# skhu101/SHERF

Hardware: AMD Instinct MI355X
Metric: rendered rays/sec at 512x512x64 samples (ImportanceRenderer.forward) (higher is better)
Workload: dtype f16 MFMA (fp16 operands rounded to nearest, one product, fp32 accumulate), fp32 elsewhere

## Files before the change

include/sherf_hip.h:

```cpp
#ifndef SHERF_HIP_H
#define SHERF_HIP_H
#include <stdint.h>

#ifdef __cplusplus
extern "C" {
#endif

typedef void* sherf_stream_t;

#define SHERF_OK 0
#define SHERF_EINVAL (-1)
#define SHERF_ELAUNCH (-2)

#define SHERF_V 6890
#define SHERF_NJ 24
#define SHERF_MAX_CELLS (64 * 64 * 64)
#define SHERF_SHELL_RADIUS 0.05f

int sherf_version(void);
const char* sherf_last_error(void);
int sherf_set_debug(int flags);

int sherf_smpl_bones(const float* poses, const float* shapes, int n_sets, const float* J_template,
                     const float* J_shapedirs, const int32_t* parents, float* A, float* posefeat,
                     sherf_stream_t stream);

int sherf_smpl_offsets(const float* posedirs, const float* shapedirs, const float* posefeat,
                       const float* shapes, int n_sets, float* PO, float* SO, sherf_stream_t stream);

int sherf_smpl_t2c_table(const float* weights, const float* A_tgt, const float* A_big, const float* PO_tgt,
                         const float* SO_tgt, const float* PO_big, float* T2C, sherf_stream_t stream);

int sherf_smpl_c2s_table(const float* weights, const float* A_big, const float* A_obs, const float* PO_big,
                         const float* SO_obs, const float* PO_obs, const float* R_obs, const float* Th_obs,
                         const float* cam_R, const float* cam_T, const float* cam_K, float* C2S,
                         sherf_stream_t stream);

int sherf_build_cells(const float* verts, int n, const float* R, const float* Th, float cell_size,
                      float* grid_hdr, int32_t* cell_start, float* cell_pts, int32_t* scratch,
                      uint32_t* near_mask, sherf_stream_t stream);
int sherf_build_cells2(const float* verts_a, const float* R_a, const float* Th_a, const float* verts_b, int n,
                       float cell_size, float* grid_hdr, int32_t* cell_start, float* cell_pts, int32_t* scratch,
                       uint32_t* near_mask, sherf_stream_t stream);
#define SHERF_NEAR_SUBCELLS 524288
int sherf_build_near_lists(const float* grid_hdr, const float* cell_pts, int n, float radius, int32_t* near_hdr,
                           uint16_t* near_list, int64_t list_cap, uint32_t* near_mask, sherf_stream_t stream);

int sherf_sample_mask_nn(const float* ray_o, const float* ray_d, const float* near, const float* far,
                         int R, int S, const float* Rg, const float* Th, const float* grid_hdr,
                         const int32_t* cell_start, const float* cell_pts, const uint32_t* near_mask,
                         int64_t capacity, int32_t* counters, int32_t* ray_base, int32_t* ray_cnt, int32_t* cs_idx,
                         int32_t* cs_vid, float* cs_xs, int32_t* dense_vid, uint64_t* ray_mask,
                         int32_t* scan_ws, const int32_t* near_hdr, const uint16_t* near_list, sherf_stream_t stream);

int sherf_warp_geom(const int32_t* counters, const int32_t* cs_idx, const int32_t* cs_vid, const float* cs_xs,
                    const float* ray_d, int S, const float* Rg, const float* T2C, const float* C2S,
                    const float* t_verts, const float* tgrid_hdr, const int32_t* tcell_start,
                    const float* tcell_pts, int64_t capacity, float* geom, int32_t* cs_tvid,
                    sherf_stream_t stream);

typedef struct {
    const uint32_t* wp;
    const float* rows;
    int32_t D, H, W;
} sherf_vox_level;

int sherf_gather_tokens(const int32_t* counters, const float* geom, const float* planes_f, int P,
                        const float* feat_f, int Hf, int Wf, const float* img4, int H, int W,
                        const sherf_vox_level* levels_host, const float* tok_bias, const float* bounds,
                        const float* vox_min, const int32_t* vox_sh_host, int mode, int64_t capacity, float* tokens,
                        float* extras, sherf_stream_t stream);

int sherf_gather_tokens_bwd(const int32_t* counters, const float* geom, const float* d_tokens, int P, int Hf, int Wf,
                            int H, int W, const sherf_vox_level* levels_host, const float* bounds, const float* vox_min,
                            const int32_t* vox_sh_host, int64_t capacity, float* d_planes_f, float* d_feat_f,
                            float* d_rows0, float* d_rows1, float* d_rows2, float* d_tok_bias, sherf_stream_t stream);
int sherf_gather_tokens_bwd_binned(const int32_t* counters, const float* geom, const float* d_tokens, int P, int Hf, int Wf,
                                   int H, int W, const sherf_vox_level* levels_host, const float* bounds, const float* vox_min,
                                   const int32_t* vox_sh_host, int64_t capacity, float* d_planes_f, float* d_feat_f,
                                   float* d_rows0, float* d_rows1, float* d_rows2, float* d_tok_bias, int32_t* scratch,
                                   int64_t scratch_words, sherf_stream_t stream);
int sherf_gather_bwd_scratch_words(const sherf_vox_level* levels_host, int64_t capacity, int64_t* words_host);
int sherf_gather_tokens_bwd_masked(const int32_t* counters, const float* geom, const float* d_tokens, int P, int Hf, int Wf,
                                   int H, int W, const sherf_vox_level* levels_host, const float* bounds, const float* vox_min,
                                   const int32_t* vox_sh_host, int64_t capacity, float* d_planes_f, float* d_feat_f,
                                   float* d_rows0, float* d_rows1, float* d_rows2, float* d_tok_bias, int32_t* scratch,
                                   int64_t scratch_words, int branches, sherf_stream_t stream);

int sherf_fold_tables(const float* in, const float* Wt, float* out, int HW, int groups, int pix_stride,
                      int64_t group_base, int out_half, sherf_stream_t stream);
int sherf_img_to_hwc4(const float* img, float* out, int HW, sherf_stream_t stream);

int sherf_nerf_mlp(const int32_t* counters, const float* tokens, const float* extras, const void* wstream,
                   const float* wbias, int prec, int64_t capacity, float* out, sherf_stream_t stream);
#define SHERF_MLP_NO_TRANSFORMER 256
#define SHERF_MLP_OSG_DECODER 512
int sherf_osg_decoder(const int32_t* counters, const float* tokens, const float* extras, const float* weights, int flags,
                      int64_t capacity, float* out, sherf_stream_t stream);
int sherf_nerf_mlp_part(const int32_t* counters, const float* tokens, const float* extras, const void* wstream,
                        const float* wbias, int prec, int64_t capacity, float* out, int part, int nparts, sherf_stream_t stream);
int sherf_nerf_mlp2(const int32_t* counters, const float* tokens, const float* extras, const void* wstream,
                    const float* wbias, int prec, int64_t capacity, float* out, sherf_stream_t stream);
int sherf_nerf_mlp3(const int32_t* counters, const float* tokens, const float* extras, const void* wstream,
                    const float* wbias, int prec, int64_t capacity, float* out, sherf_stream_t stream);
int sherf_nerf_mlp3_part(const int32_t* counters, const float* tokens, const float* extras, const void* wstream, const float* wbias, int prec,
                         int64_t capacity, float* out, int part, int nparts, int wgs_per_cu, sherf_stream_t stream);
int sherf_gather_tokens_pe(const int32_t* counters, const float* geom, const float* planes_f, int P,
                           const float* feat_f, int Hf, int Wf, const float* img4, int H, int W,
                           const sherf_vox_level* levels_host, const float* tok_bias, const float* bounds,
                           const float* vox_min, const int32_t* vox_sh_host, int mode, int64_t capacity, float* tokens,
                           float* extras, void* pefrag, sherf_stream_t stream);
int sherf_nerf_mlp3_pe(const int32_t* counters, const float* tokens, const float* extras, const void* pefrag, const void* wstream,
                       const float* wbias, int prec, int64_t capacity, float* out, sherf_stream_t stream);
int sherf_nerf_mlp_split(const int32_t* counters, const float* tokens, const float* extras, const void* wstream,
                         const float* wbias, int prec, int64_t capacity, void* zfrag, float* out, sherf_stream_t stream);
int sherf_mlp_pack_stream(const float* flat, const int32_t* src, int64_t n_slots, int prec, void* stream_out,
                          const int32_t* bias_src, int n_bias, float* bias_out, int32_t* flag, sherf_stream_t stream);
int sherf_mlp_stream_layout(int prec, int32_t* n_steps, int32_t* step_pieces_host, int32_t* units, int32_t max_steps);

#define SHERF_COMPOSITE_WHITE_BACK 1
#define SHERF_COMPOSITE_SOFTPLUS 2

int sherf_composite_compact(const int32_t* counters, const int32_t* ray_base, const int32_t* ray_cnt,
                            const int32_t* cs_idx, const float* sample_out, const float* ray_d,
                            const float* near, const float* far, int R, int S, int white_back, float* rgb,
                            float* depth, float* acc, sherf_stream_t stream);
int sherf_composite_compact_cap(int32_t* counters, const int32_t* ray_base, const int32_t* ray_cnt,
                                const int32_t* cs_idx, const float* sample_out, const float* ray_d,
                                const float* near, const float* far, int R, int S, int white_back, int64_t tok_cap,
                                float* rgb, float* depth, float* acc, sherf_stream_t stream);

int sherf_composite_compact_bwd(const int32_t* ray_base, const int32_t* ray_cnt, const int32_t* cs_idx,
                                const float* sample_out, const float* ray_d, const float* near, const float* far,
                                int R, int S, int white_back, const float* d_rgb, const float* d_acc,
                                float* d_sample_out, sherf_stream_t stream);

int sherf_composite_dense(const float* colors, const float* sigma, const float* depths, const float* rays_d,
                          int R, int S, int white_back, const float* dminmax, float* rgb, float* depth,
                          float* weights, sherf_stream_t stream);
int sherf_composite_dense_bwd(const float* colors, const float* sigma, const float* depths, const float* rays_d,
                              int R, int S, int white_back, const float* dminmax, const float* d_rgb,
                              const float* d_depth, const float* d_weights, float* d_colors, float* d_sigma,
                              sherf_stream_t stream);

int sherf_svox_mark_rows(const int32_t* coord, int n, int D, int H, int W, uint32_t* bitmap, sherf_stream_t stream);
int sherf_svox_mark_down(const int32_t* keys, const int32_t* n_rows, int D, int H, int W, uint32_t* bitmap_out,
                         int max_rows, sherf_stream_t stream);
int sherf_svox_scan(const uint32_t* bitmap, int n_words, int32_t* prefix, int32_t* n_rows, int32_t* chunk_ws,
                    uint32_t* wp, sherf_stream_t stream);
int sherf_svox_keys(const uint32_t* bitmap, const int32_t* prefix, int n_words, int32_t* keys, sherf_stream_t stream);
int sherf_svox_scatter_rows(const int32_t* coord, const float* feat, int n, int C, int D, int H, int W,
                            const uint32_t* bitmap, const int32_t* prefix, const int32_t* n_rows, int64_t* acc_fix,
                            float* g, int32_t* mult, sherf_stream_t stream);
int sherf_svox_conv3(const int32_t* keys_out, const int32_t* n_rows_out, int Do, int Ho, int Wo,
                     const uint32_t* wp_in, int Di, int Hi, int Wi, const float* in_raw, int Cin,
                     const float* in_bn, const int32_t* in_mult, const void* w_packed, int Cout, int mode,
                     int max_rows, float* out_raw, int64_t* out_acc, sherf_stream_t stream);
int sherf_svox_conv3_dgrad(const int32_t* keys_i, const int32_t* n_rows_i, int Di, int Hi, int Wi, const uint32_t* wp_o, int Do,
                           int Ho, int Wo, const float* d_raw, int Cout, const uint32_t* d_raw_amax, const void* w_packed_t,
                           int Cin, int down, int max_rows, float* d_in, sherf_stream_t stream);
int sherf_svox_bn_finalize(const int64_t* acc, const int32_t* n_total_rows, int C, const float* gamma, const float* beta,
                           float* stats, int training, float* bnparam, sherf_stream_t stream);
int sherf_svox_bn_running_update(int n_layers, const float* const* stats, float* const* running_mean, float* const* running_var,
                                 int64_t* const* num_batches_tracked, const int32_t* const* n_rows, const int32_t* channels,
                                 const float* momentum, sherf_stream_t stream);
#define SHERF_SVOX_MAX_LAYERS 16
typedef struct {
    uint32_t* bitmap;
    int32_t* prefix;
    int32_t* n_rows;
    int32_t* chunk_ws;
    uint32_t* wp;
    int32_t* keys;
    int32_t n_words, cap, D, H, W, pad_;
} sherf_svox_level_ws;
typedef struct {
    int32_t cin, cout, down, tap;
    const void* wt;
    const float* gamma;
    const float* beta;
    float* stats;
    float* bnparam;
    float* out;
    int64_t* acc;
} sherf_svox_layer;
typedef struct {
    sherf_svox_level_ws lev[4];
    sherf_svox_layer layers[SHERF_SVOX_MAX_LAYERS];
    int32_t n_layers, pad_;
    int64_t* acc_fix;
    float* g0;
    int32_t* mult;
    const int32_t* n_total;
    void* zero_ptr;
    int64_t zero_bytes;
    const float* fold_mat[3];
    float* fold_rows[3];
} sherf_svox_plan;
int sherf_svox_encode(const sherf_svox_plan* plan, const int32_t* coord, const float* feat, int n, int training,
                      sherf_vox_level* levels_out_host, sherf_stream_t stream);

#define SHERF_FRAME_EXACT_GRIDS 1
#define SHERF_FRAME_HALF_TABLES 2
#define SHERF_FRAME_ENCODER_SINGLE 4
#define SHERF_FRAME_MLP_SPLIT 8
#define SHERF_FRAME_MLP_TWO_TILES 32
#define SHERF_FRAME_MLP_PIPELINED 64
#define SHERF_FRAME_REPORT_COUNT 16
#define SHERF_FRAME_PE_FRAGS 128
#define SHERF_FRAME_REUSE_OBSERVATION 256
typedef struct {
    const float* poses; const float* shapes;
    const float* J_template; const float* J_shapedirs; const int32_t* parents;
    const float* posedirs; const float* shapedirs; const float* weights;
    float* A; float* posefeat; float* PO; float* SO; float* T2C; float* C2S;
    const float* obs_R; const float* obs_Th; const float* cam_R; const float* cam_T; const float* cam_K;
    const float* verts; const float* Rg; const float* Th; const float* tverts;
    float* grid_hdr; int32_t* cell_start; float* cell_pts; int32_t* cell_scratch; uint32_t* near_mask;
    const float* ray_o; const float* ray_d; const float* near; const float* far;
    int32_t R, S; int64_t capacity;
    int32_t* counters; int32_t* ray_base; int32_t* ray_cnt; int32_t* cs_idx; int32_t* cs_vid; float* cs_xs;
    int32_t* dense_vid; uint64_t* ray_mask; int32_t* scan_ws;
    const float* planes; const float* Wa_t; float* planes_f; int32_t P, flags;
    const float* obs_feat; const float* Wb_t; float* feat_f; int32_t Hf, Wf;
    const float* obs_img; float* img4; int32_t H, W;
    float* geom; int32_t* cs_tvid;
    const float* tok_bias; const float* bounds; const float* vox_min; int32_t vox_sh[3]; int32_t gather_split;
    float* tokens; float* extras;
    const sherf_svox_plan* vox_plan; const int32_t* vox_coord; const float* vox_feat; int32_t vox_n, vox_training;
    const void* wstream; const float* wbias; int32_t mlp_prec, mlp_parts; float* sample_out;
    int32_t white_back;
    int32_t main_after_layer;
    float* rgb; float* depth; float* acc;
    void* zfrag;
    int32_t* near_hdr; uint16_t* near_list; int64_t near_list_cap;
    int64_t tok_capacity;
    void* pefrag;
    int32_t* sticky;
} sherf_frame;
int sherf_render_frame(const sherf_frame* frame, int phase, sherf_vox_level* levels_out_host, sherf_stream_t stream_main,
                       sherf_stream_t stream_side, sherf_stream_t stream_aux);
int sherf_points_mask_nn(const float* points, int64_t n, const float* Rg, const float* Th, const float* grid_hdr,
                         const int32_t* cell_start, const float* cell_pts, const uint32_t* near_mask, int64_t capacity,
                         int32_t* counters, int32_t* ray_base, int32_t* ray_cnt, int32_t* cs_idx, int32_t* cs_vid, float* cs_xs,
                         int32_t* dense_vid, uint64_t* ray_mask, int32_t* scan_ws, const int32_t* near_hdr,
                         const uint16_t* near_list, sherf_stream_t stream);
int sherf_field_scatter(int32_t* counters, const uint64_t* ray_mask, const int32_t* ray_base, const float* sample_out,
                        int64_t n, int64_t tok_cap, float* rgb, float* sigma, uint8_t* mask, sherf_stream_t stream);
typedef struct {
    const float* points;
    const float* dirs;
    int64_t n;
    float* rgb;
    float* sigma;
    uint8_t* mask;
} sherf_field_query;
int sherf_query_field(const sherf_frame* frame, const sherf_field_query* query, sherf_vox_level* levels_out_host,
                      sherf_stream_t stream_main, sherf_stream_t stream_side, sherf_stream_t stream_aux);

int sherf_frame_count(int32_t* nv_host);
int sherf_frame_graphs(int enable);
int sherf_frame_graph_stats(int64_t* stats_host, int32_t n);
int sherf_frame_observation_stats(int64_t* stats_host, int32_t n);
int sherf_struct_sizes(int32_t* sizes_host, int32_t n);
#define SHERF_PROF_FIELDS 8
int sherf_profile_frames(int enable);
int sherf_profile_frames_read(float* ms_host, int32_t max_n, int32_t* n_host);

int sherf_vertex_features(const float* verts, const int32_t* tri, const int32_t* last_face, int V, const float* cam_R,
                          const float* cam_T, const float* cam_K, const float* feat, int Hf, int Wf, const float* img, int H, int W,
                          const float* Wp, const float* bp, float* f3d, uint8_t* front, sherf_stream_t stream);
int sherf_voxelize(const float* t_verts, const float* can, int V, float* bounds, int32_t* coord, int32_t* out_sh,
                   sherf_stream_t stream);

int sherf_ray_sampler(const float* cam2world, const float* intrinsics, int N, int res, float* origins,
                      float* dirs, sherf_stream_t stream);
int sherf_dataset_rays(const double* K_inv, const double* Rc, const double* Tc, const double* bounds, int H, int W,
                       float* ray_o, float* ray_d, float* near, float* far, uint8_t* mask_at_box,
                       sherf_stream_t stream);

#ifdef __cplusplus
}
#endif
#endif
```

sherf_amd/_lib.py:

```python
import ctypes
import os
import re

import torch

_HERE = os.path.dirname(os.path.abspath(__file__))
HEADER = os.path.join(_HERE, '..', 'include', 'sherf_hip.h')
LIB_PATH = os.environ.get('SHERF_HIP_LIB') or os.path.join(_HERE, 'libsherf_hip.so')

_lib = None
_protos = None


_vp, _i32, _i64 = ctypes.c_void_p, ctypes.c_int32, ctypes.c_int64


class VoxLevel(ctypes.Structure):
    _fields_ = [('wp', _vp), ('rows', _vp), ('D', _i32), ('H', _i32), ('W', _i32)]


class SvoxLevelWs(ctypes.Structure):
    _fields_ = [(n, _vp) for n in ('bitmap', 'prefix', 'n_rows', 'chunk_ws', 'wp', 'keys')] + \
               [(n, _i32) for n in ('n_words', 'cap', 'D', 'H', 'W', 'pad_')]


class SvoxLayer(ctypes.Structure):
    _fields_ = [(n, _i32) for n in ('cin', 'cout', 'down', 'tap')] + \
               [(n, _vp) for n in ('wt', 'gamma', 'beta', 'stats', 'bnparam', 'out', 'acc')]


SVOX_MAX_LAYERS = 16


class SvoxPlan(ctypes.Structure):
    _fields_ = [('lev', SvoxLevelWs * 4), ('layers', SvoxLayer * SVOX_MAX_LAYERS), ('n_layers', _i32), ('pad_', _i32),
                ('acc_fix', _vp), ('g0', _vp), ('mult', _vp), ('n_total', _vp), ('zero_ptr', _vp), ('zero_bytes', _i64),
                ('fold_mat', _vp * 3), ('fold_rows', _vp * 3)]


def _frame_fields():
    f = []
    P = lambda *names: f.extend((n, _vp) for n in names)
    I = lambda *names: f.extend((n, _i32) for n in names)
    P('poses', 'shapes', 'J_template', 'J_shapedirs', 'parents', 'posedirs', 'shapedirs', 'weights',
      'A', 'posefeat', 'PO', 'SO', 'T2C', 'C2S', 'obs_R', 'obs_Th', 'cam_R', 'cam_T', 'cam_K',
      'verts', 'Rg', 'Th', 'tverts', 'grid_hdr', 'cell_start', 'cell_pts', 'cell_scratch', 'near_mask',
      'ray_o', 'ray_d', 'near', 'far')
    I('R', 'S')
    f.append(('capacity', _i64))
    P('counters', 'ray_base', 'ray_cnt', 'cs_idx', 'cs_vid', 'cs_xs', 'dense_vid', 'ray_mask', 'scan_ws')
    P('planes', 'Wa_t', 'planes_f'); I('P', 'flags')
    P('obs_feat', 'Wb_t', 'feat_f'); I('Hf', 'Wf')
    P('obs_img', 'img4'); I('H', 'W')
    P('geom', 'cs_tvid', 'tok_bias', 'bounds', 'vox_min')
    f.append(('vox_sh', _i32 * 3)); I('gather_split')
    P('tokens', 'extras', 'vox_plan', 'vox_coord', 'vox_feat'); I('vox_n', 'vox_training')
    P('wstream', 'wbias'); I('mlp_prec', 'mlp_parts')
    P('sample_out'); I('white_back', 'main_after_layer')
    P('rgb', 'depth', 'acc', 'zfrag', 'near_hdr', 'near_list')
    f.append(('near_list_cap', _i64))
    f.append(('tok_capacity', _i64))
    P('pefrag')
    P('sticky')
    return f


class Frame(ctypes.Structure):
    _fields_ = _frame_fields()


class FieldQuery(ctypes.Structure):
    _fields_ = [('points', _vp), ('dirs', _vp), ('n', _i64), ('rgb', _vp), ('sigma', _vp), ('mask', _vp)]


_STRUCTS = (VoxLevel, SvoxLevelWs, SvoxLayer, SvoxPlan, Frame)


COMPOSITE_WHITE_BACK, COMPOSITE_SOFTPLUS = 1, 2
CLAMP_MODES = ('relu', 'softplus')


def composite_bits(white_back, clamp_mode='relu'):
    if clamp_mode not in CLAMP_MODES:
        raise AssertionError("MipRayMarcher only supports `clamp_mode`=`softplus`!")
    return (COMPOSITE_WHITE_BACK if white_back else 0) | (COMPOSITE_SOFTPLUS if clamp_mode == 'softplus' else 0)


BRANCH_PLANES, BRANCH_PIXEL, BRANCH_VOXEL = 1, 2, 4


def branch_mask(on):
    return (BRANCH_PLANES if on[0] else 0) | (BRANCH_PIXEL if on[1] else 0) | (BRANCH_VOXEL if on[2] else 0)


MLP_NO_TRANSFORMER, MLP_OSG_DECODER = 256, 512


FRAME_REUSE_OBSERVATION = 256


def frame_observation_stats():
    s = (ctypes.c_int64 * 2)()
    call('sherf_frame_observation_stats', s, 2)
    return int(s[0]), int(s[1])


_SCALARS = {'int': ctypes.c_int, 'int32_t': ctypes.c_int32, 'int64_t': ctypes.c_int64, 'float': ctypes.c_float,
            'sherf_stream_t': ctypes.c_void_p}


def parse_header(path=HEADER):
    src = open(path).read()
    src = re.sub(r'/\*.*?\*/', '', src, flags=re.S)
    protos = {}
    for m in re.finditer(r'(int|const char\*)\s+(sherf_\w+)\s*\(([^;{]*?)\)\s*;', src, flags=re.S):
        ret, name, args = m.group(1), m.group(2), m.group(3).strip()
        parsed = []
        if args and args != 'void':
            for a in args.split(','):
                a = ' '.join(a.split())
                is_ptr = '*' in a
                base = a.replace('const ', '').replace('*', ' ').split()
                ctype = ctypes.c_void_p if is_ptr else _SCALARS[base[0]]
                parsed.append((ctype, is_ptr, base[-1]))
        protos[name] = (ctypes.c_char_p if ret != 'int' else ctypes.c_int, parsed)
    return protos


def _init():
    global _lib, _protos
    if _lib is not None:
        return _lib
    if not os.path.exists(LIB_PATH):
        raise RuntimeError(f'{LIB_PATH} not found: build it with `python -m sherf_amd.build` '
                           '(hipcc --offload-arch=gfx950). There is no CPU fallback.')
    lib = ctypes.CDLL(LIB_PATH)
    _protos = parse_header()
    for name, (ret, args) in _protos.items():
        fn = getattr(lib, name)
        fn.restype = ret
        fn.argtypes = [a[0] for a in args]
    sizes = (ctypes.c_int32 * len(_STRUCTS))()
    if lib.sherf_struct_sizes(sizes, len(_STRUCTS)) != 0 or [int(v) for v in sizes] != [ctypes.sizeof(c) for c in _STRUCTS]:
        raise RuntimeError(f'struct layout mismatch between include/sherf_hip.h and sherf_amd/_lib.py: '
                           f'{[int(v) for v in sizes]} vs {[ctypes.sizeof(c) for c in _STRUCTS]}')
    _lib = lib
    return lib


def lib():
    return _init()


def addr(t, dtype=None):
    p = ptr(t, dtype)
    return None if p is None else p.value


def ptr(t, dtype=None, channels_last_ok=False):
    if t is None:
        return None
    if not isinstance(t, torch.Tensor):
        raise RuntimeError(f'expected a tensor, got {type(t)}')
    if not t.is_cuda:
        raise RuntimeError('sherf_amd: tensor is not on a GPU; the HIP path has no CPU fallback')
    if not t.is_contiguous() and not (channels_last_ok and t.ndim == 4 and t.is_contiguous(memory_format=torch.channels_last)):
        raise RuntimeError('sherf_amd: tensor must be contiguous')
    if dtype is not None and t.dtype != dtype:
        raise RuntimeError(f'sherf_amd: expected dtype {dtype}, got {t.dtype}')
    return ctypes.c_void_p(t.data_ptr())


def stream():
    return ctypes.c_void_p(torch.cuda.current_stream().cuda_stream)


def call(name, *args):
    l = _init()
    rc = getattr(l, name)(*args)
    if rc != 0:
        raise RuntimeError(f'{name} failed ({rc}): {l.sherf_last_error().decode()}')


HEADER_BWD = os.path.join(_HERE, '..', 'include', 'sherf_hip_bwd.h')
LIB_BWD_PATH = os.path.join(_HERE, 'libsherf_hip_bwd.so')
_lib_bwd = None


def lib_bwd():
    global _lib_bwd
    if _lib_bwd is None:
        if not os.path.exists(LIB_BWD_PATH):
            raise RuntimeError(f'{LIB_BWD_PATH} not found: build it with `python -m sherf_amd.build`')
        l = ctypes.CDLL(LIB_BWD_PATH)
        for name, (ret, args) in parse_header(HEADER_BWD).items():
            fn = getattr(l, name)
            fn.restype = ret
            fn.argtypes = [a[0] for a in args]
        _lib_bwd = l
    return _lib_bwd


def call_bwd(name, *args):
    l = lib_bwd()
    rc = getattr(l, name)(*args)
    if rc != 0:
        raise RuntimeError(f'{name} failed ({rc}): {l.sherf_bwd_last_error().decode()}')


HEADER_OPS = os.path.join(_HERE, '..', 'include', 'sherf_hip_ops.h')
LIB_OPS_PATH = os.path.join(_HERE, 'libsherf_hip_ops.so')
_lib_ops = None


def lib_ops():
    global _lib_ops
    if _lib_ops is None:
        if not os.path.exists(LIB_OPS_PATH):
            raise RuntimeError(f'{LIB_OPS_PATH} not found: build it with `python -m sherf_amd.build`. There is no CPU fallback.')
        l = ctypes.CDLL(LIB_OPS_PATH)
        for name, (ret, args) in parse_header(HEADER_OPS).items():
            fn = getattr(l, name)
            fn.restype = ret
            fn.argtypes = [a[0] for a in args]
        _lib_ops = l
    return _lib_ops


def call_ops(name, *args):
    l = lib_ops()
    rc = getattr(l, name)(*args)
    if rc != 0:
        raise RuntimeError(f'{name} failed ({rc}): {l.sherf_ops_last_error().decode()}')
```

sherf_amd/csrc/frame.hip:

```cpp
#include "common.h"

#include <algorithm>
#include <chrono>
#include <cstdlib>
#include <functional>
#include <mutex>

int sherf_svox_encode_impl(const sherf_svox_plan* p, const int32_t* coord, const float* feat, int n, int training,
                           sherf_vox_level* levels_out_host, sherf_stream_t stream, hipEvent_t ev, int ev_layer,
                           sherf_stream_t aux, hipEvent_t* lev_ev, const std::function<int()>* after_levels, int fold_half);
int sherf_sample_mask_nn_impl(const float* ray_o, const float* ray_d, const float* near, const float* far, int R, int S, const float* Rg, const float* Th,
                              const float* grid_hdr, const int32_t* cell_start, const float* cell_pts, const uint32_t* near_mask, int64_t capacity,
                              int32_t* counters, int32_t* ray_base, int32_t* ray_cnt, int32_t* cs_idx, int32_t* cs_vid, float* cs_xs, int32_t* dense_vid,
                              uint64_t* ray_mask, int32_t* scan_ws, const int32_t* near_hdr, const uint16_t* near_list, sherf_stream_t stream,
                              int32_t* sticky);
int sherf_warp_geom_impl(const int32_t* counters, const int32_t* cs_idx, const int32_t* cs_vid, const float* cs_xs, const float* ray_d, int S, const float* Rg,
                         const float* T2C, const float* C2S, const float* t_verts, const float* tgrid_hdr, const int32_t* tcell_start, const float* tcell_pts,
                         int64_t capacity, float* geom, int32_t* cs_tvid, sherf_stream_t stream);
int sherf_points_mask_nn_impl(const float* points, int64_t n, const float* Rg, const float* Th, const float* grid_hdr, const int32_t* cell_start,
                              const float* cell_pts, const uint32_t* near_mask, int64_t capacity, int32_t* counters, int32_t* ray_base, int32_t* ray_cnt,
                              int32_t* cs_idx, int32_t* cs_vid, float* cs_xs, int32_t* dense_vid, uint64_t* ray_mask, int32_t* scan_ws, const int32_t* near_hdr,
                              const uint16_t* near_list, sherf_stream_t stream, int32_t* sticky);

namespace {

constexpr int kMaxDev = 16;
constexpr int kRing = 64;
constexpr int kMaxParts = 8;

struct DevState {
    bool init = false;
    hipEvent_t ev_start, ev_smpl, ev_enc, ev_mid, ev_fold, ev_lev[8], ev_cnt, ev_part[kMaxParts], ev_mlp;
    int32_t* host_nv = nullptr;
    hipEvent_t ev_rep[8];
    int rep_next = 0;
    unsigned long long rep_seq[8] = {0, 0, 0, 0, 0, 0, 0, 0}, rep_counter = 0;
    hipStream_t cap_stream = nullptr;
};
thread_local int t_rep_last[kMaxDev] = {-1, -1, -1, -1, -1, -1, -1, -1, -1, -1, -1, -1, -1, -1, -1, -1};
thread_local unsigned long long t_rep_seq[kMaxDev] = {0};
DevState g_dev[kMaxDev];
std::mutex g_mu;
std::mutex g_frame_mu;

constexpr int kEv = 7;
bool g_prof_on = false;
int g_prof_n = 0;
hipEvent_t g_prof_ev[kRing][kEv];
float g_prof_host_ms[kRing];
bool g_prof_init = false;

}

extern "C" int sherf_struct_sizes(int32_t* sizes_host, int32_t n) {
    SHERF_CHECK_ARG(sizes_host && n >= 5);
    sizes_host[0] = (int32_t)sizeof(sherf_vox_level);
    sizes_host[1] = (int32_t)sizeof(sherf_svox_level_ws);
    sizes_host[2] = (int32_t)sizeof(sherf_svox_layer);
    sizes_host[3] = (int32_t)sizeof(sherf_svox_plan);
    sizes_host[4] = (int32_t)sizeof(sherf_frame);
    return SHERF_OK;
}

extern "C" int sherf_profile_frames(int enable) {
    std::lock_guard<std::mutex> lk(g_mu);
    if (enable && !g_prof_init) {
        for (int i = 0; i < kRing; ++i)
            for (int j = 0; j < kEv; ++j) SHERF_HIP_CHECK(hipEventCreate(&g_prof_ev[i][j]));
        g_prof_init = true;
    }
    g_prof_on = enable != 0;
    g_prof_n = 0;
    return SHERF_OK;
}

extern "C" int sherf_profile_frames_read(float* ms_host, int32_t max_n, int32_t* n_host) {
    SHERF_CHECK_ARG(ms_host && n_host && max_n > 0);
    std::lock_guard<std::mutex> lk(g_mu);
    const int have = g_prof_n < kRing ? g_prof_n : kRing;
    const int n = have < max_n ? have : max_n;
    const int first = g_prof_n - have;
    for (int i = 0; i < n; ++i) {
        const int slot = (first + i) % kRing;
        float* o = ms_host + (size_t)i * SHERF_PROF_FIELDS;
        SHERF_HIP_CHECK(hipEventSynchronize(g_prof_ev[slot][kEv - 1]));
        o[0] = g_prof_host_ms[slot];
        for (int j = 1; j < kEv; ++j) SHERF_HIP_CHECK(hipEventElapsedTime(&o[j], g_prof_ev[slot][0], g_prof_ev[slot][j]));
        o[7] = o[5] - o[4];
    }
    *n_host = n;
    return SHERF_OK;
}

extern "C" int sherf_frame_count(int32_t* nv_host) {
    SHERF_CHECK_ARG(nv_host);
    int dev = 0;
    SHERF_HIP_CHECK(hipGetDevice(&dev));
    SHERF_CHECK_ARG(dev >= 0 && dev < kMaxDev);
    DevState& d = g_dev[dev];
    const int slot = t_rep_last[dev];
    hipEvent_t ev;
    auto overtaken = [&]() -> int {
        snprintf(g_sherf_err, sizeof(g_sherf_err), "sherf_frame_count: eight later frames on this device have reused the slot of this thread's last frame");
        return SHERF_EINVAL;
    };
    {
        std::lock_guard<std::mutex> frame_lock(g_frame_mu);
        SHERF_CHECK_ARG(d.init && slot >= 0);
        if (d.rep_seq[slot] != t_rep_seq[dev]) return overtaken();
        ev = d.ev_rep[slot];
    }
    SHERF_HIP_CHECK(hipEventSynchronize(ev));
    const int32_t nv = d.host_nv[8 + slot];
    {
        std::lock_guard<std::mutex> frame_lock(g_frame_mu);
        if (d.rep_seq[slot] != t_rep_seq[dev]) return overtaken();
    }
    *nv_host = nv;
    return SHERF_OK;
}

static int render_frame_enqueue(const sherf_frame* f, int phase, sherf_vox_level* levels, sherf_stream_t stream_main,
                                sherf_stream_t stream_side, sherf_stream_t stream_aux, const sherf_field_query* q = nullptr) {
    hipStream_t main = as_stream(stream_main), side = as_stream(stream_side);
    if (phase == 4) {
        SHERF_CHECK_ARG(f->R > 0 && f->S > 0 && f->capacity > 0);
        const bool lists = f->near_hdr && f->near_list;
        SHERF_RUN(sherf_build_cells2(f->verts, f->Rg, f->Th, f->tverts, SHERF_V, 0.05f, f->grid_hdr, f->cell_start, f->cell_pts,
                                     f->cell_scratch, lists ? nullptr : f->near_mask, stream_main));
        if (lists)
            SHERF_RUN(sherf_build_near_lists(f->grid_hdr, f->cell_pts, SHERF_V, 0.05f, f->near_hdr, f->near_list, f->near_list_cap, f->near_mask, stream_main));
        SHERF_RUN(sherf_sample_mask_nn_impl(f->ray_o, f->ray_d, f->near, f->far, f->R, f->S, f->Rg, f->Th, f->grid_hdr, f->cell_start,
                                       f->cell_pts, f->near_mask, f->capacity, f->counters, f->ray_base, f->ray_cnt, f->cs_idx,
                                       f->cs_vid, f->cs_xs, f->dense_vid, f->ray_mask, f->scan_ws, f->near_hdr, f->near_list, stream_main, f->sticky));
        return SHERF_OK;
    }
    const int64_t tok_cap = (f->tok_capacity > 0 && f->tok_capacity < f->capacity) ? f->tok_capacity : f->capacity;
    const auto host_t0 = std::chrono::steady_clock::now();
    static int cur_slot = -1;
#define SHERF_PROF(j, strm) do { if (cur_slot >= 0) SHERF_HIP_CHECK(hipEventRecord(g_prof_ev[cur_slot][j], strm)); } while (0)
    if (phase & 1) {
        int dev = 0;
        SHERF_HIP_CHECK(hipGetDevice(&dev));
        SHERF_CHECK_ARG(dev >= 0 && dev < kMaxDev);
        DevState& d = g_dev[dev];
        {
            std::lock_guard<std::mutex> lk(g_mu);
            if (!d.init) {
                const unsigned evf = hipEventDisableTiming | ((sherf_experiment() & 4) ? hipEventReleaseToDevice : 0u);
                SHERF_HIP_CHECK(hipEventCreateWithFlags(&d.ev_start, evf));
                SHERF_HIP_CHECK(hipEventCreateWithFlags(&d.ev_smpl, evf));
                SHERF_HIP_CHECK(hipEventCreateWithFlags(&d.ev_enc, evf));
                SHERF_HIP_CHECK(hipEventCreateWithFlags(&d.ev_mid, evf));
                SHERF_HIP_CHECK(hipEventCreateWithFlags(&d.ev_fold, evf));
                for (int k = 0; k < 8; ++k) SHERF_HIP_CHECK(hipEventCreateWithFlags(&d.ev_lev[k], evf));
                SHERF_HIP_CHECK(hipEventCreateWithFlags(&d.ev_cnt, hipEventDisableTiming));
                for (int k = 0; k < kMaxParts; ++k) SHERF_HIP_CHECK(hipEventCreateWithFlags(&d.ev_part[k], evf));
                SHERF_HIP_CHECK(hipEventCreateWithFlags(&d.ev_mlp, evf));
                SHERF_HIP_CHECK(hipHostMalloc(reinterpret_cast<void**>(&d.host_nv), 64, 0));
                for (int k = 0; k < 8; ++k) SHERF_HIP_CHECK(hipEventCreateWithFlags(&d.ev_rep[k], hipEventDisableTiming));
                d.init = true;
            }
        }
        SHERF_CHECK_ARG((q || (f->R > 0 && f->S > 0)) && f->capacity > 0 && f->vox_plan);
        const int V = SHERF_V;
        {
            std::lock_guard<std::mutex> lk(g_mu);
            cur_slot = g_prof_on ? g_prof_n % kRing : -1;
        }
        const int xp = sherf_experiment();
        SHERF_HOST_STAMP(xp, "frame enter");
        SHERF_PROF(0, main);
        SHERF_GPU_STAMP(xp, main, "frame start");
        SHERF_CAP_TRACE("record ev_start");
        SHERF_HIP_CHECK(hipEventRecord(d.ev_start, main));
        SHERF_CAP_TRACE("side waits ev_start");
        SHERF_HIP_CHECK(hipStreamWaitEvent(side, d.ev_start, 0));
        const bool reuse = (f->flags & SHERF_FRAME_REUSE_OBSERVATION) != 0;
        auto smpl_tables = [&](sherf_stream_t st) -> int {
            SHERF_RUN(sherf_smpl_bones(f->poses, f->shapes, 3, f->J_template, f->J_shapedirs, f->parents, f->A, f->posefeat, st));
            SHERF_RUN(sherf_smpl_offsets(f->posedirs, f->shapedirs, f->posefeat, f->shapes, 3, f->PO, f->SO, st));
            const float *A0 = f->A, *A1 = f->A + 24 * 12, *A2 = f->A + 2 * 24 * 12;
            const float *PO0 = f->PO, *PO1 = f->PO + V * 3, *PO2 = f->PO + 2 * V * 3;
            const float *SO0 = f->SO, *SO2 = f->SO + 2 * V * 3;
            SHERF_RUN(sherf_smpl_t2c_table(f->weights, A0, A1, PO0, SO0, PO1, f->T2C, st));
            SHERF_RUN(sherf_smpl_c2s_table(f->weights, A1, A2, PO1, SO2, PO2, f->obs_R, f->obs_Th, f->cam_R, f->cam_T, f->cam_K,
                                           f->C2S, st));
            SHERF_HIP_CHECK(hipEventRecord(d.ev_smpl, as_stream(st)));
            SHERF_PROF(1, as_stream(st));
            return SHERF_OK;
        };
        if (!stream_aux) SHERF_RUN(smpl_tables(stream_side));
        const int stagger = reuse ? -1 : f->main_after_layer;
        const int half_tables = (f->flags & SHERF_FRAME_HALF_TABLES) ? 1 : 0;
        auto fold_tables = [&](sherf_stream_t st) -> int {
            SHERF_RUN(sherf_fold_tables(f->planes, f->Wa_t, f->planes_f, f->P * f->P, 3, 32, (int64_t)f->P * f->P * 32, half_tables, st));
            SHERF_RUN(sherf_fold_tables(f->obs_feat, f->Wb_t, f->feat_f, f->Hf * f->Wf, 2, 64, 32, half_tables, st));
            return sherf_img_to_hwc4(f->obs_img, f->img4, f->H * f->W, st);
        };
        SHERF_CAP_TRACE("fold tables on aux");
        if (stream_aux) {
            SHERF_HIP_CHECK(hipStreamWaitEvent(as_stream(stream_aux), d.ev_start, 0));
            if (reuse) {
                SHERF_RUN(smpl_tables(stream_aux));
            } else {
                SHERF_RUN(fold_tables(stream_aux));
                SHERF_HIP_CHECK(hipEventRecord(d.ev_fold, as_stream(stream_aux)));
            }
        }
        const size_t ncell1 = (size_t)SHERF_MAX_CELLS + 1;
        auto enqueue_encoder = [&]() -> int {
            if (reuse) {
                SHERF_PROF(2, side);
                return SHERF_OK;
            }
            const std::function<int()> smpl_on_aux = [&]() -> int { return smpl_tables(stream_aux); };
            SHERF_RUN(sherf_svox_encode_impl(f->vox_plan, f->vox_coord, f->vox_feat, f->vox_n, f->vox_training, levels, stream_side,
                                             stagger >= 0 ? d.ev_mid : nullptr, stagger, stream_aux, d.ev_lev,
                                             stream_aux ? &smpl_on_aux : nullptr,
                                             half_tables | ((f->flags & SHERF_FRAME_ENCODER_SINGLE) ? 2 : 0)));
            SHERF_HIP_CHECK(hipEventRecord(d.ev_enc, side));
            SHERF_PROF(2, side);
            return SHERF_OK;
        };
        const bool encoder_first = stagger >= 0 || (xp & 8);
        SHERF_CAP_TRACE("cells");
        if (encoder_first) SHERF_RUN(enqueue_encoder());
        const bool lists = f->near_hdr && f->near_list;
        SHERF_RUN(sherf_build_cells2(f->verts, f->Rg, f->Th, f->tverts, V, 0.05f, f->grid_hdr, f->cell_start, f->cell_pts,
                                     f->cell_scratch, lists ? nullptr : f->near_mask, stream_main));
        if (stagger >= 0) SHERF_HIP_CHECK(hipStreamWaitEvent(main, stagger < f->vox_plan->n_layers ? d.ev_mid : d.ev_enc, 0));
        SHERF_CAP_TRACE("near lists");
        if (lists)
            SHERF_RUN(sherf_build_near_lists(f->grid_hdr, f->cell_pts, V, 0.05f, f->near_hdr, f->near_list, f->near_list_cap, f->near_mask, stream_main));
        SHERF_CAP_TRACE("sampler");
        if (q)
            SHERF_RUN(sherf_points_mask_nn_impl(q->points, q->n, f->Rg, f->Th, f->grid_hdr, f->cell_start, f->cell_pts, f->near_mask, f->capacity, f->counters,
                                                f->ray_base, f->ray_cnt, f->cs_idx, f->cs_vid, f->cs_xs, f->dense_vid, f->ray_mask, f->scan_ws, f->near_hdr,
                                                f->near_list, stream_main, f->sticky));
        else
        SHERF_RUN(sherf_sample_mask_nn_impl(f->ray_o, f->ray_d, f->near, f->far, f->R, f->S, f->Rg, f->Th, f->grid_hdr, f->cell_start,
                                       f->cell_pts, f->near_mask, f->capacity, f->counters, f->ray_base, f->ray_cnt, f->cs_idx,
                                       f->cs_vid, f->cs_xs, f->dense_vid, f->ray_mask, f->scan_ws, f->near_hdr, f->near_list, stream_main, f->sticky));
        SHERF_CAP_TRACE("sampler queued");
        if (f->flags & SHERF_FRAME_REPORT_COUNT) {
            const int slot = d.rep_next;
            d.rep_next = (d.rep_next + 1) % 8;
            SHERF_HIP_CHECK(hipMemcpyAsync(d.host_nv + 8 + slot, f->counters, sizeof(int32_t), hipMemcpyDeviceToHost, main));
            SHERF_HIP_CHECK(hipEventRecord(d.ev_rep[slot], main));
            t_rep_last[dev] = slot;
            d.rep_seq[slot] = t_rep_seq[dev] = ++d.rep_counter;
        }
        const bool exact = (f->flags & SHERF_FRAME_EXACT_GRIDS) != 0;
        if (exact) {
            SHERF_HIP_CHECK(hipMemcpyAsync(d.host_nv, f->counters, sizeof(int32_t), hipMemcpyDeviceToHost, main));
            SHERF_HIP_CHECK(hipEventRecord(d.ev_cnt, main));
        }
        SHERF_CAP_TRACE("encoder");
        if (!encoder_first) SHERF_RUN(enqueue_encoder());
        SHERF_CAP_TRACE("encoder queued");
        if (!stream_aux && !reuse) SHERF_RUN(fold_tables(stream_main));
        SHERF_HIP_CHECK(hipStreamWaitEvent(main, d.ev_smpl, 0));
        if (stream_aux && !reuse) SHERF_HIP_CHECK(hipStreamWaitEvent(main, d.ev_fold, 0));
        int64_t cap = tok_cap;
        if (exact) {
            SHERF_HOST_STAMP(xp, "count wait begins");
            SHERF_HIP_CHECK(hipEventSynchronize(d.ev_cnt));
            SHERF_HOST_STAMP(xp, "count wait ends");
            int64_t c = *d.host_nv > 0 ? ((int64_t)*d.host_nv + 255) / 256 * 256 : 256;
            if (c < cap) cap = c;
        }
        SHERF_CAP_TRACE("warp");
        if (q)
            SHERF_RUN(sherf_warp_geom_impl(f->counters, f->cs_idx, f->cs_vid, f->cs_xs, q->dirs, 1, f->Rg, f->T2C, f->C2S, f->tverts,
                                           f->grid_hdr + kGridHdr, f->cell_start + ncell1, f->cell_pts + (size_t)V * 4, cap, f->geom,
                                           f->cs_tvid, stream_main));
        else
        SHERF_RUN(sherf_warp_geom(f->counters, f->cs_idx, f->cs_vid, f->cs_xs, f->ray_d, f->S, f->Rg, f->T2C, f->C2S, f->tverts,
                                  f->grid_hdr + kGridHdr, f->cell_start + ncell1, f->cell_pts + (size_t)V * 4, cap, f->geom,
                                  f->cs_tvid, stream_main));
        const int gv = ((f->gather_split & 2) ? 4 : 0) | ((f->gather_split & 4) ? 12 : 0) |
                       (half_tables ? 16 : 0);
        const bool osg = (f->mlp_prec & SHERF_MLP_OSG_DECODER) != 0;
        const int nparts = osg ? 1 : std::min(((g_sherf_debug >> 16) & 15) ? ((g_sherf_debug >> 16) & 15) : f->mlp_parts, kMaxParts);
        const bool split_form = !osg && f->zfrag && (((f->flags & SHERF_FRAME_MLP_SPLIT) != 0) != ((g_sherf_debug & 8192) != 0));
        const bool pe_frags = !osg && (f->flags & SHERF_FRAME_PE_FRAGS) && f->pefrag && half_tables && (f->mlp_prec & 255) == 2 && (f->flags & SHERF_FRAME_MLP_PIPELINED) &&
                              !(g_sherf_debug & (1 << 25)) && !split_form && nparts <= 1 && !(f->gather_split & 7) && !(g_sherf_debug & (2048 | (1 << 29)));
        if (nparts > 1 && !(f->gather_split & 1) && !split_form) {
            SHERF_PROF(3, main);
            if (!reuse) SHERF_HIP_CHECK(hipStreamWaitEvent(main, d.ev_enc, 0));
            for (int k = 0; k < nparts; ++k) {
                SHERF_RUN(sherf_gather_tokens(f->counters, f->geom, f->planes_f, f->P, f->feat_f, f->Hf, f->Wf, f->img4, f->H, f->W,
                                              levels, f->tok_bias, f->bounds, f->vox_min, f->vox_sh, 0 | gv | (k << 8) | (nparts << 16), cap,
                                              f->tokens, f->extras, stream_main));
                SHERF_HIP_CHECK(hipEventRecord(d.ev_part[k], main));
                SHERF_HIP_CHECK(hipStreamWaitEvent(side, d.ev_part[k], 0));
                if ((f->mlp_prec & 255) != 1 && (f->flags & SHERF_FRAME_MLP_PIPELINED))
                    SHERF_RUN(sherf_nerf_mlp3_part(f->counters, f->tokens, f->extras, f->wstream, f->wbias, f->mlp_prec, cap, f->sample_out, k, nparts,
                                                   (g_sherf_debug & (1 << 26)) ? 3 : (g_sherf_debug & (1 << 27)) ? 1 : 2, stream_side));
                else
                    SHERF_RUN(sherf_nerf_mlp_part(f->counters, f->tokens, f->extras, f->wstream, f->wbias, f->mlp_prec, cap, f->sample_out, k, nparts,
                                                  stream_side));
            }
            SHERF_PROF(4, main);
            SHERF_HIP_CHECK(hipEventRecord(d.ev_mlp, side));
            SHERF_HIP_CHECK(hipStreamWaitEvent(main, d.ev_mlp, 0));
            SHERF_PROF(5, main);
        } else {
        if (f->gather_split & 1) {
            SHERF_RUN(sherf_gather_tokens(f->counters, f->geom, f->planes_f, f->P, f->feat_f, f->Hf, f->Wf, f->img4, f->H, f->W,
                                          nullptr, f->tok_bias, f->bounds, f->vox_min, f->vox_sh, 1 | gv, cap, f->tokens,
                                          f->extras, stream_main));
            SHERF_PROF(3, main);
            if (!reuse) SHERF_HIP_CHECK(hipStreamWaitEvent(main, d.ev_enc, 0));
            SHERF_RUN(sherf_gather_tokens(f->counters, f->geom, f->planes_f, f->P, f->feat_f, f->Hf, f->Wf, f->img4, f->H, f->W,
                                          levels, f->tok_bias, f->bounds, f->vox_min, f->vox_sh, 2 | gv, cap, f->tokens,
                                          f->extras, stream_main));
        } else {
            SHERF_PROF(3, main);
            if (!reuse) SHERF_HIP_CHECK(hipStreamWaitEvent(main, d.ev_enc, 0));
            if (pe_frags)
                SHERF_RUN(sherf_gather_tokens_pe(f->counters, f->geom, f->planes_f, f->P, f->feat_f, f->Hf, f->Wf, f->img4, f->H, f->W,
                                                 levels, f->tok_bias, f->bounds, f->vox_min, f->vox_sh, 0 | gv, cap, f->tokens,
                                                 f->extras, f->pefrag, stream_main));
            else
            SHERF_RUN(sherf_gather_tokens(f->counters, f->geom, f->planes_f, f->P, f->feat_f, f->Hf, f->Wf, f->img4, f->H, f->W,
                                          levels, f->tok_bias, f->bounds, f->vox_min, f->vox_sh, 0 | gv, cap, f->tokens,
                                          f->extras, stream_main));
        }
        SHERF_CAP_TRACE("network");
        SHERF_PROF(4, main);
        const bool split = split_form;
        if (osg)
            SHERF_RUN(sherf_osg_decoder(f->counters, f->tokens, f->extras, static_cast<const float*>(f->wstream), (f->mlp_prec & SHERF_MLP_NO_TRANSFORMER) ? 1 : 0, cap,
                                        f->sample_out, stream_main));
        else if (pe_frags)
            SHERF_RUN(sherf_nerf_mlp3_pe(f->counters, f->tokens, f->extras, f->pefrag, f->wstream, f->wbias, f->mlp_prec, cap, f->sample_out, stream_main));
        else if (split)
            SHERF_RUN(sherf_nerf_mlp_split(f->counters, f->tokens, f->extras, f->wstream, f->wbias, f->mlp_prec, cap, f->zfrag,
                                           f->sample_out, stream_main));
        else if ((f->mlp_prec & 255) != 1 && (((f->flags & SHERF_FRAME_MLP_PIPELINED) != 0) != ((g_sherf_debug & (1 << 25)) != 0)))
            SHERF_RUN(sherf_nerf_mlp3(f->counters, f->tokens, f->extras, f->wstream, f->wbias, f->mlp_prec, cap, f->sample_out, stream_main));
        else if ((f->mlp_prec & 255) != 1 && (((f->flags & SHERF_FRAME_MLP_TWO_TILES) != 0) != ((g_sherf_debug & (1 << 24)) != 0)))
            SHERF_RUN(sherf_nerf_mlp2(f->counters, f->tokens, f->extras, f->wstream, f->wbias, f->mlp_prec, cap, f->sample_out, stream_main));
        else
            SHERF_RUN(sherf_nerf_mlp(f->counters, f->tokens, f->extras, f->wstream, f->wbias, f->mlp_prec, cap,
                                     f->sample_out, stream_main));
        SHERF_PROF(5, main);
        }
    }
    if (phase & 2) {
        SHERF_CAP_TRACE("compositing");
        if (q)
            SHERF_RUN(sherf_field_scatter(f->counters, f->ray_mask, f->ray_base, f->sample_out, q->n, tok_cap, q->rgb, q->sigma, q->mask, stream_main));
        else
        SHERF_RUN(sherf_composite_compact_cap(f->counters, f->ray_base, f->ray_cnt, f->cs_idx, f->sample_out, f->ray_d, f->near, f->far,
                                              f->R, f->S, f->white_back, tok_cap, f->rgb, f->depth, f->acc, stream_main));
        SHERF_PROF(6, main);
        SHERF_HOST_STAMP(sherf_experiment(), "frame leave");
        if (cur_slot >= 0) {
            std::lock_guard<std::mutex> lk(g_mu);
            g_prof_host_ms[cur_slot] = std::chrono::duration<float, std::milli>(std::chrono::steady_clock::now() - host_t0).count();
            ++g_prof_n;
            cur_slot = -1;
        }
    }
#undef SHERF_PROF
    return SHERF_OK;
}

namespace {

struct GraphEntry {
    uint64_t key = 0, stamp = 0;
    int state = 0;
    hipGraph_t graph = nullptr;
    hipGraphExec_t exec = nullptr;
    sherf_vox_level lv[3];
};
constexpr int kGraphSlots = 8;
GraphEntry g_graphs[kMaxDev][kGraphSlots];
uint64_t g_graph_clock = 0;
int g_graph_on = -1;
bool g_graph_aux_ok = false;
int64_t g_graph_stats[4] = {0, 0, 0, 0};
int64_t g_obs_stats[2] = {0, 0};

inline void fnv(uint64_t& h, const void* p, size_t n) {
    const unsigned char* b = static_cast<const unsigned char*>(p);
    for (size_t i = 0; i < n; ++i) { h ^= b[i]; h *= 1099511628211ull; }
}

void graph_drop(GraphEntry& e) {
    if (e.exec) (void)hipGraphExecDestroy(e.exec);
    if (e.graph) (void)hipGraphDestroy(e.graph);
    e = GraphEntry();
}

}

extern "C" int sherf_frame_graphs(int enable) {
    std::lock_guard<std::mutex> frame_lock(g_frame_mu);
    g_graph_on = enable ? 1 : 0;
    if (!enable)
        for (auto& dev : g_graphs)
            for (auto& e : dev) graph_drop(e);
    return SHERF_OK;
}

extern "C" int sherf_frame_graph_stats(int64_t* stats_host, int32_t n) {
    SHERF_CHECK_ARG(stats_host && n >= 4);
    std::lock_guard<std::mutex> frame_lock(g_frame_mu);
    for (int i = 0; i < 4; ++i) stats_host[i] = g_graph_stats[i];
    return SHERF_OK;
}

extern "C" int sherf_frame_observation_stats(int64_t* stats_host, int32_t n) {
    SHERF_CHECK_ARG(stats_host && n >= 2);
    std::lock_guard<std::mutex> frame_lock(g_frame_mu);
    for (int i = 0; i < 2; ++i) stats_host[i] = g_obs_stats[i];
    return SHERF_OK;
}

static int check_frame_call(const sherf_frame* f, int phase, const sherf_vox_level* levels, sherf_stream_t stream_main, sherf_stream_t stream_side,
                            sherf_stream_t stream_aux) {
    SHERF_CHECK_ARG(f && levels && ((phase & 3) || phase == 4) && stream_side != stream_main && (!stream_aux || (stream_aux != stream_main && stream_aux != stream_side)));
    SHERF_CHECK_ARG((f->white_back & ~(SHERF_COMPOSITE_WHITE_BACK | SHERF_COMPOSITE_SOFTPLUS)) == 0);
    SHERF_CHECK_ARG(!(f->mlp_prec & SHERF_MLP_OSG_DECODER) || f->wstream);
    if (phase != 4 && (phase & 1) && (f->flags & SHERF_FRAME_REUSE_OBSERVATION)) {
        SHERF_CHECK_ARG(f->vox_plan && f->planes_f && f->feat_f && f->img4);
        for (int i = 0; i < 3; ++i)
            SHERF_CHECK_ARG(levels[i].wp && levels[i].rows && levels[i].rows == f->vox_plan->fold_rows[i] && levels[i].D > 0 && levels[i].H > 0 && levels[i].W > 0);
    }
    return SHERF_OK;
}

extern "C" int sherf_query_field(const sherf_frame* f, const sherf_field_query* q, sherf_vox_level* levels, sherf_stream_t stream_main,
                                 sherf_stream_t stream_side, sherf_stream_t stream_aux) {
    SHERF_CHECK_ARG(q && q->points && q->dirs && q->rgb && q->sigma && q->mask && q->n > 0 && q->n < 2147483648LL);
    SHERF_RUN(check_frame_call(f, 3, levels, stream_main, stream_side, stream_aux));
    SHERF_CHECK_ARG(f->capacity > 0 && f->capacity >= q->n && f->vox_plan);
    std::lock_guard<std::mutex> frame_lock(g_frame_mu);
    ++g_obs_stats[(f->flags & SHERF_FRAME_REUSE_OBSERVATION) ? 1 : 0];
    return render_frame_enqueue(f, 3, levels, stream_main, stream_side, stream_aux, q);
}

extern "C" int sherf_render_frame(const sherf_frame* f, int phase, sherf_vox_level* levels, sherf_stream_t stream_main,
                                  sherf_stream_t stream_side, sherf_stream_t stream_aux) {
    SHERF_RUN(check_frame_call(f, phase, levels, stream_main, stream_side, stream_aux));
    std::lock_guard<std::mutex> frame_lock(g_frame_mu);
    if (phase != 4 && (phase & 1)) ++g_obs_stats[(f->flags & SHERF_FRAME_REUSE_OBSERVATION) ? 1 : 0];
    if (g_graph_on < 0) {
        const char* e = getenv("SHERF_FRAME_GRAPH");
        g_graph_on = (e && atoi(e) != 0) ? 1 : 0;
        const char* ea = getenv("SHERF_FRAME_GRAPH_AUX");
        g_graph_aux_ok = ea && atoi(ea) != 0;
    }
    int dev = 0;
    bool prof;
    { std::lock_guard<std::mutex> lk(g_mu); prof = g_prof_on; }
    const int xp = sherf_experiment();
    const bool eligible = g_graph_on == 1 && (phase == 1 || phase == 3) && !prof && !(f->flags & (SHERF_FRAME_EXACT_GRIDS | SHERF_FRAME_REPORT_COUNT)) &&
                          !(xp & (16 | 32)) && f->vox_plan && hipGetDevice(&dev) == hipSuccess && dev >= 0 && dev < kMaxDev && g_dev[dev].init &&
                          (!stream_aux || g_graph_aux_ok);
    if (!eligible) {
        ++g_graph_stats[2];
        return render_frame_enqueue(f, phase, levels, stream_main, stream_side, stream_aux);
    }
    uint64_t key = 1469598103934665603ull;
    fnv(key, f, sizeof(*f));
    fnv(key, f->vox_plan, sizeof(*f->vox_plan));
    const uint64_t words[7] = {(uint64_t)phase, (uint64_t)(size_t)stream_main, (uint64_t)(size_t)stream_side, (uint64_t)(size_t)stream_aux,
                               (uint64_t)(unsigned)g_sherf_debug, (uint64_t)(unsigned)xp, (uint64_t)dev};
    fnv(key, words, sizeof(words));
    if (key == 0) key = 1;
    GraphEntry* slot = nullptr;
    GraphEntry* lru = &g_graphs[dev][0];
    for (auto& e : g_graphs[dev]) {
        if (e.state && e.key == key) { slot = &e; break; }
        if (e.stamp < lru->stamp) lru = &e;
    }
    hipStream_t main = as_stream(stream_main);
    if (slot && slot->state == 2) {
        slot->stamp = ++g_graph_clock;
        for (int i = 0; i < 3; ++i) levels[i] = slot->lv[i];
        SHERF_HIP_CHECK(hipGraphLaunch(slot->exec, main));
        ++g_graph_stats[1];
        return SHERF_OK;
    }
    if (!slot) {
        graph_drop(*lru);
        lru->key = key; lru->state = 1; lru->stamp = ++g_graph_clock;
        ++g_graph_stats[2];
        return render_frame_enqueue(f, phase, levels, stream_main, stream_side, stream_aux);
    }
    slot->stamp = ++g_graph_clock;
    if (slot->state == 3) {
        ++g_graph_stats[2];
        return render_frame_enqueue(f, phase, levels, stream_main, stream_side, stream_aux);
    }
    hipGraph_t graph = nullptr;
    hipGraphExec_t exec = nullptr;
    int rc = SHERF_ELAUNCH;
    const char* stage = "stream";
    hipError_t e = hipSuccess;
    DevState& d = g_dev[dev];
    if (!d.cap_stream) e = hipStreamCreateWithFlags(&d.cap_stream, hipStreamNonBlocking);
    bool ok = e == hipSuccess && d.cap_stream;
    g_sherf_cap_trace = getenv("SHERF_FRAME_GRAPH_DEBUG") ? 1 : 0;
    SHERF_CAP_TRACE("begin");
    if (ok) { stage = "begin"; e = hipStreamBeginCapture(d.cap_stream, hipStreamCaptureModeThreadLocal); ok = e == hipSuccess; }
    if (ok) {
        stage = "enqueue";
        rc = render_frame_enqueue(f, phase, levels, reinterpret_cast<sherf_stream_t>(d.cap_stream), stream_side, stream_aux);
        SHERF_CAP_TRACE("end capture");
        e = hipStreamEndCapture(d.cap_stream, &graph);
        SHERF_CAP_TRACE("capture ended");
        if (rc == SHERF_OK) stage = "end";
        ok = rc == SHERF_OK && e == hipSuccess && graph != nullptr;
    }
    if (ok) { stage = "instantiate"; SHERF_CAP_TRACE(stage); e = hipGraphInstantiate(&exec, graph, nullptr, nullptr, 0); ok = e == hipSuccess && exec != nullptr; }
    if (ok) { stage = "launch"; SHERF_CAP_TRACE(stage); e = hipGraphLaunch(exec, main); ok = e == hipSuccess; }
    SHERF_CAP_TRACE("done");
    g_sherf_cap_trace = 0;
    if (!ok) {
        if (getenv("SHERF_FRAME_GRAPH_DEBUG"))
            fprintf(stderr, "[sherf] frame graph: capture failed at '%s' (rc %d, %s: %s); this descriptor renders launch by launch\n", stage, rc,
                    hipGetErrorName(e), rc != SHERF_OK ? g_sherf_err : hipGetErrorString(e));
        (void)hipGetLastError();
        if (exec) (void)hipGraphExecDestroy(exec);
        if (graph) (void)hipGraphDestroy(graph);
        slot->state = 3;
        ++g_graph_stats[3]; ++g_graph_stats[2];
        return render_frame_enqueue(f, phase, levels, stream_main, stream_side, stream_aux);
    }
    slot->graph = graph; slot->exec = exec; slot->state = 2;
    for (int i = 0; i < 3; ++i) slot->lv[i] = levels[i];
    ++g_graph_stats[0];
    return SHERF_OK;
}
```

sherf_amd/csrc/sample.hip:

```cpp
#include "common.h"

namespace {

constexpr float kThresh2 = (float)(0.05 * 0.05);
constexpr float kShellRadius = SHERF_SHELL_RADIUS;

constexpr int kLdsCells = 24576;

__device__ __forceinline__ void build_cells_body(const float* __restrict__ verts, int n,
                                                           const float* __restrict__ R, const float* __restrict__ Th,
                                                           float cell_size, float* __restrict__ hdr,
                                                           int32_t* __restrict__ cell_start, float4* __restrict__ cell_pts,
                                                           int32_t* __restrict__ scratch, uint32_t* __restrict__ near_mask) {
    __shared__ float red[6][1024 / 64];
    __shared__ float s_hdr[kGridHdr];
    __shared__ int s_part[1024];
    const int tid = threadIdx.x, lane = tid & 63, wave = tid >> 6;
    float* pos = reinterpret_cast<float*>(scratch) ;
    int32_t* cid = scratch + 3 * n;
    int32_t* rank = scratch + 4 * n;
    float mn[3] = {3.0e38f, 3.0e38f, 3.0e38f}, mx[3] = {-3.0e38f, -3.0e38f, -3.0e38f};
    for (int i = tid; i < n; i += 1024) {
        float x = verts[i * 3], y = verts[i * 3 + 1], z = verts[i * 3 + 2];
        if (R) to_smpl_frame(x, y, z, R, Th, x, y, z);
        pos[i * 3] = x; pos[i * 3 + 1] = y; pos[i * 3 + 2] = z;
        mn[0] = fminf(mn[0], x); mn[1] = fminf(mn[1], y); mn[2] = fminf(mn[2], z);
        mx[0] = fmaxf(mx[0], x); mx[1] = fmaxf(mx[1], y); mx[2] = fmaxf(mx[2], z);
    }
    for (int c = 0; c < 3; ++c) {
        float a = mn[c], b = mx[c];
        for (int off = 32; off > 0; off >>= 1) { a = fminf(a, __shfl_xor(a, off)); b = fmaxf(b, __shfl_xor(b, off)); }
        if (lane == 0) { red[c][wave] = a; red[3 + c][wave] = b; }
    }
    __syncthreads();
    if (tid == 0) {
        float lo[3], hi[3];
        for (int c = 0; c < 3; ++c) {
            lo[c] = red[c][0]; hi[c] = red[3 + c][0];
            for (int w = 1; w < 16; ++w) { lo[c] = fminf(lo[c], red[c][w]); hi[c] = fmaxf(hi[c], red[3 + c][w]); }
        }
        float cell = cell_size;
        for (int c = 0; c < 3; ++c) cell = fmaxf(cell, (hi[c] - lo[c]) / 60.0f);
        float inv = 1.0f / cell;
        int dims[3];
        for (int c = 0; c < 3; ++c) dims[c] = min(64, (int)floorf((hi[c] - lo[c]) * inv) + 3);
        for (int c = 0; c < 3; ++c) {
            float o = lo[c] - cell;
            const float step = fmaxf(fabsf(lo[c]), cell) * 2.4e-7f;
            for (int it = 0; it < 8 && (lo[c] - o) * inv < 1.0f; ++it) o -= step;
            s_hdr[c] = o;
        }
        s_hdr[3] = cell; s_hdr[4] = inv;
        s_hdr[5] = __int_as_float(dims[0]); s_hdr[6] = __int_as_float(dims[1]); s_hdr[7] = __int_as_float(dims[2]);
        const int sub = (8 * dims[0] * dims[1] * dims[2] <= 16384 * 32) ? 2 : 1;
        s_hdr[8] = __int_as_float(sub); s_hdr[9] = s_hdr[10] = s_hdr[11] = 0.f;
        for (int i = 0; i < kGridHdr; ++i) hdr[i] = s_hdr[i];
    }
    __syncthreads();
    const float ox = s_hdr[0], oy = s_hdr[1], oz = s_hdr[2], inv = s_hdr[4];
    const int nx = __float_as_int(s_hdr[5]), ny = __float_as_int(s_hdr[6]), nz = __float_as_int(s_hdr[7]);
    const int ncell = nx * ny * nz;
    if (ncell + 1 <= kLdsCells && n <= 8 * 1024) {
        __shared__ int s_cnt[kLdsCells];
        for (int i = tid; i <= ncell; i += 1024) s_cnt[i] = 0;
        __syncthreads();
        constexpr int kPer = 8;
        float px[kPer], py[kPer], pz[kPer];
        int pc[kPer], pr[kPer];
#pragma unroll
        for (int k = 0; k < kPer; ++k) {
            const int i = tid + k * 1024;
            pc[k] = -1;
            if (i < n) {
                px[k] = pos[i * 3]; py[k] = pos[i * 3 + 1]; pz[k] = pos[i * 3 + 2];
                const int cx = min(nx - 1, max(0, (int)floorf((px[k] - ox) * inv)));
                const int cy = min(ny - 1, max(0, (int)floorf((py[k] - oy) * inv)));
                const int cz = min(nz - 1, max(0, (int)floorf((pz[k] - oz) * inv)));
                pc[k] = (cz * ny + cy) * nx + cx;
                pr[k] = atomicAdd(&s_cnt[pc[k]], 1);
            }
        }
        __syncthreads();
        const int seg = (ncell + 1 + 1023) / 1024;
        const int s0 = tid * seg, s1 = min(ncell + 1, s0 + seg);
        int sum = 0;
        for (int i = s0; i < s1; ++i) sum += s_cnt[i];
        s_part[tid] = sum;
        __syncthreads();
        for (int off = 1; off < 1024; off <<= 1) {
            int v = tid >= off ? s_part[tid - off] : 0;
            __syncthreads();
            s_part[tid] += v;
            __syncthreads();
        }
        int run = s_part[tid] - sum;
        for (int i = s0; i < s1; ++i) { const int c = s_cnt[i]; s_cnt[i] = run; run += c; }
        __syncthreads();
        for (int i = tid; i <= ncell; i += 1024) cell_start[i] = s_cnt[i];
#pragma unroll
        for (int k = 0; k < kPer; ++k)
            if (pc[k] >= 0) cell_pts[s_cnt[pc[k]] + pr[k]] = make_float4(px[k], py[k], pz[k], __int_as_float(tid + k * 1024));
        return;
    }
    for (int i = tid; i <= ncell; i += 1024) cell_start[i] = 0;
    __syncthreads();
    for (int i = tid; i < n; i += 1024) {
        int cx = min(nx - 1, max(0, (int)floorf((pos[i * 3] - ox) * inv)));
        int cy = min(ny - 1, max(0, (int)floorf((pos[i * 3 + 1] - oy) * inv)));
        int cz = min(nz - 1, max(0, (int)floorf((pos[i * 3 + 2] - oz) * inv)));
        int c = (cz * ny + cy) * nx + cx;
        cid[i] = c;
        rank[i] = atomicAdd(&cell_start[c], 1);
    }
    __syncthreads();
    const int seg = (ncell + 1 + 1023) / 1024;
    const int s0 = tid * seg, s1 = min(ncell + 1, s0 + seg);
    int sum = 0;
    for (int i = s0; i < s1; ++i) sum += __hip_atomic_load(&cell_start[i], __ATOMIC_RELAXED, __HIP_MEMORY_SCOPE_AGENT);
    s_part[tid] = sum;
    __syncthreads();
    for (int off = 1; off < 1024; off <<= 1) {
        int v = tid >= off ? s_part[tid - off] : 0;
        __syncthreads();
        s_part[tid] += v;
        __syncthreads();
    }
    int run = s_part[tid] - sum;
    for (int i = s0; i < s1; ++i) {
        int c = __hip_atomic_load(&cell_start[i], __ATOMIC_RELAXED, __HIP_MEMORY_SCOPE_AGENT);
        cell_start[i] = run; run += c;
    }
    __syncthreads();
    for (int i = tid; i < n; i += 1024)
        cell_pts[cell_start[cid[i]] + rank[i]] = make_float4(pos[i * 3], pos[i * 3 + 1], pos[i * 3 + 2], __int_as_float(i));
}

__global__ void __launch_bounds__(1024) build_cells_kernel(const float* __restrict__ verts, int n, const float* __restrict__ R,
                                                           const float* __restrict__ Th, float cell_size, float* __restrict__ hdr,
                                                           int32_t* __restrict__ cell_start, float4* __restrict__ cell_pts,
                                                           int32_t* __restrict__ scratch, uint32_t* __restrict__ near_mask) {
    build_cells_body(verts, n, R, Th, cell_size, hdr, cell_start, cell_pts, scratch, near_mask);
}

__global__ void __launch_bounds__(1024) build_cells2_kernel(const float* __restrict__ verts_a, const float* __restrict__ R_a,
                                                            const float* __restrict__ Th_a, const float* __restrict__ verts_b, int n,
                                                            float cell_size, float* __restrict__ hdr, int32_t* __restrict__ cell_start,
                                                            float4* __restrict__ cell_pts, int32_t* __restrict__ scratch,
                                                            uint32_t* __restrict__ near_mask) {
    if (blockIdx.x == 0)
        build_cells_body(verts_a, n, R_a, Th_a, cell_size, hdr, cell_start, cell_pts, scratch, near_mask);
    else
        build_cells_body(verts_b, n, nullptr, nullptr, cell_size, hdr + kGridHdr, cell_start + (SHERF_MAX_CELLS + 1), cell_pts + n,
                         scratch + 5 * n, nullptr);
}

__global__ void __launch_bounds__(256) near_mask_kernel(const float* __restrict__ pos, int n, const float* __restrict__ hdr,
                                                        float radius, uint32_t* __restrict__ near_mask) {
    extern __shared__ uint32_t s_mask[];
    const CellGrid g = load_grid(hdr);
    const int sub = g.sub, snx = g.nx * sub, sny = g.ny * sub, snz = g.nz * sub;
    const int words = (snx * sny * snz + 31) / 32;
    for (int w = threadIdx.x; w < words; w += 256) s_mask[w] = 0u;
    __syncthreads();
    const int i = blockIdx.x * 256 + threadIdx.x;
    if (i < n) {
        const float px = pos[i * 3], py = pos[i * 3 + 1], pz = pos[i * 3 + 2];
        const float cs = g.cell / (float)sub, rad = radius + 1e-3f * cs, rad2 = rad * rad, fs = g.inv_cell * (float)sub;
        const int sx = (int)floorf((px - g.ox) * fs), sy = (int)floorf((py - g.oy) * fs), sz = (int)floorf((pz - g.oz) * fs);
        for (int dz = -sub; dz <= sub; ++dz)
            for (int dy = -sub; dy <= sub; ++dy)
                for (int dx = -sub; dx <= sub; ++dx) {
                    const int qx = sx + dx, qy = sy + dy, qz = sz + dz;
                    if (qx < 0 || qx >= snx || qy < 0 || qy >= sny || qz < 0 || qz >= snz) continue;
                    const float bx = g.ox + qx * cs, by = g.oy + qy * cs, bz = g.oz + qz * cs;
                    const float ex = fmaxf(fmaxf(bx - px, px - (bx + cs)), 0.f), ey = fmaxf(fmaxf(by - py, py - (by + cs)), 0.f),
                                ez = fmaxf(fmaxf(bz - pz, pz - (bz + cs)), 0.f);
                    if (ex * ex + ey * ey + ez * ez < rad2) {
                        const int q = (qz * sny + qy) * snx + qx;
                        atomicOr(&s_mask[q >> 5], 1u << (q & 31));
                    }
                }
    }
    __syncthreads();
    for (int w = threadIdx.x; w < words; w += 256) {
        const uint32_t m = s_mask[w];
        if (m) atomicOr(&near_mask[w], m);
    }
}

template <bool FILL>
__global__ void __launch_bounds__(256) near_lists_pairs_kernel(const float4* __restrict__ pts, int n, const float* __restrict__ hdr,
                                                               float radius, int2* __restrict__ near_hdr,
                                                               uint16_t* __restrict__ near_list, int64_t list_cap, int32_t* __restrict__ cursor) {
    const CellGrid g = load_grid(hdr);
    const int sub = g.sub, snx = g.nx * sub, sny = g.ny * sub, snz = g.nz * sub;
    if (!FILL && cursor && blockIdx.x == 0 && threadIdx.x == 0) { cursor[0] = 0; cursor[1] = 0; }
    const int i = (blockIdx.x * 256 + threadIdx.x) >> 5, t = threadIdx.x & 31;
    if (i >= n) return;
    const float4 p = pts[i];
    const float cs = g.cell / (float)sub, rad = radius + 1e-3f * cs, rad2 = rad * rad, fs = g.inv_cell * (float)sub;
    const int sx = (int)floorf((p.x - g.ox) * fs), sy = (int)floorf((p.y - g.oy) * fs), sz = (int)floorf((p.z - g.oz) * fs);
    const int w = 2 * sub + 1, w3 = w * w * w;
    for (int e = t; e < w3; e += 32) {
        const int dz = e / (w * w) - sub, dy = (e / w) % w - sub, dx = e % w - sub;
        const int qx = sx + dx, qy = sy + dy, qz = sz + dz;
        if (qx < 0 || qx >= snx || qy < 0 || qy >= sny || qz < 0 || qz >= snz) continue;
        const float bx = g.ox + qx * cs, by = g.oy + qy * cs, bz = g.oz + qz * cs;
        const float ex = fmaxf(fmaxf(bx - p.x, p.x - (bx + cs)), 0.f), ey = fmaxf(fmaxf(by - p.y, p.y - (by + cs)), 0.f),
                    ez = fmaxf(fmaxf(bz - p.z, p.z - (bz + cs)), 0.f);
        if (ex * ex + ey * ey + ez * ez < rad2) {
            const int q = (qz * sny + qy) * snx + qx;
            if (!FILL) atomicAdd(&near_hdr[q].y, 1);
            else {
                const int start = near_hdr[q].x;
                const int64_t at = (int64_t)start + atomicAdd(&near_hdr[q].y, 1);
                if (at < list_cap) near_list[at] = (uint16_t)i;
            }
        }
    }
}

__global__ void __launch_bounds__(256) near_lists_alloc_kernel(const float* __restrict__ hdr, int2* __restrict__ near_hdr, int32_t* __restrict__ cursor,
                                                               int64_t list_cap, uint32_t* __restrict__ near_mask) {
    const CellGrid g = load_grid(hdr);
    const int nsub = g.nx * g.ny * g.nz * g.sub * g.sub * g.sub;
    if ((int)blockIdx.x * 256 >= ((nsub + 63) & ~63)) return;
    const int q = blockIdx.x * 256 + threadIdx.x, lane = threadIdx.x & 63;
    const int c = q < nsub ? near_hdr[q].y : 0;
    const int pc = (c + 3) & ~3;
    int incl = pc;
    for (int off = 1; off < 64; off <<= 1) { const int v = __shfl_up(incl, off); if (lane >= off) incl += v; }
    const int total = __shfl(incl, 63);
    int base = 0;
    if (lane == 0 && total) base = atomicAdd(cursor, total);
    base = __shfl(base, 0);
    const unsigned long long any = __ballot(c > 0);
    if (near_mask && (lane & 31) == 0) near_mask[q >> 5] = (uint32_t)(any >> (lane & 32));
    if (q < nsub) {
        const int64_t start = (int64_t)base + (incl - pc);
        near_hdr[q] = start + pc <= list_cap ? make_int2((int)start, 0) : make_int2(0, 0);
    }
}

__device__ __forceinline__ float depth_at(float near, float range, int k, int S) {
    float step = __fdiv_rn((float)k, (float)(S - 1));
    return __fadd_rn(near, __fmul_rn(step, range));
}

struct Cand { float x, y, z; uint16_t s[9]; uint16_t cum[9]; unsigned long long key; };
static_assert(sizeof(Cand) == 56, "candidate record layout");
constexpr int kMaxPtsUnroll = 4;

template <int NCH>
__global__ void __launch_bounds__(256) sample_nn_kernel(const float* __restrict__ ray_o, const float* __restrict__ ray_d,
                                                        const float* __restrict__ near, const float* __restrict__ far,
                                                        int R, int S, const float* __restrict__ Rg,
                                                        const float* __restrict__ Th, const float* __restrict__ hdr,
                                                        const int32_t* __restrict__ cell_start,
                                                        const float4* __restrict__ cell_pts,
                                                        const uint32_t* __restrict__ near_mask,
                                                        int32_t* __restrict__ ray_cnt, uint64_t* __restrict__ ray_mask,
                                                        int32_t* __restrict__ dense_vid, int dbg) {
    __shared__ Cand s_cand[4][64];
    const int lane = threadIdx.x & 63, wave = threadIdx.x >> 6;
    const int ray = blockIdx.x * 4 + wave;
    if (ray >= R) return;
    const CellGrid g = load_grid(hdr);
    const float o0 = ray_o[ray * 3], o1 = ray_o[ray * 3 + 1], o2 = ray_o[ray * 3 + 2];
    const float d0 = ray_d[ray * 3], d1 = ray_d[ray * 3 + 1], d2 = ray_d[ray * 3 + 2];
    const float nr = near[ray], range = __fsub_rn(far[ray], nr);
    const unsigned long long kInit = ((unsigned long long)__float_as_uint(kThresh2) << 32) | 0x7FFFFFFFull;
    Cand* const rec = s_cand[wave];
    const int grp = lane >> 3, sub = lane & 7;
    int total = 0;
#pragma unroll
    for (int ch = 0; ch < NCH; ++ch) {
        const int k = ch * 64 + lane;
        bool cand = false;
        float xs = 0.f, ys = 0.f, zs = 0.f;
        int cx = 0, cy = 0, cz = 0;
        if (k < S) {
            float t = depth_at(nr, range, k, S);
            float x = __fadd_rn(o0, __fmul_rn(t, d0)), y = __fadd_rn(o1, __fmul_rn(t, d1)), z = __fadd_rn(o2, __fmul_rn(t, d2));
            to_smpl_frame(x, y, z, Rg, Th, xs, ys, zs);
            const float fs = g.inv_cell * (float)g.sub;
            const int sx = (int)floorf((xs - g.ox) * fs), sy = (int)floorf((ys - g.oy) * fs), sz = (int)floorf((zs - g.oz) * fs);
            cx = g.sub == 2 ? sx >> 1 : sx; cy = g.sub == 2 ? sy >> 1 : sy; cz = g.sub == 2 ? sz >> 1 : sz;
            if (sx >= 0 && cx < g.nx && sy >= 0 && cy < g.ny && sz >= 0 && cz < g.nz) {
                const int q = (sz * (g.ny * g.sub) + sy) * (g.nx * g.sub) + sx;
                cand = (((dbg & 2) || ((near_mask[q >> 5] >> (q & 31)) & 1u)) && !(dbg & 1));
            }
        }
        const unsigned long long cmask = __ballot(cand);
        const int ncand = __popcll(cmask);
        const int rank = __popcll(cmask & ((1ull << lane) - 1ull));
        if (cand) {
            Cand& c = rec[rank];
            c.x = xs; c.y = ys; c.z = zs; c.key = kInit;
            const float r = 0.05f + 1e-4f * g.cell;
            int st[9], en[9];
#pragma unroll
            for (int i = 0; i < 9; ++i) {
                const int qz = cz + i / 3 - 1, qy = cy + i % 3 - 1;
                const float y0 = g.oy + qy * g.cell, z0 = g.oz + qz * g.cell;
                const float ey = fmaxf(fmaxf(y0 - ys, ys - (y0 + g.cell)), 0.f), ez = fmaxf(fmaxf(z0 - zs, zs - (z0 + g.cell)), 0.f);
                const float rem = r * r - (ey * ey + ez * ez);
                const bool ok = qz >= 0 && qz < g.nz && qy >= 0 && qy < g.ny && rem > 0.f;
                const float rx = sqrtf(fmaxf(rem, 0.f)) + 1e-4f * g.cell;
                const int x0 = max(max((int)floorf((xs - rx - g.ox) * g.inv_cell), cx - 1), 0);
                const int x1 = min(min((int)floorf((xs + rx - g.ox) * g.inv_cell), cx + 1), g.nx - 1);
                const int row = ok ? (qz * g.ny + qy) * g.nx : 0;
                st[i] = cell_start[row + (ok ? x0 : 0)];
                en[i] = ok && x1 >= x0 ? cell_start[row + x1 + 1] : st[i];
            }
            int cum = 0;
#pragma unroll
            for (int i = 0; i < 9; ++i) { c.s[i] = (uint16_t)st[i]; cum += en[i] - st[i]; c.cum[i] = (uint16_t)cum; }
        }
        __builtin_amdgcn_wave_barrier();
        for (int c0 = 0; c0 < ncand; c0 += 8) {
            const int ci = c0 + grp;
            if (ci < ncand) {
                Cand& c = rec[ci];
                const float qx = c.x, qy = c.y, qz = c.z;
                int bs[9], cum[9];
#pragma unroll
                for (int i = 0; i < 9; ++i) { bs[i] = c.s[i]; cum[i] = c.cum[i]; }
                const int npts = cum[8];
                for (int base = 0; base < npts; base += 8 * kMaxPtsUnroll) {
                    float4 v[kMaxPtsUnroll];
#pragma unroll
                    for (int u = 0; u < kMaxPtsUnroll; ++u) {
                        const int t = base + u * 8 + sub;
                        int p = bs[0] + t;
#pragma unroll
                        for (int i = 1; i < 9; ++i) p = (t >= cum[i - 1]) ? bs[i] + (t - cum[i - 1]) : p;
                        v[u] = cell_pts[t < npts ? p : 0];
                    }
#pragma unroll
                    for (int u = 0; u < kMaxPtsUnroll; ++u) {
                        const int t = base + u * 8 + sub;
                        const float dd = dist2_exact(qx, qy, qz, v[u].x, v[u].y, v[u].z);
                        if (t < npts && dd < kThresh2)
                            atomicMin(&c.key, ((unsigned long long)__float_as_uint(dd) << 32) | (unsigned)__float_as_int(v[u].w));
                    }
                }
            }
        }
        __builtin_amdgcn_wave_barrier();
        const unsigned long long my_key = cand ? __hip_atomic_load(&rec[rank].key, __ATOMIC_RELAXED, __HIP_MEMORY_SCOPE_WAVEFRONT) : kInit;
        __builtin_amdgcn_wave_barrier();
        const bool valid = (unsigned)(my_key >> 32) < __float_as_uint(kThresh2);
        const uint64_t m = __ballot(valid);
        if (valid) dense_vid[(size_t)ray * S + k] = (int)(my_key & 0x7FFFFFFFull);
        if (lane == 0) ray_mask[(size_t)ray * NCH + ch] = m;
        total += __popcll(m);
    }
    if (lane == 0) ray_cnt[ray] = total;
}

constexpr int kMarkRays = 4;

template <int NCH>
__global__ void __launch_bounds__(256) cand_mark_kernel(const float* __restrict__ ray_o, const float* __restrict__ ray_d,
                                                        const float* __restrict__ near, const float* __restrict__ far, int R, int S,
                                                        const float* __restrict__ Rg, const float* __restrict__ Th,
                                                        const float* __restrict__ hdr, const uint32_t* __restrict__ near_mask,
                                                        float4* __restrict__ cand_list, int64_t list_cap, int32_t* __restrict__ cand_count,
                                                        uint64_t* __restrict__ ray_mask, int dbg) {
    constexpr int RPW = 16 / NCH;
    __shared__ int s_list[4096];
    __shared__ int s_n, s_base;
    const int lane = threadIdx.x & 63, wave = threadIdx.x >> 6;
    if (threadIdx.x == 0) s_n = 0;
    __syncthreads();
    const CellGrid g = load_grid(hdr);
    const float fs = g.inv_cell * (float)g.sub;
    const int ray0 = (blockIdx.x * 4 + wave) * RPW;
    for (int rb = 0; rb < RPW; rb += kMarkRays) {
        float o[kMarkRays][3], d[kMarkRays][3], nr[kMarkRays], rg[kMarkRays];
#pragma unroll
        for (int u = 0; u < kMarkRays; ++u) {
            const int ray = min(ray0 + rb + u, R - 1);
            o[u][0] = ray_o[ray * 3]; o[u][1] = ray_o[ray * 3 + 1]; o[u][2] = ray_o[ray * 3 + 2];
            d[u][0] = ray_d[ray * 3]; d[u][1] = ray_d[ray * 3 + 1]; d[u][2] = ray_d[ray * 3 + 2];
            nr[u] = near[ray]; rg[u] = __fsub_rn(far[ray], nr[u]);
        }
#pragma unroll
        for (int ch = 0; ch < NCH; ++ch) {
            const int k = ch * 64 + lane;
            uint32_t word[kMarkRays];
            int bit[kMarkRays];
#pragma unroll
            for (int u = 0; u < kMarkRays; ++u) {
                bit[u] = -1; word[u] = 0u;
                if (k < S && rb + u < RPW && ray0 + rb + u < R) {
                    const float t = depth_at(nr[u], rg[u], k, S);
                    const float x = __fadd_rn(o[u][0], __fmul_rn(t, d[u][0])), y = __fadd_rn(o[u][1], __fmul_rn(t, d[u][1])),
                                z = __fadd_rn(o[u][2], __fmul_rn(t, d[u][2]));
                    float xs, ys, zs;
                    to_smpl_frame(x, y, z, Rg, Th, xs, ys, zs);
                    const int sx = (int)floorf((xs - g.ox) * fs), sy = (int)floorf((ys - g.oy) * fs), sz = (int)floorf((zs - g.oz) * fs);
                    const int cx = g.sub == 2 ? sx >> 1 : sx, cy = g.sub == 2 ? sy >> 1 : sy, cz = g.sub == 2 ? sz >> 1 : sz;
                    if (sx >= 0 && cx < g.nx && sy >= 0 && cy < g.ny && sz >= 0 && cz < g.nz) {
                        const int q = (sz * (g.ny * g.sub) + sy) * (g.nx * g.sub) + sx;
                        bit[u] = q & 31;
                        word[u] = near_mask[q >> 5];
                    }
                }
            }
#pragma unroll
            for (int u = 0; u < kMarkRays; ++u) {
                const int ray = ray0 + rb + u;
                const bool cand = bit[u] >= 0 && (((dbg & 2) || ((word[u] >> bit[u]) & 1u)) && !(dbg & 1));
                const unsigned long long cm = __ballot(cand);
                if (rb + u < RPW && ray < R && lane == 0) ray_mask[(size_t)ray * NCH + ch] = 0ull;
                if (cm) {
                    int base = 0;
                    if (lane == 0) base = atomicAdd(&s_n, __popcll(cm));
                    base = __shfl(base, 0);
                    if (cand) s_list[base + __popcll(cm & ((1ull << lane) - 1ull))] = ray * S + k;
                }
            }
        }
    }
    __syncthreads();
    const int n = s_n;
    if (threadIdx.x == 0) s_base = n ? atomicAdd(cand_count, n) : 0;
    __syncthreads();
    const int64_t gb = s_base;
    for (int i = threadIdx.x; i < n; i += 256)
        if (gb + i < list_cap) {
            const int idx = s_list[i];
            const int ray = idx / S, k = idx - ray * S;
            const float nr1 = near[ray], t = depth_at(nr1, __fsub_rn(far[ray], nr1), k, S);
            const float x = __fadd_rn(ray_o[ray * 3], __fmul_rn(t, ray_d[ray * 3])), y = __fadd_rn(ray_o[ray * 3 + 1], __fmul_rn(t, ray_d[ray * 3 + 1])),
                        z = __fadd_rn(ray_o[ray * 3 + 2], __fmul_rn(t, ray_d[ray * 3 + 2]));
            float xs, ys, zs;
            to_smpl_frame(x, y, z, Rg, Th, xs, ys, zs);
            cand_list[gb + i] = make_float4(xs, ys, zs, __int_as_float(idx));
        }
}

constexpr int kSearchU = 1;

template <int NCH>
__global__ void __launch_bounds__(256) cand_search_kernel(const float4* __restrict__ cand_list, int64_t list_cap,
                                                          const int32_t* __restrict__ cand_count, int S, const float* __restrict__ hdr,
                                                          const int32_t* __restrict__ cell_start, const float4* __restrict__ cell_pts,
                                                          unsigned long long* __restrict__ ray_mask, int32_t* __restrict__ dense_vid) {
    constexpr int U = kSearchU;
    __shared__ int s_seg[U][32][20];
    const int grp = threadIdx.x >> 3, sub = threadIdx.x & 7;
    const CellGrid g = load_grid(hdr);
    const int64_t n = min((int64_t)*cand_count, list_cap);
    const float r = 0.05f + 1e-4f * g.cell;
    const unsigned long long kInit = ((unsigned long long)__float_as_uint(kThresh2) << 32) | 0x7FFFFFFFull;
    float4 rec_next[U];
#pragma unroll
    for (int u = 0; u < U; ++u) {
        const int64_t ci = (int64_t)blockIdx.x * 32 * U + u * 32 + grp;
        rec_next[u] = cand_list[ci < n ? ci : 0];
    }
    for (int64_t c0 = (int64_t)blockIdx.x * 32 * U; c0 < n; c0 += (int64_t)gridDim.x * 32 * U) {
        bool live[U];
        int idx[U], ray[U], k[U];
        float xs[U], ys[U], zs[U];
#pragma unroll
        for (int u = 0; u < U; ++u) {
            const int64_t ci = c0 + u * 32 + grp;
            live[u] = ci < n;
            const float4 rec = rec_next[u];
            const int64_t cn = ci + (int64_t)gridDim.x * 32 * U;
            rec_next[u] = cand_list[cn < n ? cn : 0];
            xs[u] = rec.x; ys[u] = rec.y; zs[u] = rec.z;
            idx[u] = live[u] ? __float_as_int(rec.w) : 0;
            ray[u] = idx[u] / S; k[u] = idx[u] - ray[u] * S;
        }
#pragma unroll
        for (int u = 0; u < U; ++u) {
            const int cx = (int)floorf((xs[u] - g.ox) * g.inv_cell), cy = (int)floorf((ys[u] - g.oy) * g.inv_cell), cz = (int)floorf((zs[u] - g.oz) * g.inv_cell);
#pragma unroll
            for (int pass = 0; pass < 2; ++pass) {
                const int i = pass ? 8 : sub;
                if (pass && sub != 0) break;
                const int qz = cz + i / 3 - 1, qy = cy + i % 3 - 1;
                const float y0 = g.oy + qy * g.cell, z0 = g.oz + qz * g.cell;
                const float ey = fmaxf(fmaxf(y0 - ys[u], ys[u] - (y0 + g.cell)), 0.f), ez = fmaxf(fmaxf(z0 - zs[u], zs[u] - (z0 + g.cell)), 0.f);
                const float rem = r * r - (ey * ey + ez * ez);
                const bool ok = live[u] && qz >= 0 && qz < g.nz && qy >= 0 && qy < g.ny && rem > 0.f;
                const float rx = sqrtf(fmaxf(rem, 0.f)) + 1e-4f * g.cell;
                const int x0 = max(max((int)floorf((xs[u] - rx - g.ox) * g.inv_cell), cx - 1), 0);
                const int x1 = min(min((int)floorf((xs[u] + rx - g.ox) * g.inv_cell), cx + 1), g.nx - 1);
                const int row = ok ? (qz * g.ny + qy) * g.nx : 0;
                const int st = cell_start[row + (ok ? x0 : 0)];
                const int en = ok && x1 >= x0 ? cell_start[row + x1 + 1] : st;
                s_seg[u][grp][i] = st; s_seg[u][grp][9 + i] = en - st;
            }
        }
        __builtin_amdgcn_wave_barrier();
        int bs[U][9], cum[U][9], npts[U];
#pragma unroll
        for (int u = 0; u < U; ++u) {
            int run = 0;
#pragma unroll
            for (int i = 0; i < 9; ++i) { bs[u][i] = s_seg[u][grp][i]; run += s_seg[u][grp][9 + i]; cum[u][i] = run; }
            npts[u] = run;
        }
        __builtin_amdgcn_wave_barrier();
        unsigned long long key[U];
        int most = 0;
#pragma unroll
        for (int u = 0; u < U; ++u) { key[u] = kInit; most = max(most, npts[u]); }
        for (int base = 0; base < most; base += 8 * kMaxPtsUnroll) {
            float4 v[U][kMaxPtsUnroll];
#pragma unroll
            for (int u = 0; u < U; ++u)
#pragma unroll
                for (int w = 0; w < kMaxPtsUnroll; ++w) {
                    const int tt = base + w * 8 + sub;
                    int p = bs[u][0] + tt;
#pragma unroll
                    for (int i = 1; i < 9; ++i) p = (tt >= cum[u][i - 1]) ? bs[u][i] + (tt - cum[u][i - 1]) : p;
                    v[u][w] = cell_pts[tt < npts[u] ? p : 0];
                }
#pragma unroll
            for (int u = 0; u < U; ++u)
#pragma unroll
                for (int w = 0; w < kMaxPtsUnroll; ++w) {
                    const int tt = base + w * 8 + sub;
                    const float dd = dist2_exact(xs[u], ys[u], zs[u], v[u][w].x, v[u][w].y, v[u][w].z);
                    if (tt < npts[u] && dd < kThresh2) {
                        const unsigned long long cand = ((unsigned long long)__float_as_uint(dd) << 32) | (unsigned)__float_as_int(v[u][w].w);
                        key[u] = cand < key[u] ? cand : key[u];
                    }
                }
        }
#pragma unroll
        for (int u = 0; u < U; ++u) {
#pragma unroll
            for (int off = 4; off > 0; off >>= 1) {
                const unsigned lo = __shfl_xor((unsigned)key[u], off), hi = __shfl_xor((unsigned)(key[u] >> 32), off);
                const unsigned long long other = ((unsigned long long)hi << 32) | lo;
                key[u] = other < key[u] ? other : key[u];
            }
            if (live[u] && sub == 0 && (unsigned)(key[u] >> 32) < __float_as_uint(kThresh2)) {
                dense_vid[idx[u]] = (int)(key[u] & 0x7FFFFFFFull);
                atomicOr(&ray_mask[(size_t)ray[u] * NCH + (k[u] >> 6)], 1ull << (k[u] & 63));
            }
        }
    }
}

template <int NCH>
__global__ void __launch_bounds__(256) cand_search_lists_kernel(const float4* __restrict__ cand_list, int64_t list_cap,
                                                                const int32_t* __restrict__ cand_count, int S, const float* __restrict__ hdr,
                                                                const int2* __restrict__ near_hdr, const uint16_t* __restrict__ near_list,
                                                                const float4* __restrict__ cell_pts,
                                                                unsigned long long* __restrict__ ray_mask, int32_t* __restrict__ dense_vid) {
    const int grp = threadIdx.x >> 3, sub = threadIdx.x & 7;
    const CellGrid g = load_grid(hdr);
    const int snx = g.nx * g.sub, sny = g.ny * g.sub, snz = g.nz * g.sub;
    const float fs = g.inv_cell * (float)g.sub;
    const int64_t n = min((int64_t)*cand_count, list_cap);
    const unsigned long long kInit = ((unsigned long long)__float_as_uint(kThresh2) << 32) | 0x7FFFFFFFull;
    const int64_t stride = (int64_t)gridDim.x * 32;
    auto sub_cell = [&](const float4& rec) -> int {
        const int sx = (int)floorf((rec.x - g.ox) * fs), sy = (int)floorf((rec.y - g.oy) * fs), sz = (int)floorf((rec.z - g.oz) * fs);
        const bool in = sx >= 0 && sx < snx && sy >= 0 && sy < sny && sz >= 0 && sz < snz;
        return in ? (sz * sny + sy) * snx + sx : -1;
    };
    int64_t ci = (int64_t)blockIdx.x * 32 + grp;
    float4 rec = cand_list[ci < n ? ci : 0];
    float4 rec_next = cand_list[ci + stride < n ? ci + stride : 0];
    int q0 = sub_cell(rec);
    int2 h = near_hdr[ci < n && q0 >= 0 ? q0 : 0];
    for (; ci - grp < n; ci += stride) {
        const bool live = ci < n && sub_cell(rec) >= 0;
        const float xs = rec.x, ys = rec.y, zs = rec.z;
        const int idx = live ? __float_as_int(rec.w) : 0;
        const int st = h.x, cn = live ? h.y : 0;
        const int64_t cn1 = ci + stride, cn2 = ci + 2 * stride;
        rec = rec_next;
        const int qn = sub_cell(rec);
        h = near_hdr[cn1 < n && qn >= 0 ? qn : 0];
        rec_next = cand_list[cn2 < n ? cn2 : 0];
        unsigned long long key = kInit;
        for (int base = 0; base < cn; base += 32) {
            const int e = base + sub * 4;
            uint2 w = make_uint2(0u, 0u);
            if (e < cn) w = *reinterpret_cast<const uint2*>(near_list + st + e);
            const int id[4] = {(int)(w.x & 0xFFFFu), (int)(w.x >> 16), (int)(w.y & 0xFFFFu), (int)(w.y >> 16)};
            float4 v[4];
#pragma unroll
            for (int j = 0; j < 4; ++j) v[j] = cell_pts[e + j < cn ? id[j] : 0];
#pragma unroll
            for (int j = 0; j < 4; ++j) {
                const float dd = dist2_exact(xs, ys, zs, v[j].x, v[j].y, v[j].z);
                if (e + j < cn && dd < kThresh2) {
                    const unsigned long long cand = ((unsigned long long)__float_as_uint(dd) << 32) | (unsigned)__float_as_int(v[j].w);
                    key = cand < key ? cand : key;
                }
            }
        }
#pragma unroll
        for (int off = 4; off > 0; off >>= 1) {
            const unsigned lo = __shfl_xor((unsigned)key, off), hi = __shfl_xor((unsigned)(key >> 32), off);
            const unsigned long long other = ((unsigned long long)hi << 32) | lo;
            key = other < key ? other : key;
        }
        if (live && sub == 0 && (unsigned)(key >> 32) < __float_as_uint(kThresh2)) {
            const int ray = idx / S, k = idx - ray * S;
            dense_vid[idx] = (int)(key & 0x7FFFFFFFull);
            atomicOr(&ray_mask[(size_t)ray * NCH + (k >> 6)], 1ull << (k & 63));
        }
    }
}

template <int NCH, int WAVES>
__global__ void __launch_bounds__(256, WAVES) cand_search_lists2_kernel(const float4* __restrict__ cand_list, int64_t list_cap,
                                                                 const int32_t* __restrict__ cand_count, int S, const float* __restrict__ hdr,
                                                                 const int2* __restrict__ near_hdr, const uint16_t* __restrict__ near_list,
                                                                 const float4* __restrict__ cell_pts,
                                                                 unsigned long long* __restrict__ ray_mask, int32_t* __restrict__ dense_vid) {
    const int grp = threadIdx.x >> 3, sub = threadIdx.x & 7;
    const CellGrid g = load_grid(hdr);
    const int snx = g.nx * g.sub, sny = g.ny * g.sub, snz = g.nz * g.sub;
    const float fs = g.inv_cell * (float)g.sub;
    const int64_t n = min((int64_t)*cand_count, list_cap);
    const unsigned long long kInit = ((unsigned long long)__float_as_uint(kThresh2) << 32) | 0x7FFFFFFFull;
    const int64_t stride = (int64_t)gridDim.x * 32;
    auto sub_cell = [&](const float4& rec) -> int {
        const int sx = (int)floorf((rec.x - g.ox) * fs), sy = (int)floorf((rec.y - g.oy) * fs), sz = (int)floorf((rec.z - g.oz) * fs);
        const bool in = sx >= 0 && sx < snx && sy >= 0 && sy < sny && sz >= 0 && sz < snz;
        return in ? (sz * sny + sy) * snx + sx : -1;
    };
    auto entries = [&](int st, int cn, int e, uint2& a, uint2& b) {
        a = make_uint2(0u, 0u); b = make_uint2(0u, 0u);
        if (e < cn) a = *reinterpret_cast<const uint2*>(near_list + st + e);
        if (e + 4 < cn) b = *reinterpret_cast<const uint2*>(near_list + st + e + 4);
    };
    int64_t ci = (int64_t)blockIdx.x * 32 + grp;
    float4 r0 = cand_list[ci < n ? ci : 0];
    float4 r1 = cand_list[ci + stride < n ? ci + stride : 0];
    float4 r2 = cand_list[ci + 2 * stride < n ? ci + 2 * stride : 0];
    const int q0 = sub_cell(r0), q1 = sub_cell(r1);
    bool l0 = ci < n && q0 >= 0, l1 = ci + stride < n && q1 >= 0;
    int2 h0 = near_hdr[l0 ? q0 : 0], h1 = near_hdr[l1 ? q1 : 0];
    uint2 wa, wb;
    entries(h0.x, l0 ? h0.y : 0, sub * 8, wa, wb);
    for (; ci - grp < n; ci += stride) {
        const bool live = l0;
        const float xs = r0.x, ys = r0.y, zs = r0.z;
        const int idx = live ? __float_as_int(r0.w) : 0;
        const int st = h0.x, cn = live ? h0.y : 0;
        uint2 ca = wa, cb = wb;
        const int cn1 = l1 ? h1.y : 0;
        entries(h1.x, cn1, sub * 8, wa, wb);
        const int q2 = sub_cell(r2);
        const bool l2 = ci + 2 * stride < n && q2 >= 0;
        const int2 h2 = near_hdr[l2 ? q2 : 0];
        const float4 r3 = cand_list[ci + 3 * stride < n ? ci + 3 * stride : 0];
        unsigned long long key = kInit;
        for (int base = 0; base < cn; base += 64) {
            const int e = base + sub * 8;
            if (base > 0) entries(st, cn, e, ca, cb);
            const int id[8] = {(int)(ca.x & 0xFFFFu), (int)(ca.x >> 16), (int)(ca.y & 0xFFFFu), (int)(ca.y >> 16),
                               (int)(cb.x & 0xFFFFu), (int)(cb.x >> 16), (int)(cb.y & 0xFFFFu), (int)(cb.y >> 16)};
            float4 v[8];
#pragma unroll
            for (int j = 0; j < 8; ++j) v[j] = cell_pts[e + j < cn ? id[j] : 0];
#pragma unroll
            for (int j = 0; j < 8; ++j) {
                const float dd = dist2_exact(xs, ys, zs, v[j].x, v[j].y, v[j].z);
                if (e + j < cn && dd < kThresh2) {
                    const unsigned long long cand = ((unsigned long long)__float_as_uint(dd) << 32) | (unsigned)__float_as_int(v[j].w);
                    key = cand < key ? cand : key;
                }
            }
        }
#pragma unroll
        for (int off = 4; off > 0; off >>= 1) {
            const unsigned lo = __shfl_xor((unsigned)key, off), hi = __shfl_xor((unsigned)(key >> 32), off);
            const unsigned long long other = ((unsigned long long)hi << 32) | lo;
            key = other < key ? other : key;
        }
        if (live && sub == 0 && (unsigned)(key >> 32) < __float_as_uint(kThresh2)) {
            const int ray = idx / S, k = idx - ray * S;
            dense_vid[idx] = (int)(key & 0x7FFFFFFFull);
            atomicOr(&ray_mask[(size_t)ray * NCH + (k >> 6)], 1ull << (k & 63));
        }
        r0 = r1; r1 = r2; r2 = r3; l0 = l1; l1 = l2; h0 = h1; h1 = h2;
    }
}

template <int NCH>
__global__ void __launch_bounds__(1024) scan_chunk_mask_kernel(const uint64_t* __restrict__ ray_mask, int R, int32_t* __restrict__ cnt,
                                                               int32_t* __restrict__ base, int32_t* __restrict__ chunk_sum) {
    __shared__ int s[1024];
    const int i = blockIdx.x * 1024 + threadIdx.x;
    int v = 0;
    if (i < R) {
#pragma unroll
        for (int ch = 0; ch < NCH; ++ch) v += __popcll(ray_mask[(size_t)i * NCH + ch]);
        cnt[i] = v;
    }
    s[threadIdx.x] = v;
    __syncthreads();
    for (int off = 1; off < 1024; off <<= 1) {
        int a = threadIdx.x >= off ? s[threadIdx.x - off] : 0;
        __syncthreads();
        s[threadIdx.x] += a;
        __syncthreads();
    }
    if (i < R) base[i] = s[threadIdx.x] - v;
    if (threadIdx.x == 1023) chunk_sum[blockIdx.x] = s[1023];
}

__global__ void __launch_bounds__(1024) scan_chunk_kernel(const int32_t* __restrict__ cnt, int R,
                                                          int32_t* __restrict__ base, int32_t* __restrict__ chunk_sum) {
    __shared__ int s[1024];
    const int i = blockIdx.x * 1024 + threadIdx.x;
    int v = i < R ? cnt[i] : 0;
    s[threadIdx.x] = v;
    __syncthreads();
    for (int off = 1; off < 1024; off <<= 1) {
        int a = threadIdx.x >= off ? s[threadIdx.x - off] : 0;
        __syncthreads();
        s[threadIdx.x] += a;
        __syncthreads();
    }
    if (i < R) base[i] = s[threadIdx.x] - v;
    if (threadIdx.x == 1023) chunk_sum[blockIdx.x] = s[1023];
}

__global__ void __launch_bounds__(1024) scan_top_kernel(int32_t* __restrict__ chunk_sum, int n_chunks,
                                                        int32_t* __restrict__ counters) {
    __shared__ int s[1024];
    int carry = 0;
    for (int b0 = 0; b0 < n_chunks; b0 += 1024) {
        int i = b0 + threadIdx.x;
        int v = i < n_chunks ? chunk_sum[i] : 0;
        s[threadIdx.x] = v;
        __syncthreads();
        for (int off = 1; off < 1024; off <<= 1) {
            int a = threadIdx.x >= off ? s[threadIdx.x - off] : 0;
            __syncthreads();
            s[threadIdx.x] += a;
            __syncthreads();
        }
        if (i < n_chunks) chunk_sum[i] = carry + s[threadIdx.x] - v;
        int tot = s[1023];
        __syncthreads();
        carry += tot;
    }
    if (threadIdx.x == 0) counters[0] = carry;
}

__global__ void __launch_bounds__(256) depth_minmax_kernel(const float* __restrict__ near, const float* __restrict__ far,
                                                           int R, int S, int32_t* __restrict__ counters) {
    __shared__ float smn[4], smx[4];
    float mn = 3.0e38f, mx = -3.0e38f;
    for (int r = blockIdx.x * 256 + threadIdx.x; r < R; r += gridDim.x * 256) {
        float nr = near[r], range = __fsub_rn(far[r], nr);
        float t0 = depth_at(nr, range, 0, S), t1 = depth_at(nr, range, S - 1, S);
        mn = fminf(mn, fminf(t0, t1)); mx = fmaxf(mx, fmaxf(t0, t1));
    }
    for (int off = 32; off > 0; off >>= 1) { mn = fminf(mn, __shfl_xor(mn, off)); mx = fmaxf(mx, __shfl_xor(mx, off)); }
    if ((threadIdx.x & 63) == 0) { smn[threadIdx.x >> 6] = mn; smx[threadIdx.x >> 6] = mx; }
    __syncthreads();
    if (threadIdx.x == 0) {
        for (int w = 1; w < 4; ++w) { mn = fminf(mn, smn[w]); mx = fmaxf(mx, smx[w]); }
        atomicMin(&counters[1], f2ord(fminf(mn, smn[0])));
        atomicMax(&counters[2], f2ord(fmaxf(mx, smx[0])));
    }
}

__global__ void init_counters_kernel(int32_t* counters, int32_t* cand_count, int32_t* sticky) {
    if (sticky) { sticky[0] = max(sticky[0], counters[0]); sticky[1] |= counters[3]; sticky[2] += 1; }
    counters[0] = 0; counters[1] = 0x7FFFFFFF; counters[2] = (int32_t)0x80000000; counters[3] = 0;
    *cand_count = 0;
}

template <int NCH>
__global__ void __launch_bounds__(256) compact_kernel(const float* __restrict__ ray_o, const float* __restrict__ ray_d,
                                                      const float* __restrict__ near, const float* __restrict__ far,
                                                      int R, int S, const float* __restrict__ Rg, const float* __restrict__ Th,
                                                      const int32_t* __restrict__ ray_base_local,
                                                      const int32_t* __restrict__ chunk_off, const uint64_t* __restrict__ ray_mask,
                                                      const int32_t* __restrict__ dense_vid, int64_t capacity,
                                                      int32_t* __restrict__ ray_base, int32_t* __restrict__ cs_idx,
                                                      int32_t* __restrict__ cs_vid, float4* __restrict__ cs_xs,
                                                      const float4* __restrict__ cell_pts_unused) {
    const int lane = threadIdx.x & 63;
    const int ray = blockIdx.x * 4 + (threadIdx.x >> 6);
    if (ray >= R) return;
    int base = ray_base_local[ray] + chunk_off[ray >> 10];
    if (lane == 0) ray_base[ray] = base;
    uint64_t any = 0;
#pragma unroll
    for (int ch = 0; ch < NCH; ++ch) any |= ray_mask[(size_t)ray * NCH + ch];
    if (any == 0) return;
    const float o0 = ray_o[ray * 3], o1 = ray_o[ray * 3 + 1], o2 = ray_o[ray * 3 + 2];
    const float d0 = ray_d[ray * 3], d1 = ray_d[ray * 3 + 1], d2 = ray_d[ray * 3 + 2];
    const float nr = near[ray], range = __fsub_rn(far[ray], nr);
#pragma unroll
    for (int ch = 0; ch < NCH; ++ch) {
        const uint64_t m = ray_mask[(size_t)ray * NCH + ch];
        const int k = ch * 64 + lane;
        if ((m >> lane) & 1ull) {
            int rank = __popcll(m & ((1ull << lane) - 1ull));
            int64_t c = (int64_t)base + rank;
            if (c < capacity) {
                float t = depth_at(nr, range, k, S);
                float x = __fadd_rn(o0, __fmul_rn(t, d0)), y = __fadd_rn(o1, __fmul_rn(t, d1)), z = __fadd_rn(o2, __fmul_rn(t, d2));
                float xs, ys, zs;
                to_smpl_frame(x, y, z, Rg, Th, xs, ys, zs);
                int vid = dense_vid[(size_t)ray * S + k];
                cs_idx[c] = ray * S + k;
                cs_vid[c] = vid;
                cs_xs[c] = make_float4(xs, ys, zs, 0.f);
            }
        }
        base += __popcll(m);
    }
}

template <int NCH>
__global__ void __launch_bounds__(256) compact_rays_kernel(const float* __restrict__ ray_o, const float* __restrict__ ray_d,
                                                           const float* __restrict__ near, const float* __restrict__ far,
                                                           int R, int S, const float* __restrict__ Rg, const float* __restrict__ Th,
                                                           const int32_t* __restrict__ ray_base_local,
                                                           const int32_t* __restrict__ chunk_off, const uint64_t* __restrict__ ray_mask,
                                                           const int32_t* __restrict__ dense_vid, int64_t capacity,
                                                           int32_t* __restrict__ ray_base, int32_t* __restrict__ cs_idx,
                                                           int32_t* __restrict__ cs_vid, float4* __restrict__ cs_xs) {
    const int lane = threadIdx.x & 63;
    const int ray0 = (blockIdx.x * 4 + (threadIdx.x >> 6)) * 64;
    if (ray0 >= R) return;
    const int my = ray0 + lane;
    int my_base = 0;
    uint64_t my_any = 0;
    if (my < R) {
        my_base = ray_base_local[my] + chunk_off[my >> 10];
        ray_base[my] = my_base;
#pragma unroll
        for (int ch = 0; ch < NCH; ++ch) my_any |= ray_mask[(size_t)my * NCH + ch];
    }
    uint64_t hits = __ballot(my_any != 0);
    while (hits) {
        const int rl = __ffsll((unsigned long long)hits) - 1;
        hits &= hits - 1;
        const int ray = ray0 + rl;
        int base = __shfl(my_base, rl);
        const float o0 = ray_o[ray * 3], o1 = ray_o[ray * 3 + 1], o2 = ray_o[ray * 3 + 2];
        const float d0 = ray_d[ray * 3], d1 = ray_d[ray * 3 + 1], d2 = ray_d[ray * 3 + 2];
        const float nr = near[ray], range = __fsub_rn(far[ray], nr);
#pragma unroll
        for (int ch = 0; ch < NCH; ++ch) {
            const uint64_t m = ray_mask[(size_t)ray * NCH + ch];
            const int k = ch * 64 + lane;
            if ((m >> lane) & 1ull) {
                const int rank = __popcll(m & ((1ull << lane) - 1ull));
                const int64_t c = (int64_t)base + rank;
                if (c < capacity) {
                    const float t = depth_at(nr, range, k, S);
                    const float x = __fadd_rn(o0, __fmul_rn(t, d0)), y = __fadd_rn(o1, __fmul_rn(t, d1)), z = __fadd_rn(o2, __fmul_rn(t, d2));
                    float xs, ys, zs;
                    to_smpl_frame(x, y, z, Rg, Th, xs, ys, zs);
                    cs_idx[c] = ray * S + k;
                    cs_vid[c] = dense_vid[(size_t)ray * S + k];
                    cs_xs[c] = make_float4(xs, ys, zs, 0.f);
                }
            }
            base += __popcll(m);
        }
    }
}

template <int NCH>
__global__ void __launch_bounds__(256) compact_quad_kernel(const float* __restrict__ ray_o, const float* __restrict__ ray_d,
                                                           const float* __restrict__ near, const float* __restrict__ far,
                                                           int R, int S, const float* __restrict__ Rg, const float* __restrict__ Th,
                                                           const int32_t* __restrict__ ray_base_local,
                                                           const int32_t* __restrict__ chunk_off, const uint64_t* __restrict__ ray_mask,
                                                           const int32_t* __restrict__ dense_vid, int64_t capacity,
                                                           int32_t* __restrict__ ray_base, int32_t* __restrict__ cs_idx,
                                                           int32_t* __restrict__ cs_vid, float4* __restrict__ cs_xs) {
    static_assert(NCH == 1 || NCH == 2 || NCH == 4, "a lane's samples must not straddle a mask word");
    constexpr int SPL = 4 * NCH;
    const int lane = threadIdx.x & 63, sub = lane & 15;
    const int ray = (blockIdx.x * 4 + (threadIdx.x >> 6)) * 4 + (lane >> 4);
    if (ray >= R) return;
    const int base = ray_base_local[ray] + chunk_off[ray >> 10];
    if (sub == 0) ray_base[ray] = base;
    const int k0 = sub * SPL, word = k0 >> 6, shift = k0 & 63;
    int below = 0;
    uint64_t mine = 0;
#pragma unroll
    for (int ch = 0; ch < NCH; ++ch) {
        const uint64_t m = ray_mask[(size_t)ray * NCH + ch];
        below += ch < word ? __popcll(m) : (ch == word ? __popcll(m & ((1ull << shift) - 1ull)) : 0);
        mine = ch == word ? m : mine;
    }
    const unsigned bits = (unsigned)(mine >> shift) & ((1u << SPL) - 1u);
    if (bits == 0) return;
    const float o0 = ray_o[ray * 3], o1 = ray_o[ray * 3 + 1], o2 = ray_o[ray * 3 + 2];
    const float d0 = ray_d[ray * 3], d1 = ray_d[ray * 3 + 1], d2 = ray_d[ray * 3 + 2];
    const float nr = near[ray], range = __fsub_rn(far[ray], nr);
    int vid[SPL];
#pragma unroll
    for (int j = 0; j < SPL; ++j) vid[j] = ((bits >> j) & 1u) ? dense_vid[(size_t)ray * S + k0 + j] : 0;
#pragma unroll
    for (int j = 0; j < SPL; ++j) {
        if (!((bits >> j) & 1u)) continue;
        const int k = k0 + j;
        const int64_t c = (int64_t)base + below + __popc(bits & ((1u << j) - 1u));
        if (c < capacity) {
            const float t = depth_at(nr, range, k, S);
            const float x = __fadd_rn(o0, __fmul_rn(t, d0)), y = __fadd_rn(o1, __fmul_rn(t, d1)), z = __fadd_rn(o2, __fmul_rn(t, d2));
            float xs, ys, zs;
            to_smpl_frame(x, y, z, Rg, Th, xs, ys, zs);
            cs_idx[c] = ray * S + k;
            cs_vid[c] = vid[j];
            cs_xs[c] = make_float4(xs, ys, zs, 0.f);
        }
    }
}

__global__ void __launch_bounds__(256) warp_geom_kernel(const int32_t* __restrict__ counters, const int32_t* __restrict__ cs_idx,
                                                        const int32_t* __restrict__ cs_vid, const float4* __restrict__ cs_xs,
                                                        const float* __restrict__ ray_d, int S, const float* __restrict__ Rg,
                                                        const float* __restrict__ T2C, const float* __restrict__ C2S,
                                                        const float* __restrict__ t_verts, const float* __restrict__ thdr,
                                                        const int32_t* __restrict__ tcell_start,
                                                        const float4* __restrict__ tcell_pts, int64_t capacity,
                                                        float* __restrict__ geom, int32_t* __restrict__ cs_tvid) {
    const int64_t nv = min((int64_t)counters[0], capacity);
    const CellGrid g = load_grid(thdr);
    for (int64_t c = (int64_t)blockIdx.x * 256 + threadIdx.x; c < nv; c += (int64_t)gridDim.x * 256) {
    const int ray = cs_idx[c] / S;
    const int vid = cs_vid[c];
    const float4 xs = cs_xs[c];
    float vx, vy, vz;
    const float* rd = ray_d + (size_t)ray * 3;
    rot_only(rd[0], rd[1], rd[2], Rg, vx, vy, vz);
    const float4* P4 = reinterpret_cast<const float4*>(T2C) + (size_t)vid * 3;
    const float4 pa = P4[0], pb = P4[1], pc = P4[2];
    const float P[12] = {pa.x, pa.y, pa.z, pa.w, pb.x, pb.y, pb.z, pb.w, pc.x, pc.y, pc.z, pc.w};
    float xc = P[0] * xs.x + P[1] * xs.y + P[2] * xs.z + P[9];
    float yc = P[3] * xs.x + P[4] * xs.y + P[5] * xs.z + P[10];
    float zc = P[6] * xs.x + P[7] * xs.y + P[8] * xs.z + P[11];
    float ux = P[0] * vx + P[1] * vy + P[2] * vz;
    float uy = P[3] * vx + P[4] * vy + P[5] * vz;
    float uz = P[6] * vx + P[7] * vy + P[8] * vz;
    float best = dist2_exact(xc, yc, zc, t_verts[vid * 3], t_verts[vid * 3 + 1], t_verts[vid * 3 + 2]);
    int bid = vid;
    float r = sqrtf(best) * 1.00001f + 1e-6f;
    nn_search_batched(g, tcell_start, tcell_pts, xc, yc, zc, r, best, bid);
    const float4* L4 = reinterpret_cast<const float4*>(C2S) + (size_t)bid * 3;
    const float4 la = L4[0], lb = L4[1], lc = L4[2];
    const float L[12] = {la.x, la.y, la.z, la.w, lb.x, lb.y, lb.z, lb.w, lc.x, lc.y, lc.z, lc.w};
    float hx = L[0] * xc + L[1] * yc + L[2] * zc + L[9];
    float hy = L[3] * xc + L[4] * yc + L[5] * zc + L[10];
    float hz = L[6] * xc + L[7] * yc + L[8] * zc + L[11];
    float iz = hz + 1e-5f;
    float4* o = reinterpret_cast<float4*>(geom + c * 8);
    o[0] = make_float4(xc, yc, zc, ux); o[1] = make_float4(uy, uz, hx / iz, hy / iz);
    cs_tvid[c] = bid;
    }
}

}

int sherf_sample_mask_nn_impl(const float* ray_o, const float* ray_d, const float* near, const float* far, int R, int S, const float* Rg, const float* Th,
                              const float* grid_hdr, const int32_t* cell_start, const float* cell_pts, const uint32_t* near_mask, int64_t capacity,
                              int32_t* counters, int32_t* ray_base, int32_t* ray_cnt, int32_t* cs_idx, int32_t* cs_vid, float* cs_xs, int32_t* dense_vid,
                              uint64_t* ray_mask, int32_t* scan_ws, const int32_t* near_hdr, const uint16_t* near_list, sherf_stream_t stream, int32_t* sticky);
int sherf_warp_geom_impl(const int32_t* counters, const int32_t* cs_idx, const int32_t* cs_vid, const float* cs_xs, const float* ray_d, int S, const float* Rg,
                         const float* T2C, const float* C2S, const float* t_verts, const float* tgrid_hdr, const int32_t* tcell_start, const float* tcell_pts,
                         int64_t capacity, float* geom, int32_t* cs_tvid, sherf_stream_t stream);

extern "C" int sherf_build_cells(const float* verts, int n, const float* R, const float* Th, float cell_size,
                                 float* grid_hdr, int32_t* cell_start, float* cell_pts, int32_t* scratch,
                                 uint32_t* near_mask, sherf_stream_t stream) {
    SHERF_CHECK_ARG(verts && grid_hdr && cell_start && cell_pts && scratch);
    SHERF_CHECK_ARG(n > 0 && n <= 65535 && cell_size > 0.f);
    SHERF_CHECK_ARG((R == nullptr) == (Th == nullptr));
    SHERF_CHECK_ARG(near_mask == nullptr || cell_size >= kShellRadius);
    hipLaunchKernelGGL(build_cells_kernel, dim3(1), dim3(1024), 0, as_stream(stream), verts, n, R, Th, cell_size,
                       grid_hdr, cell_start, reinterpret_cast<float4*>(cell_pts), scratch, near_mask);
    if (near_mask) {
        (void)hipMemsetAsync(near_mask, 0, 32768 * sizeof(uint32_t), as_stream(stream));
        hipLaunchKernelGGL(near_mask_kernel, dim3(cdiv(n, 256)), dim3(256), 16384 * sizeof(uint32_t), as_stream(stream),
                           reinterpret_cast<const float*>(scratch), n, grid_hdr, cell_size, near_mask);
    }
    SHERF_LAUNCH_CHECK();
}

extern "C" int sherf_build_cells2(const float* verts_a, const float* R_a, const float* Th_a, const float* verts_b, int n,
                                  float cell_size, float* grid_hdr, int32_t* cell_start, float* cell_pts, int32_t* scratch,
                                  uint32_t* near_mask, sherf_stream_t stream) {
    SHERF_CHECK_ARG(verts_a && R_a && Th_a && verts_b && grid_hdr && cell_start && cell_pts && scratch);
    SHERF_CHECK_ARG(n > 0 && n <= 65535 && cell_size >= kShellRadius);
    hipLaunchKernelGGL(build_cells2_kernel, dim3(2), dim3(1024), 0, as_stream(stream), verts_a, R_a, Th_a, verts_b, n, cell_size,
                       grid_hdr, cell_start, reinterpret_cast<float4*>(cell_pts), scratch, near_mask);
    if (near_mask) {
        (void)hipMemsetAsync(near_mask, 0, 32768 * sizeof(uint32_t), as_stream(stream));
        hipLaunchKernelGGL(near_mask_kernel, dim3(cdiv(n, 256)), dim3(256), 16384 * sizeof(uint32_t), as_stream(stream),
                           reinterpret_cast<const float*>(scratch), n, grid_hdr, cell_size, near_mask);
    }
    SHERF_LAUNCH_CHECK();
}

extern "C" int sherf_build_near_lists(const float* grid_hdr, const float* cell_pts, int n, float radius, int32_t* near_hdr,
                                      uint16_t* near_list, int64_t list_cap, uint32_t* near_mask, sherf_stream_t stream) {
    SHERF_CHECK_ARG(grid_hdr && cell_pts && near_hdr && near_list);
    SHERF_CHECK_ARG(n > 0 && n <= 65535 && radius >= kShellRadius && list_cap >= (int64_t)125 * n + 3 * SHERF_NEAR_SUBCELLS);
    hipStream_t st = as_stream(stream);
    int2* nh = reinterpret_cast<int2*>(near_hdr);
    int32_t* cursor = near_hdr + 2 * SHERF_NEAR_SUBCELLS;
    (void)hipMemsetAsync(near_hdr, 0, 2 * (size_t)SHERF_NEAR_SUBCELLS * sizeof(int32_t), st);
    const float4* pts = reinterpret_cast<const float4*>(cell_pts);
    hipLaunchKernelGGL(near_lists_pairs_kernel<false>, dim3(cdiv(n * 32, 256)), dim3(256), 0, st, pts, n, grid_hdr, radius, nh, near_list, list_cap, cursor);
    hipLaunchKernelGGL(near_lists_alloc_kernel, dim3(SHERF_NEAR_SUBCELLS / 256), dim3(256), 0, st, grid_hdr, nh, cursor, list_cap, near_mask);
    hipLaunchKernelGGL(near_lists_pairs_kernel<true>, dim3(cdiv(n * 32, 256)), dim3(256), 0, st, pts, n, grid_hdr, radius, nh, near_list, list_cap, static_cast<int32_t*>(nullptr));
    SHERF_LAUNCH_CHECK();
}

extern "C" int sherf_sample_mask_nn(const float* ray_o, const float* ray_d, const float* near, const float* far,
                                       int R, int S, const float* Rg, const float* Th, const float* grid_hdr,
                                       const int32_t* cell_start, const float* cell_pts, const uint32_t* near_mask, int64_t capacity,
                                    int32_t* counters, int32_t* ray_base, int32_t* ray_cnt, int32_t* cs_idx,
                                       int32_t* cs_vid, float* cs_xs, int32_t* dense_vid, uint64_t* ray_mask,
                                       int32_t* scan_ws, const int32_t* near_hdr, const uint16_t* near_list, sherf_stream_t stream) {
    return sherf_sample_mask_nn_impl(ray_o, ray_d, near, far, R, S, Rg, Th, grid_hdr, cell_start, cell_pts, near_mask, capacity, counters, ray_base, ray_cnt,
                                     cs_idx, cs_vid, cs_xs, dense_vid, ray_mask, scan_ws, near_hdr, near_list, stream, nullptr);
}

template <int N>
static void search_and_scan(hipStream_t st, int R, int S, const float* grid_hdr, const int32_t* cell_start, const float4* cp, const float4* cand_list, int64_t list_cap,
                            const int32_t* cand_count, const int32_t* near_hdr, const uint16_t* near_list, int32_t* dense_vid, uint64_t* ray_mask, int32_t* ray_cnt,
                            int32_t* base_local, int32_t* chunk_sum) {
    unsigned long long* rm = reinterpret_cast<unsigned long long*>(ray_mask);
    const bool lists = near_hdr && near_list && !(g_sherf_debug & 16384);
    const int search_wgs = ((g_sherf_debug >> 20) & 15) ? ((g_sherf_debug >> 20) & 15) : 6;
    const bool tight = (sherf_experiment() & 32768) != 0;
    const bool deep = (sherf_experiment() & 16384) != 0;
    if (lists && deep && tight)
        hipLaunchKernelGGL((cand_search_lists2_kernel<N, 6>), dim3(search_wgs * n_cus()), dim3(256), 0, st, cand_list, list_cap, cand_count, S,
                           grid_hdr, reinterpret_cast<const int2*>(near_hdr), near_list, cp, rm, dense_vid);
    else if (lists && deep)
        hipLaunchKernelGGL((cand_search_lists2_kernel<N, 5>), dim3(min(search_wgs, 5) * n_cus()), dim3(256), 0, st, cand_list, list_cap, cand_count, S,
                           grid_hdr, reinterpret_cast<const int2*>(near_hdr), near_list, cp, rm, dense_vid);
    else if (lists)
        hipLaunchKernelGGL(cand_search_lists_kernel<N>, dim3(search_wgs * n_cus()), dim3(256), 0, st, cand_list, list_cap, cand_count, S,
                           grid_hdr, reinterpret_cast<const int2*>(near_hdr), near_list, cp, rm, dense_vid);
    else
        hipLaunchKernelGGL(cand_search_kernel<N>, dim3(8 * n_cus()), dim3(256), 0, st, cand_list, list_cap, cand_count, S,
                           grid_hdr, cell_start, cp, rm, dense_vid);
    hipLaunchKernelGGL(scan_chunk_mask_kernel<N>, dim3(cdiv(R, 1024)), dim3(1024), 0, st, ray_mask, R, ray_cnt, base_local, chunk_sum);
}

int sherf_points_begin_impl(int32_t* counters, int32_t* scan_ws, int rows, int32_t* sticky, sherf_stream_t stream) {
    hipLaunchKernelGGL(init_counters_kernel, dim3(1), dim3(1), 0, as_stream(stream), counters, sherf_scan_ws(scan_ws, rows).cand_count, sticky);
    SHERF_LAUNCH_CHECK();
}
int sherf_points_search_impl(int rows, const float* grid_hdr, const int32_t* cell_start, const float* cell_pts, const float* cand_list, int64_t list_cap,
                             int32_t* counters, int32_t* ray_cnt, int32_t* dense_vid, uint64_t* ray_mask, int32_t* scan_ws, const int32_t* near_hdr,
                             const uint16_t* near_list, sherf_stream_t stream) {
    const SherfScanWs w = sherf_scan_ws(scan_ws, rows);
    search_and_scan<1>(as_stream(stream), rows, 64, grid_hdr, cell_start, reinterpret_cast<const float4*>(cell_pts), reinterpret_cast<const float4*>(cand_list),
                       list_cap, w.cand_count, near_hdr, near_list, dense_vid, ray_mask, ray_cnt, w.base_local, w.chunk_sum);
    hipLaunchKernelGGL(scan_top_kernel, dim3(1), dim3(1024), 0, as_stream(stream), w.chunk_sum, cdiv(rows, 1024), counters);
    SHERF_LAUNCH_CHECK();
}

int sherf_sample_mask_nn_impl(const float* ray_o, const float* ray_d, const float* near, const float* far,
                              int R, int S, const float* Rg, const float* Th, const float* grid_hdr,
                              const int32_t* cell_start, const float* cell_pts, const uint32_t* near_mask, int64_t capacity,
                              int32_t* counters, int32_t* ray_base, int32_t* ray_cnt, int32_t* cs_idx,
                              int32_t* cs_vid, float* cs_xs, int32_t* dense_vid, uint64_t* ray_mask,
                              int32_t* scan_ws, const int32_t* near_hdr, const uint16_t* near_list, sherf_stream_t stream, int32_t* sticky) {
    SHERF_CHECK_ARG(ray_o && ray_d && near && far && Rg && Th && grid_hdr && cell_start && cell_pts && near_mask);
    SHERF_CHECK_ARG(counters && ray_base && ray_cnt && cs_idx && cs_vid && cs_xs && dense_vid && ray_mask && scan_ws);
    SHERF_CHECK_ARG(R > 0 && S >= 2 && S <= 256 && (int64_t)R * S < 2147483647LL && capacity > 0 && (near_hdr == nullptr) == (near_list == nullptr));
    hipStream_t st = as_stream(stream);
    const int nch = (S + 63) / 64;
    const int n_chunks = cdiv(R, 1024);
    const SherfScanWs sw = sherf_scan_ws(scan_ws, R);
    int32_t* base_local = sw.base_local;
    int32_t* chunk_sum = sw.chunk_sum;
    const float4* cp = reinterpret_cast<const float4*>(cell_pts);
    int32_t* cand_count = sw.cand_count;
    hipLaunchKernelGGL(init_counters_kernel, dim3(1), dim3(1), 0, st, counters, cand_count, sticky);
    hipLaunchKernelGGL(depth_minmax_kernel, dim3(min(256, cdiv(R, 256))), dim3(256), 0, st, near, far, R, S, counters);
    const bool two_pass = !(g_sherf_debug & 512) && capacity >= (int64_t)R * S;
    if (two_pass) {
        float4* cand_list = reinterpret_cast<float4*>(cs_xs);
        const int64_t list_cap = capacity;
#define SHERF_TWO_PASS(N)                                                                                                          \
        hipLaunchKernelGGL(cand_mark_kernel<N>, dim3(cdiv(R, 4 * (16 / N))), dim3(256), 0, st, ray_o, ray_d, near, far, R, S, Rg, Th,    \
                           grid_hdr, near_mask, cand_list, list_cap, cand_count, ray_mask, g_sherf_debug);                         \
        search_and_scan<N>(st, R, S, grid_hdr, cell_start, cp, cand_list, list_cap, cand_count, near_hdr, near_list, dense_vid, ray_mask, ray_cnt, base_local, \
                           chunk_sum)
        if (nch == 1) { SHERF_TWO_PASS(1); } else if (nch == 2) { SHERF_TWO_PASS(2); } else if (nch == 3) { SHERF_TWO_PASS(3); } else { SHERF_TWO_PASS(4); }
#undef SHERF_TWO_PASS
    } else {
    constexpr int nn_pad = 10 * 1024;
#define SHERF_SAMPLE_LAUNCH(N)                                                                                        \
    hipLaunchKernelGGL(sample_nn_kernel<N>, dim3(cdiv(R, 4)), dim3(256), nn_pad, st, ray_o, ray_d, near, far, R, S, Rg, Th, \
                       grid_hdr, cell_start, cp, near_mask, ray_cnt, ray_mask, dense_vid, g_sherf_debug)
    if (nch == 1) SHERF_SAMPLE_LAUNCH(1); else if (nch == 2) SHERF_SAMPLE_LAUNCH(2);
    else if (nch == 3) SHERF_SAMPLE_LAUNCH(3); else SHERF_SAMPLE_LAUNCH(4);
    hipLaunchKernelGGL(scan_chunk_kernel, dim3(n_chunks), dim3(1024), 0, st, ray_cnt, R, base_local, chunk_sum);
    }
    hipLaunchKernelGGL(scan_top_kernel, dim3(1), dim3(1024), 0, st, chunk_sum, n_chunks, counters);
#define SHERF_COMPACT_LAUNCH(N)                                                                                        \
    hipLaunchKernelGGL(compact_kernel<N>, dim3(cdiv(R, 4)), dim3(256), 0, st, ray_o, ray_d, near, far, R, S, Rg, Th,   \
                       base_local, chunk_sum, ray_mask, dense_vid, capacity, ray_base, cs_idx, cs_vid,                 \
                       reinterpret_cast<float4*>(cs_xs), cp)
#define SHERF_COMPACT_RAYS_LAUNCH(N)                                                                                   \
    hipLaunchKernelGGL(compact_rays_kernel<N>, dim3(cdiv(R, 256)), dim3(256), 0, st, ray_o, ray_d, near, far, R, S, Rg, Th, \
                       base_local, chunk_sum, ray_mask, dense_vid, capacity, ray_base, cs_idx, cs_vid,                 \
                       reinterpret_cast<float4*>(cs_xs))
#define SHERF_COMPACT_QUAD_LAUNCH(N)                                                                                   \
    hipLaunchKernelGGL(compact_quad_kernel<N>, dim3(cdiv(R, 16)), dim3(256), 0, st, ray_o, ray_d, near, far, R, S, Rg, Th, \
                       base_local, chunk_sum, ray_mask, dense_vid, capacity, ray_base, cs_idx, cs_vid,                 \
                       reinterpret_cast<float4*>(cs_xs))
    if ((sherf_experiment() & 8192) && nch != 3) {
        if (nch == 1) SHERF_COMPACT_QUAD_LAUNCH(1); else if (nch == 2) SHERF_COMPACT_QUAD_LAUNCH(2); else SHERF_COMPACT_QUAD_LAUNCH(4);
    } else
    if (sherf_experiment() & 2048) {
        if (nch == 1) SHERF_COMPACT_RAYS_LAUNCH(1); else if (nch == 2) SHERF_COMPACT_RAYS_LAUNCH(2);
        else if (nch == 3) SHERF_COMPACT_RAYS_LAUNCH(3); else SHERF_COMPACT_RAYS_LAUNCH(4);
    } else {
    if (nch == 1) SHERF_COMPACT_LAUNCH(1); else if (nch == 2) SHERF_COMPACT_LAUNCH(2);
    else if (nch == 3) SHERF_COMPACT_LAUNCH(3); else SHERF_COMPACT_LAUNCH(4);
    }
    SHERF_LAUNCH_CHECK();
}

extern "C" int sherf_warp_geom(const int32_t* counters, const int32_t* cs_idx, const int32_t* cs_vid,
                               const float* cs_xs, const float* ray_d, int S, const float* Rg, const float* T2C,
                               const float* C2S, const float* t_verts, const float* tgrid_hdr,
                               const int32_t* tcell_start, const float* tcell_pts, int64_t capacity, float* geom,
                               int32_t* cs_tvid, sherf_stream_t stream) {
    SHERF_CHECK_ARG(S >= 2);
    return sherf_warp_geom_impl(counters, cs_idx, cs_vid, cs_xs, ray_d, S, Rg, T2C, C2S, t_verts, tgrid_hdr, tcell_start, tcell_pts, capacity, geom, cs_tvid, stream);
}

int sherf_warp_geom_impl(const int32_t* counters, const int32_t* cs_idx, const int32_t* cs_vid, const float* cs_xs, const float* ray_d, int S, const float* Rg,
                         const float* T2C, const float* C2S, const float* t_verts, const float* tgrid_hdr, const int32_t* tcell_start, const float* tcell_pts,
                         int64_t capacity, float* geom, int32_t* cs_tvid, sherf_stream_t stream) {
    SHERF_CHECK_ARG(counters && cs_idx && cs_vid && cs_xs && ray_d && Rg && T2C && C2S && t_verts && tgrid_hdr &&
                    tcell_start && tcell_pts && geom && cs_tvid);
    SHERF_CHECK_ARG(S >= 1 && capacity > 0);
    const int warp_wgs = (sherf_experiment() >> 16) & 15;
    const int warp_grid = warp_wgs ? min(warp_wgs * n_cus(), cdiv(capacity, 256)) : min(8192, cdiv(capacity, 256));
    hipLaunchKernelGGL(warp_geom_kernel, dim3(warp_grid), dim3(256), 0, as_stream(stream), counters, cs_idx,
                       cs_vid, reinterpret_cast<const float4*>(cs_xs), ray_d, S, Rg, T2C, C2S, t_verts, tgrid_hdr,
                       tcell_start, reinterpret_cast<const float4*>(tcell_pts), capacity, geom, cs_tvid);
    SHERF_LAUNCH_CHECK();
}
```

sherf_amd/renderer.py:

```python
import ctypes as _ct
import os
import pickle

import numpy as np
import torch
import torch.nn as nn

from . import _lib, mlp_pack, osg_pack
from .ray_marcher import MipRayMarcher2
from .voxel import SparseConvNet, SparseConvTensor, pack_conv_weights

MLP_PRECISIONS = mlp_pack.PRECISIONS

V = 6890
NEAR_SUBCELLS = 524288


def compute_normal(vertices, faces):
    tris = vertices[:, faces]
    n = torch.cross(tris[:, :, 1] - tris[:, :, 0], tris[:, :, 2] - tris[:, :, 0], dim=-1)
    n = n / torch.sqrt((n ** 2).sum(-1, keepdim=True)).clamp_min(1e-8)
    norm = torch.zeros_like(vertices)
    nf = faces.shape[0]
    ar = torch.arange(nf, device=faces.device)
    for c in range(3):
        last = torch.full((vertices.shape[1],), -1, dtype=torch.long, device=faces.device).scatter_reduce_(0, faces[:, c], ar, reduce='amax')
        has = last >= 0
        norm[:, has] = norm[:, has] + n[:, last[has]]
    return norm / torch.sqrt((norm ** 2).sum(-1, keepdim=True)).clamp_min(1e-8)


class PositionalEncoding(nn.Module):

    def __init__(self, num_freqs=6, d_in=3, freq_factor=None, include_input=True):
        super().__init__()
        self.num_freqs, self.d_in, self.include_input = num_freqs, d_in, include_input
        self.freqs = 2.0 ** torch.linspace(0.0, num_freqs - 1, steps=num_freqs)
        self.d_out = num_freqs * 2 * d_in + (d_in if include_input else 0)
        self.register_buffer('_freqs', torch.repeat_interleave(self.freqs, 2).view(1, -1, 1))
        ph = torch.zeros(2 * num_freqs)
        ph[1::2] = np.pi * 0.5
        self.register_buffer('_phases', ph.view(1, -1, 1))

    def forward(self, x):
        e = torch.sin(torch.addcmul(self._phases, x.unsqueeze(1).repeat(1, self.num_freqs * 2, 1), self._freqs))
        e = e.view(x.shape[0], self.num_freqs * 2 * self.d_in)
        return torch.cat((x, e), dim=-1) if self.include_input else e


class _Fn(nn.Module):
    def __init__(self, fn, norm_dim=None):
        super().__init__()
        if norm_dim is not None:
            self.norm = nn.LayerNorm(norm_dim)
        self.fn = fn


class _Attention(nn.Module):
    def __init__(self, dim, heads, dim_head):
        super().__init__()
        self.heads, self.scale = heads, dim_head ** -0.5
        self.to_qkv = nn.Linear(dim, heads * dim_head * 3, bias=False)
        self.to_out = nn.Sequential(nn.Linear(heads * dim_head, dim), nn.Dropout(0.0))


class _FeedForward(nn.Module):
    def __init__(self, dim, hidden):
        super().__init__()
        self.net = nn.Sequential(nn.Linear(dim, hidden), nn.GELU(), nn.Dropout(0.0), nn.Linear(hidden, dim), nn.Dropout(0.0))


class Transformer(nn.Module):

    def __init__(self, dim=32, depth=1, heads=3, dim_head=16, mlp_dim=32):
        super().__init__()
        assert (dim, depth, heads, dim_head, mlp_dim) == (32, 1, 3, 16, 32), 'fused kernel is specialised to the reference shape'
        self.layers = nn.ModuleList([nn.ModuleList([_Fn(_Fn(_Attention(dim, heads, dim_head), dim)),
                                                    _Fn(_Fn(_FeedForward(dim, mlp_dim), dim))])])


def read_pickle(pkl_path):
    with open(pkl_path, 'rb') as f:
        u = pickle._Unpickler(f)
        u.encoding = 'latin1'
        return u.load()


def SMPL_to_tensor(params, device):
    out = {}
    for k in ('v_template', 'shapedirs', 'weights', 'posedirs'):
        out[k] = torch.tensor(np.asarray(params[k]).astype(float), dtype=torch.float32, device=device)
    J = params['J_regressor']
    J = J.toarray() if hasattr(J, 'toarray') else np.asarray(J)
    out['J_regressor'] = torch.tensor(J.astype(float), dtype=torch.float32, device=device)
    out['kintree_table'] = torch.tensor(np.asarray(params['kintree_table']).astype(float), dtype=torch.long, device=device)
    out['f'] = torch.tensor(np.asarray(params['f']).astype(float), dtype=torch.long, device=device)
    out['J_template'] = (out['J_regressor'] @ out['v_template']).contiguous()
    out['J_shapedirs'] = torch.einsum('jv,vcb->jcb', out['J_regressor'], out['shapedirs']).contiguous()
    par = out['kintree_table'][0].clone()
    par[0] = 0
    out['parents_i32'] = par.to(torch.int32).contiguous()
    out['posedirs_flat'] = out['posedirs'].reshape(V * 3, 207).contiguous()
    out['weights'] = out['weights'].contiguous()
    out['shapedirs'] = out['shapedirs'].contiguous()
    f = np.asarray(params['f']).astype(np.int64)
    last = np.full((3, out['v_template'].shape[0]), -1, np.int32)
    for c in range(3):
        np.maximum.at(last[c], f[:, c], np.arange(f.shape[0], dtype=np.int32))
    out['f_i32'] = torch.tensor(f.astype(np.int32), dtype=torch.int32, device=device).contiguous()
    out['last_face_i32'] = torch.tensor(last, dtype=torch.int32, device=device).contiguous()
    return out


def fast_params(module, out=None, buffers=False):
    out = [] if out is None else out
    for p in module._parameters.values():
        if p is not None:
            out.append(p)
    if buffers:
        for b in module._buffers.values():
            if b is not None:
                out.append(b)
    for c in module._modules.values():
        if c is not None:
            fast_params(c, out, buffers)
    return out


def state_key(tensors):
    return tuple([(t.data_ptr(), t._version) for t in tensors])


class _Workspace:
    def __init__(self):
        self.key = None
        self.t = {}
        self.vox = None
        self.bn = {}
        self.desc = None
        self.stacked = None
        self.tok_cap = 0
        self.obs_key = None
        self.obs_levels = None
        self.obs_refs = None

    def frame(self, R, S, cap, dev):
        key = (R, S, cap, str(dev))
        if self.key == key:
            return self.t
        i32 = dict(dtype=torch.int32, device=dev)
        f32 = dict(dtype=torch.float32, device=dev)
        nch = (S + 63) // 64
        t = dict(
            counters=torch.zeros(8, **i32), ray_base=torch.zeros(R, **i32), ray_cnt=torch.zeros(R, **i32),
            cs_idx=torch.zeros(cap, **i32), cs_vid=torch.zeros(cap, **i32),
            cs_xs=torch.zeros(cap, 4, **f32), dense_vid=torch.zeros(R * S, **i32),
            ray_mask=torch.zeros(R * nch, dtype=torch.int64, device=dev), scan_ws=torch.zeros(R + R // 1024 + 2, **i32),
            A=torch.zeros(3, 24, 12, **f32), posefeat=torch.zeros(3, 207, **f32), PO=torch.zeros(3, V, 3, **f32),
            SO=torch.zeros(3, V, 3, **f32), T2C=torch.zeros(V, 12, **f32), C2S=torch.zeros(V, 12, **f32),
            grid_hdr=torch.zeros(2, 12, **f32), cell_start=torch.zeros(2, 64 * 64 * 64 + 1, **i32),
            cell_pts=torch.zeros(2, V, 4, **f32), cell_scratch=torch.zeros(2 * 5 * V, **i32),
            near_mask=torch.zeros(32768, **i32),
            near_hdr=torch.zeros(2 * NEAR_SUBCELLS + 2, **i32),
            near_list=torch.zeros(125 * V + 3 * NEAR_SUBCELLS, dtype=torch.int16, device=dev),
        )
        self.key, self.t = key, t
        self.desc = None
        self.tok_cap = 0
        self.obs_key = None
        self.tokens(min(cap, 256), dev)
        return t

    def tokens(self, tok_cap, dev):
        if tok_cap == self.tok_cap:
            return
        f32 = dict(dtype=torch.float32, device=dev)
        tiles = (tok_cap + 31) // 32 + 8
        for k in ('geom', 'tokens', 'extras', 'sample_out', 'cs_tvid', 'zfrag', 'pefrag'):
            self.t.pop(k, None)
        self.t.update(geom=torch.zeros(tok_cap, 8, **f32), tokens=torch.zeros(tiles * 3 * 8 * 32 * 4, **f32),
                      extras=torch.zeros(tiles * 12 * 32, **f32), sample_out=torch.zeros(tok_cap, 4, **f32),
                      cs_tvid=torch.zeros(tok_cap, dtype=torch.int32, device=dev))
        self.tok_cap = tok_cap
        if self.desc is not None:
            fr = self.desc[2]
            for k in ('geom', 'tokens', 'extras', 'sample_out', 'cs_tvid'):
                setattr(fr, k, _lib.addr(self.t[k]))
            fr.pefrag = None

    def pefrag(self, dev):
        z = self.t.get('pefrag')
        words = ((self.tok_cap + 31) // 32 + 8) * 7 * 64 * 4
        if z is None or z.numel() != words or z.device != torch.device(dev):
            z = self.t['pefrag'] = torch.zeros(words, dtype=torch.int32, device=dev)
        return z

    def nbytes(self):
        seen, n = set(), 0
        for v in list(self.t.values()) + list(self.bn.values()):
            if torch.is_tensor(v) and v.untyped_storage().data_ptr() not in seen:
                seen.add(v.untyped_storage().data_ptr()); n += v.untyped_storage().nbytes()
        return n

    STATIC_FIELDS = ('A', 'posefeat', 'PO', 'SO', 'T2C', 'C2S', 'grid_hdr', 'cell_start', 'cell_pts', 'cell_scratch', 'near_mask',
                     'counters', 'ray_base', 'ray_cnt', 'cs_idx', 'cs_vid', 'cs_xs', 'dense_vid', 'ray_mask', 'scan_ws', 'geom',
                     'cs_tvid', 'tokens', 'extras', 'sample_out')

    def descriptor(self, smpl):
        d = self.desc
        if d is not None and d[0] is self.t and d[1] is smpl:
            return d[2]
        A = _lib.addr
        fr = _lib.Frame()
        for k in self.STATIC_FIELDS:
            setattr(fr, k, A(self.t[k]))
        fr.sticky = A(self.t['counters']) + 16
        fr.J_template, fr.J_shapedirs, fr.parents = A(smpl['J_template']), A(smpl['J_shapedirs']), A(smpl['parents_i32'])
        fr.posedirs, fr.shapedirs, fr.weights = A(smpl['posedirs_flat']), A(smpl['shapedirs']), A(smpl['weights'])
        self.desc = (self.t, smpl, fr, dict(near_hdr=A(self.t['near_hdr']), near_list=A(self.t['near_list']), near_cap=self.t['near_list'].numel()))
        return fr

    def zfrag(self, cap, prec_name, dev):
        words = ((cap + 31) // 32 + 8) * (2048 if prec_name == 'f16x3' else 1024)
        z = self.t.get('zfrag')
        if z is None or z.numel() < words or z.device != torch.device(dev):
            z = self.t['zfrag'] = torch.empty(words, dtype=torch.int32, device=dev)
        return z

    def voxel_levels(self, shapes, N, dev):
        key = (tuple(shapes), N, str(dev))
        if self.vox is not None and self.vox[0] == key:
            return self.vox[1]
        i32 = dict(dtype=torch.int32, device=dev)
        dims = []
        for li, (D, H, W) in enumerate(shapes):
            nvox = D * H * W
            dims.append((nvox, (nvox + 31) // 32, N if li == 0 else min(nvox, 8 * N)))
        n_acc = 16 * 8 * 2 * 96 * 2
        zsize = sum(d[1] for d in dims) + N + N * 32 * 2 + 2 + n_acc + 2
        zsize = (zsize + 3) // 4 * 4
        zero_region = torch.zeros(zsize, **i32)
        L, off = [], 0
        for li, (nvox, nwords, cap) in enumerate(dims):
            lv = dict(bitmap=zero_region[off:off + nwords], prefix=torch.zeros(nwords, **i32), keys=torch.zeros(cap, **i32),
                      n_rows=torch.zeros(1, **i32), chunk_ws=torch.zeros(nwords // 1024 + 2, **i32), wp=torch.zeros(nwords, 2, **i32),
                      nwords=nwords, cap=cap)
            off += nwords
            L.append(lv)
        L[0]['mult'] = zero_region[off:off + N]; off += N
        off += off % 2
        L[0]['acc_fix'] = zero_region[off:off + N * 64].view(torch.int64)
        off += N * 64
        L[0]['bn_acc'] = zero_region[off:off + n_acc].view(torch.int64)
        L[0]['g0'] = torch.zeros(N, 32, device=dev)
        L[0]['n_total'] = torch.full((1,), N, **i32)
        self.vox = (key, (L, zero_region))
        return self.vox[1]

    def _cached(self, kind, idx, shape, dev, dtype=torch.float32):
        k = (kind, idx, tuple(shape), str(dev))
        if k not in self.bn:
            self.bn[k] = torch.zeros(*shape, device=dev, dtype=dtype)
        return self.bn[k]

    def bn_stats(self, idx, C, dev):
        return self._cached('stats', idx, (2, C), dev)

    def bn_param(self, idx, C, dev):
        return self._cached('bnp', idx, (3, C), dev)

    def layer_out(self, idx, cap, C, dev):
        return self._cached('out', idx, (cap, C), dev)

    def fold_out(self, idx, cap, dev):
        return self._cached('fold', idx, (cap, 96), dev)

    def table(self, kind, shape, dev):
        return self._cached(kind, 0, shape, dev)


_SIDE_STREAMS = {}


class ImportanceRenderer(nn.Module):
    enable_osg_autograd = False
    reuse_observation = False

    def __init__(self, use_1d_feature=True, use_2d_feature=True, use_3d_feature=True, use_trans=False, use_NeRF_decoder=False,
                 smpl=None, smpl_path=os.path.join('assets', 'SMPL_NEUTRAL.pkl'), mlp_precision='auto', table_precision='auto', encoder_precision='auto'):
        super().__init__()
        self.use_1d_feature, self.use_2d_feature, self.use_3d_feature = use_1d_feature, use_2d_feature, use_3d_feature
        self.use_trans, self.use_NeRF_decoder = use_trans, use_NeRF_decoder
        self.ray_marcher = MipRayMarcher2()
        self.encoder_3d = SparseConvNet(num_layers=4)
        self.conv1d_projection = nn.Conv1d(192, 96, 1)
        if use_1d_feature and use_2d_feature and use_3d_feature:
            self.conv1d_reprojection = nn.Conv1d(96, 32, 1)
        elif (use_1d_feature and use_2d_feature) or (use_1d_feature and use_3d_feature) or (use_3d_feature and use_2d_feature):
            self.conv1d_reprojection = nn.Conv1d(64, 32, 1)
        self.transformer = None if not use_trans else Transformer(32)
        self.rgb_enc = PositionalEncoding(num_freqs=5)
        self.pos_enc = PositionalEncoding(num_freqs=6)
        self.view_enc = PositionalEncoding(num_freqs=4)
        self.mlp_precision = mlp_precision
        self.table_precision = table_precision
        self.encoder_precision = encoder_precision
        self.gather_split = os.environ.get('SHERF_GATHER_SPLIT', '0') == '1'
        self.gather_branchless = {'0': False, '1': True, '128': '128'}[os.environ.get('SHERF_GATHER_BRANCHLESS', '0')]
        self.exact_grids = os.environ.get('SHERF_EXACT_GRIDS', '0') == '1'
        self.mlp_split = {'': None, '0': False, '1': True}[os.environ.get('SHERF_MLP_SPLIT', '')]
        self.mlp_form = os.environ.get('SHERF_MLP_FORM', 'auto')
        self.mlp_parts = int(os.environ.get('SHERF_MLP_PARTS', '0'))
        self.token_capacity = os.environ.get('SHERF_TOKEN_CAPACITY', 'auto')
        self.main_after_layer = int(os.environ.get('SHERF_MAIN_AFTER_LAYER', '-1'))
        self.aux_stream = os.environ.get('SHERF_AUX_STREAM', '1') == '1'
        self._smpl_src = smpl
        self._smpl_path = smpl_path
        self._smpl_dev = None
        self._ws = {}
        self._wcache = None
        self.last = None

    def __getstate__(self):
        s = self.__dict__.copy()
        for k in ('_smpl_dev', '_ws', '_wcache', 'last', '_flags', '_frame_memo', '_pack_flag_pending', '_qws', 'last_query'):
            s[k] = None
        s['_ws'] = None
        return s

    def __setstate__(self, s):
        self.__dict__.update(s)
        self._ws = {}

    def _workspace(self, dev, main=None):
        sid = (main or torch.cuda.current_stream(dev)).cuda_stream
        if self._ws is None or not isinstance(self._ws, dict):
            self._ws = {}
        key = (str(dev), sid)
        w = self._ws.pop(key, None)
        if w is None:
            w = _Workspace()
            while len(self._ws) >= self.MAX_WORKSPACES:
                old_key = next(iter(self._ws))
                if dev.type == 'cuda' and torch.cuda.is_available():
                    torch.cuda.synchronize(dev)
                del self._ws[old_key]
        self._ws[key] = w
        return w

    MAX_WORKSPACES = 8

    def _side(self, dev, idx=0):
        key = (dev, torch.cuda.current_stream(dev).cuda_stream)
        cur = _SIDE_STREAMS.pop(key, None)
        if cur is None:
            xp = int(os.environ.get('SHERF_EXPERIMENT_STREAMS', '0'))
            cur = [torch.cuda.Stream(device=dev, priority=0 if xp & 2 else -1) for _ in range(4 if xp & 4 else 2)][-2:]
            if xp & 1:
                cur.reverse()
            while len(_SIDE_STREAMS) >= 4 * self.MAX_WORKSPACES:
                old = _SIDE_STREAMS.pop(next(iter(_SIDE_STREAMS)))
                for st in old:
                    st.synchronize()
        _SIDE_STREAMS[key] = cur
        return cur[idx]

    @property
    def SMPL_NEUTRAL(self):
        return self._smpl(torch.device('cuda', torch.cuda.current_device()))

    def _smpl(self, device):
        if self._smpl_dev is None or self._smpl_dev['v_template'].device != device:
            src = self._smpl_src if self._smpl_src is not None else read_pickle(self._smpl_path)
            self._smpl_dev = SMPL_to_tensor(src, device)
        return self._smpl_dev

    def projection(self, query_pts, R, T, K, face=None):
        R, T, K, q = R.float(), T.float(), K.float(), query_pts.float()
        xyz = torch.einsum('bvij,bnj->bvni', R, q) + T[:, :, None, :, 0]
        mask = None
        if face is not None:
            normal = compute_normal(q, face)
            ncam = torch.einsum('bvij,bnj->bvni', R, normal)
            mask = ((ncam * xyz).sum(-1) < 0).squeeze(1)
        h = torch.einsum('bvij,bvnj->bvni', K, xyz)
        xy = h[..., :2] / (h[..., 2:] + 1e-5)
        return (xy, mask) if face is not None else xy

    def t2c_table(self, params, t_params):
        dev = params['poses'].device
        smpl = self._smpl(dev)
        f32 = lambda t: t.detach().float().contiguous()
        poses = torch.stack([f32(params['poses']).view(72), f32(t_params['poses']).view(72)])
        shapes = torch.stack([f32(params['shapes']).view(10), f32(t_params['shapes']).view(10)])
        A = torch.zeros(2, 24, 12, device=dev); pf = torch.zeros(2, 207, device=dev)
        PO = torch.zeros(2, V, 3, device=dev); SO = torch.zeros(2, V, 3, device=dev); T2C = torch.zeros(V, 12, device=dev)
        P, st = _lib.ptr, _lib.stream()
        _lib.call('sherf_smpl_bones', P(poses), P(shapes), 2, P(smpl['J_template']), P(smpl['J_shapedirs']), P(smpl['parents_i32']),
                  P(A), P(pf), st)
        _lib.call('sherf_smpl_offsets', P(smpl['posedirs_flat']), P(smpl['shapedirs']), P(pf), P(shapes), 2, P(PO), P(SO), st)
        _lib.call('sherf_smpl_t2c_table', P(smpl['weights']), P(A[0]), P(A[1]), P(PO[0]), P(SO[0]), P(PO[1]), P(T2C), st)
        return T2C

    def coarse_deform_target2c(self, params, vertices, t_params, query_pts, query_viewdirs=None):
        if query_pts.shape[0] != 1:
            raise RuntimeError('per-GPU batch must be 1, as in the reference (renderer.py:567)')
        f32 = lambda t: t.detach().float().contiguous()
        T2C = self.t2c_table(params, t_params)
        xs = torch.matmul(f32(vertices).view(V, 3) - f32(params['Th']).view(1, 3), f32(params['R']).view(3, 3))
        q = f32(query_pts).view(-1, 3)
        if q.shape[0] == V and torch.equal(q, xs):
            vid = torch.arange(V, device=q.device)
        else:
            vid = torch.cat([(((c[:, None, 0] - xs[None, :, 0]) ** 2 + (c[:, None, 1] - xs[None, :, 1]) ** 2)
                              + (c[:, None, 2] - xs[None, :, 2]) ** 2).argmin(1) for c in q.split(8192)])
        Pm, t = T2C[vid, :9].view(-1, 3, 3), T2C[vid, 9:]
        can = (torch.einsum('nij,nj->ni', Pm, q) + t).view(1, -1, 3)
        if query_viewdirs is not None:
            return can, torch.einsum('nij,nj->ni', Pm, f32(query_viewdirs).view(-1, 3)).view(1, -1, 3)
        return can

    def check_finite(self):
        return self.last is None or (int(self.last['ws']['counters'][3]) & 3) == 0

    AUTO_RECHECK_EVERY = int(os.environ.get('SHERF_AUTO_RECHECK', '256'))

    def _auto_state_key(self):
        enc = self.encoder_3d
        pk = enc.__dict__.get('_key_memo') or state_key(fast_params(enc))
        mode = (self.__dict__.get('_clamp_mode', 'relu'),)
        if enc.training:
            return (True,) + mode + pk
        return (False,) + mode + pk + state_key([b for m in enc.modules() for b in m._buffers.values() if b is not None])

    _AUTO_STATE = ('auto', 'auto_key', 'auto_frames', 'auto_tripped')

    def _auto_for_mode(self, wc):
        mode, held = self.__dict__.get('_clamp_mode', 'relu'), wc.get('auto_mode', 'relu')
        if mode != held:
            per = wc.setdefault('auto_per_mode', {})
            per[held] = {k: wc.get(k) for k in self._AUTO_STATE}
            wc.update(per.get(mode) or dict.fromkeys(self._AUTO_STATE))
            wc['auto_mode'] = mode

    WATCH_RING = int(os.environ.get('SHERF_WATCH_RING', '4'))
    WATCH_EVERY = int(os.environ.get('SHERF_WATCH_EVERY', '8'))

    def _note_counters(self, st, c, ws=None):
        flags, nv = c[3] | (c[5] if len(c) > 5 else 0), max(c[0], c[4] if len(c) > 4 else 0)
        if flags & 1:
            st['tripped'] += 1
        if flags & 2:
            st['overflowed'] = st.get('overflowed', 0) + 1
        st['nv_seen'] = max(st.get('nv_seen', 0), nv)
        if ws is not None and len(c) > 5 and (c[5] or c[4]):
            ws['counters'][4:7].zero_()

    def _flag_watch(self, ws, dev):
        st = self.__dict__.setdefault('_flags', dict(ring=[], tripped=0))
        seen = st.setdefault('watched', {})
        seen[ws['counters'].data_ptr()] = ws['counters']
        while len(seen) > 16:
            seen.pop(next(iter(seen)))
        if dev.type != 'cuda' or getattr(ws['counters'], 'device', dev).type != 'cuda':
            self._note_counters(st, ws['counters'].tolist(), ws)
            return st
        ring = st['ring']
        for other in ring:
            if other['busy'] and other['ev'].query():
                other['busy'] = False
                self._note_counters(st, other['host'].tolist())
        since, key = st.setdefault('since', {}), ws['counters'].data_ptr()
        every = 1 if isinstance(self._ws, dict) and len(self._ws) > 1 else self.WATCH_EVERY
        since[key] = since.get(key, every - 1) + 1
        if since[key] < every:
            return st
        since[key] = 0
        while len(since) > 16:
            since.pop(next(iter(since)))
        if len(ring) < self.WATCH_RING:
            ring.append(dict(host=torch.zeros(8, dtype=torch.int32).pin_memory(), ev=torch.cuda.Event(), busy=False))
            st['next'] = len(ring) - 1
        slot = ring[st.get('next', 0) % len(ring)]
        st['next'] = (st.get('next', 0) + 1) % self.WATCH_RING
        if slot['busy']:
            slot['ev'].synchronize()
            self._note_counters(st, slot['host'].tolist())
        slot['host'].copy_(ws['counters'], non_blocking=True)
        ws['counters'][4:7].zero_()
        slot['ev'].record(torch.cuda.current_stream(dev))
        slot['busy'] = True
        return st

    def poll_flags(self, wait=False):
        st = self.__dict__.setdefault('_flags', dict(ring=[], tripped=0))
        for slot in st['ring']:
            if slot['busy'] and (wait or slot['ev'].query()):
                slot['ev'].synchronize()
                slot['busy'] = False
                self._note_counters(st, slot['host'].tolist())
        if wait:
            for w in list((st.get('watched') or {}).values()):
                if w.device.type == 'cuda':
                    torch.cuda.synchronize(w.device)
                self._note_counters(st, w.tolist(), dict(counters=w))
        return st

    TOKEN_HEADROOM = 1.5
    TOKEN_GROW_AT = 0.8

    TOKEN_GRANULE = 8192

    def _round_tokens(self, n, cap):
        g = self.TOKEN_GRANULE
        return int(min(cap, max(g, (int(n) + g - 1) // g * g)))

    def _token_capacity(self, opts, wsp, cap, dev, probe):
        want = opts.get('token_capacity', getattr(self, 'token_capacity', 'auto'))
        if want in ('worst', None) or (torch.is_grad_enabled() and getattr(self, 'enable_autograd', False)) or getattr(self, '_in_autograd', False):
# ... 708 lines not shown
```

Baseline: 162.8 million.

## Bin candidate samples by near-subcell and search per cell with shared point lists

Adds a cell-binned candidate search path. The mark kernel counts candidates per subcell with atomic ranks. An alloc kernel prefix-sums the counts into offsets and 64-wide work items, a place kernel scatters candidates into cell-sorted order, and a new search kernel processes each item so that one wave shares a single subcell's near-point list. This aims to cut redundant per-candidate loads of neighbour lists and improve coherence in the nearest-neighbour search, at the cost of extra kernels, atomics, a new workspace, and recomputing sample positions in the place pass.

New measurement: 170.2 million, median of 6. 4.5% higher.

```diff
diff --git a/include/sherf_hip.h b/include/sherf_hip.h
--- a/include/sherf_hip.h
+++ b/include/sherf_hip.h
@@ -52,6 +52,14 @@
                          int64_t capacity, int32_t* counters, int32_t* ray_base, int32_t* ray_cnt, int32_t* cs_idx,
                          int32_t* cs_vid, float* cs_xs, int32_t* dense_vid, uint64_t* ray_mask,
                          int32_t* scan_ws, const int32_t* near_hdr, const uint16_t* near_list, sherf_stream_t stream);
+#define SHERF_CELL_WS_INTS(R, S) (4 * (int64_t)SHERF_NEAR_SUBCELLS + 6 + 2 * ((int64_t)(R) * (S) / 64))
+int sherf_sample_mask_nn_ws(const float* ray_o, const float* ray_d, const float* near, const float* far,
+                            int R, int S, const float* Rg, const float* Th, const float* grid_hdr,
+                            const int32_t* cell_start, const float* cell_pts, const uint32_t* near_mask,
+                            int64_t capacity, int32_t* counters, int32_t* ray_base, int32_t* ray_cnt, int32_t* cs_idx,
+                            int32_t* cs_vid, float* cs_xs, int32_t* dense_vid, uint64_t* ray_mask,
+                            int32_t* scan_ws, const int32_t* near_hdr, const uint16_t* near_list, int32_t* cell_ws, int64_t cell_ws_len,
+                            sherf_stream_t stream);
 
 int sherf_warp_geom(const int32_t* counters, const int32_t* cs_idx, const int32_t* cs_vid, const float* cs_xs,
                     const float* ray_d, int S, const float* Rg, const float* T2C, const float* C2S,
@@ -237,6 +245,7 @@
     int64_t tok_capacity;
     void* pefrag;
     int32_t* sticky;
+    int32_t* cell_ws; int64_t cell_ws_len;
 } sherf_frame;
 int sherf_render_frame(const sherf_frame* frame, int phase, sherf_vox_level* levels_out_host, sherf_stream_t stream_main,
                        sherf_stream_t stream_side, sherf_stream_t stream_aux);
diff --git a/sherf_amd/_lib.py b/sherf_amd/_lib.py
--- a/sherf_amd/_lib.py
+++ b/sherf_amd/_lib.py
@@ -62,6 +62,8 @@
     f.append(('tok_capacity', _i64))
     P('pefrag')
     P('sticky')
+    P('cell_ws')
+    f.append(('cell_ws_len', _i64))
     return f
 
 
diff --git a/sherf_amd/csrc/frame.hip b/sherf_amd/csrc/frame.hip
--- a/sherf_amd/csrc/frame.hip
+++ b/sherf_amd/csrc/frame.hip
@@ -13,7 +13,7 @@
                               const float* grid_hdr, const int32_t* cell_start, const float* cell_pts, const uint32_t* near_mask, int64_t capacity,
                               int32_t* counters, int32_t* ray_base, int32_t* ray_cnt, int32_t* cs_idx, int32_t* cs_vid, float* cs_xs, int32_t* dense_vid,
                               uint64_t* ray_mask, int32_t* scan_ws, const int32_t* near_hdr, const uint16_t* near_list, sherf_stream_t stream,
-                              int32_t* sticky);
+                              int32_t* sticky, int32_t* cell_ws, int64_t cell_ws_len);
 int sherf_warp_geom_impl(const int32_t* counters, const int32_t* cs_idx, const int32_t* cs_vid, const float* cs_xs, const float* ray_d, int S, const float* Rg,
                          const float* T2C, const float* C2S, const float* t_verts, const float* tgrid_hdr, const int32_t* tcell_start, const float* tcell_pts,
                          int64_t capacity, float* geom, int32_t* cs_tvid, sherf_stream_t stream);
@@ -132,7 +132,8 @@
             SHERF_RUN(sherf_build_near_lists(f->grid_hdr, f->cell_pts, SHERF_V, 0.05f, f->near_hdr, f->near_list, f->near_list_cap, f->near_mask, stream_main));
         SHERF_RUN(sherf_sample_mask_nn_impl(f->ray_o, f->ray_d, f->near, f->far, f->R, f->S, f->Rg, f->Th, f->grid_hdr, f->cell_start,
                                        f->cell_pts, f->near_mask, f->capacity, f->counters, f->ray_base, f->ray_cnt, f->cs_idx,
-                                       f->cs_vid, f->cs_xs, f->dense_vid, f->ray_mask, f->scan_ws, f->near_hdr, f->near_list, stream_main, f->sticky));
+                                       f->cs_vid, f->cs_xs, f->dense_vid, f->ray_mask, f->scan_ws, f->near_hdr, f->near_list, stream_main, f->sticky,
+                                       f->cell_ws, f->cell_ws_len));
         return SHERF_OK;
     }
     const int64_t tok_cap = (f->tok_capacity > 0 && f->tok_capacity < f->capacity) ? f->tok_capacity : f->capacity;
@@ -241,7 +242,8 @@
         else
         SHERF_RUN(sherf_sample_mask_nn_impl(f->ray_o, f->ray_d, f->near, f->far, f->R, f->S, f->Rg, f->Th, f->grid_hdr, f->cell_start,
                                        f->cell_pts, f->near_mask, f->capacity, f->counters, f->ray_base, f->ray_cnt, f->cs_idx,
-                                       f->cs_vid, f->cs_xs, f->dense_vid, f->ray_mask, f->scan_ws, f->near_hdr, f->near_list, stream_main, f->sticky));
+                                       f->cs_vid, f->cs_xs, f->dense_vid, f->ray_mask, f->scan_ws, f->near_hdr, f->near_list, stream_main, f->sticky,
+                                       f->cell_ws, f->cell_ws_len));
         SHERF_CAP_TRACE("sampler queued");
         if (f->flags & SHERF_FRAME_REPORT_COUNT) {
             const int slot = d.rep_next;
diff --git a/sherf_amd/csrc/sample.hip b/sherf_amd/csrc/sample.hip
--- a/sherf_amd/csrc/sample.hip
+++ b/sherf_amd/csrc/sample.hip
@@ -4,6 +4,8 @@
 
 constexpr float kThresh2 = (float)(0.05 * 0.05);
 constexpr float kShellRadius = SHERF_SHELL_RADIUS;
+constexpr int kDebugSearchByCandidate = 1 << 28;
+constexpr int kCellSearchWgs = 4;
 
 constexpr int kLdsCells = 24576;
 
@@ -360,14 +362,16 @@
 }
 
 constexpr int kMarkRays = 4;
-
-template <int NCH>
+constexpr int kCellStage = 2048;
+
+template <int NCH, bool CELLS>
 __global__ void __launch_bounds__(256) cand_mark_kernel(const float* __restrict__ ray_o, const float* __restrict__ ray_d,
                                                         const float* __restrict__ near, const float* __restrict__ far, int R, int S,
                                                         const float* __restrict__ Rg, const float* __restrict__ Th,
                                                         const float* __restrict__ hdr, const uint32_t* __restrict__ near_mask,
                                                         float4* __restrict__ cand_list, int64_t list_cap, int32_t* __restrict__ cand_count,
-                                                        uint64_t* __restrict__ ray_mask, int dbg) {
+                                                        uint64_t* __restrict__ ray_mask, int dbg, int32_t* __restrict__ sub_cnt,
+                                                        int32_t* __restrict__ arr_idx, int32_t* __restrict__ arr_rank) {
     constexpr int RPW = 16 / NCH;
     __shared__ int s_list[4096];
     __shared__ int s_n, s_base;
@@ -390,10 +394,10 @@
         for (int ch = 0; ch < NCH; ++ch) {
             const int k = ch * 64 + lane;
             uint32_t word[kMarkRays];
-            int bit[kMarkRays];
+            int bit[kMarkRays], qs[kMarkRays];
 #pragma unroll
             for (int u = 0; u < kMarkRays; ++u) {
-                bit[u] = -1; word[u] = 0u;
+                bit[u] = -1; word[u] = 0u; qs[u] = 0;
                 if (k < S && rb + u < RPW && ray0 + rb + u < R) {
                     const float t = depth_at(nr[u], rg[u], k, S);
                     const float x = __fadd_rn(o[u][0], __fmul_rn(t, d[u][0])), y = __fadd_rn(o[u][1], __fmul_rn(t, d[u][1])),
@@ -404,30 +408,78 @@
                     const int cx = g.sub == 2 ? sx >> 1 : sx, cy = g.sub == 2 ? sy >> 1 : sy, cz = g.sub == 2 ? sz >> 1 : sz;
                     if (sx >= 0 && cx < g.nx && sy >= 0 && cy < g.ny && sz >= 0 && cz < g.nz) {
                         const int q = (sz * (g.ny * g.sub) + sy) * (g.nx * g.sub) + sx;
-                        bit[u] = q & 31;
+                        bit[u] = q & 31; qs[u] = q;
                         word[u] = near_mask[q >> 5];
                     }
                 }
             }
+            bool cnd[kMarkRays];
+            int rank[kMarkRays];
+#pragma unroll
+            for (int u = 0; u < kMarkRays; ++u) {
+                cnd[u] = bit[u] >= 0 && (((dbg & 2) || ((word[u] >> bit[u]) & 1u)) && !(dbg & 1));
+                rank[u] = 0;
+            }
+            if constexpr (CELLS) {
+                int before[kMarkRays], same[kMarkRays];
+#pragma unroll
+                for (int u = 0; u < kMarkRays; ++u) {
+                    before[u] = 0; same[u] = 0;
+#pragma unroll
+                    for (int v = 0; v < kMarkRays; ++v) {
+                        const bool eq = cnd[v] && qs[v] == qs[u];
+                        same[u] += eq ? 1 : 0;
+                        if (v < u) before[u] += eq ? 1 : 0;
+                    }
+                }
+#pragma unroll
+                for (int u = 0; u < kMarkRays; ++u)
+                    if (cnd[u] && before[u] == 0) rank[u] = atomicAdd(&sub_cnt[qs[u]], same[u]);
+#pragma unroll
+                for (int u = 1; u < kMarkRays; ++u)
+#pragma unroll
+                    for (int v = 0; v < u; ++v)
+                        if (cnd[u] && before[u] > 0 && cnd[v] && before[v] == 0 && qs[v] == qs[u]) rank[u] = rank[v] + before[u];
+            }
 #pragma unroll
             for (int u = 0; u < kMarkRays; ++u) {
                 const int ray = ray0 + rb + u;
-                const bool cand = bit[u] >= 0 && (((dbg & 2) || ((word[u] >> bit[u]) & 1u)) && !(dbg & 1));
+                const bool cand = cnd[u];
                 const unsigned long long cm = __ballot(cand);
                 if (rb + u < RPW && ray < R && lane == 0) ray_mask[(size_t)ray * NCH + ch] = 0ull;
                 if (cm) {
                     int base = 0;
                     if (lane == 0) base = atomicAdd(&s_n, __popcll(cm));
                     base = __shfl(base, 0);
-                    if (cand) s_list[base + __popcll(cm & ((1ull << lane) - 1ull))] = ray * S + k;
+                    const int pos = base + __popcll(cm & ((1ull << lane) - 1ull));
+                    if constexpr (!CELLS) {
+                        if (cand) s_list[pos] = ray * S + k;
+                    } else {
+                        if (cand && pos < kCellStage) { s_list[pos] = ray * S + k; s_list[kCellStage + pos] = rank[u]; }
+                        const bool over = cand && pos >= kCellStage;
+                        const unsigned long long om = __ballot(over);
+                        if (om) {
+                            int gb = 0;
+                            if (lane == 0) gb = atomicAdd(cand_count, __popcll(om));
+                            gb = __shfl(gb, 0);
+                            const int64_t at = (int64_t)gb + __popcll(om & ((1ull << lane) - 1ull));
+                            if (over && at < list_cap) { arr_idx[at] = ray * S + k; arr_rank[at] = rank[u]; }
+                        }
+                    }
                 }
             }
         }
     }
     __syncthreads();
-    const int n = s_n;
+    const int n = CELLS ? min(s_n, kCellStage) : s_n;
     if (threadIdx.x == 0) s_base = n ? atomicAdd(cand_count, n) : 0;
     __syncthreads();
+    if constexpr (CELLS) {
+        const int64_t gb = s_base;
+        for (int i = threadIdx.x; i < n; i += 256)
+            if (gb + i < list_cap) { arr_idx[gb + i] = s_list[i]; arr_rank[gb + i] = s_list[kCellStage + i]; }
+        return;
+    }
     const int64_t gb = s_base;
     for (int i = threadIdx.x; i < n; i += 256)
         if (gb + i < list_cap) {
@@ -694,6 +746,121 @@
     }
 }
 
+struct SherfCellWs { int32_t* sub_cnt; int32_t* sub_off; int32_t* cursors; int2* items; int64_t item_cap; };
+static inline int64_t sherf_cell_items(int R, int S) { return (int64_t)R * S / 64 + 1 + SHERF_NEAR_SUBCELLS; }
+static inline SherfCellWs sherf_cell_ws(int32_t* ws, int R, int S) {
+    return {ws, ws + SHERF_NEAR_SUBCELLS, ws + 2 * SHERF_NEAR_SUBCELLS, reinterpret_cast<int2*>(ws + 2 * SHERF_NEAR_SUBCELLS + 4), sherf_cell_items(R, S)};
+}
+
+__global__ void __launch_bounds__(256) cand_cells_alloc_kernel(const float* __restrict__ hdr, int32_t* __restrict__ sub_cnt, int32_t* __restrict__ sub_off,
+                                                               int32_t* __restrict__ cursors, int2* __restrict__ items, int64_t item_cap, int64_t list_cap) {
+    const CellGrid g = load_grid(hdr);
+    const int nsub = g.nx * g.ny * g.nz * g.sub * g.sub * g.sub;
+    if ((int)blockIdx.x * 256 >= ((nsub + 63) & ~63)) return;
+    const int q = blockIdx.x * 256 + threadIdx.x, lane = threadIdx.x & 63;
+    const int c = q < nsub ? sub_cnt[q] : 0;
+    if (c) sub_cnt[q] = 0;
+    const int nc = (c + 63) >> 6;
+    int incl = c, incl_i = nc;
+    for (int off = 1; off < 64; off <<= 1) {
+        const int v = __shfl_up(incl, off), vi = __shfl_up(incl_i, off);
+        if (lane >= off) { incl += v; incl_i += vi; }
+    }
+    const int total = __shfl(incl, 63), total_i = __shfl(incl_i, 63);
+    int base = 0, base_i = 0;
+    if (lane == 0 && total) {
+        const unsigned long long old = atomicAdd(reinterpret_cast<unsigned long long*>(cursors), ((unsigned long long)total_i << 32) | (unsigned)total);
+        base = (int)(unsigned)old; base_i = (int)(old >> 32);
+    }
+    base = __shfl(base, 0); base_i = __shfl(base_i, 0);
+    if (c) {
+        const int64_t start = (int64_t)base + (incl - c), first = (int64_t)base_i + (incl_i - nc);
+        if (start + c <= list_cap && first + nc <= item_cap) {
+            sub_off[q] = (int)start;
+            for (int j = 0; j < nc; ++j) items[first + j] = make_int2((int)start + 64 * j, q | ((min(64, c - 64 * j) - 1) << 20));
+        } else
+            sub_off[q] = -1;
+    }
+}
+
+__global__ void __launch_bounds__(256) cand_place_kernel(const float* __restrict__ ray_o, const float* __restrict__ ray_d, const float* __restrict__ near,
+                                                         const float* __restrict__ far, int S, const float* __restrict__ Rg, const float* __restrict__ Th,
+                                                         const float* __restrict__ hdr, const int32_t* __restrict__ arr_idx, const int32_t* __restrict__ arr_rank,
+                                                         const int32_t* __restrict__ cand_count, const int32_t* __restrict__ sub_off,
+                                                         float4* __restrict__ cand_list, int64_t list_cap) {
+    const CellGrid g = load_grid(hdr);
+    const float fs = g.inv_cell * (float)g.sub;
+    const int snx = g.nx * g.sub, sny = g.ny * g.sub, snz = g.nz * g.sub;
+    const int64_t n = min((int64_t)*cand_count, list_cap);
+    for (int64_t i = (int64_t)blockIdx.x * 256 + threadIdx.x; i < n; i += (int64_t)gridDim.x * 256) {
+        const int idx = arr_idx[i], rank = arr_rank[i];
+        const int ray = idx / S, k = idx - ray * S;
+        const float nr1 = near[ray], t = depth_at(nr1, __fsub_rn(far[ray], nr1), k, S);
+        const float x = __fadd_rn(ray_o[ray * 3], __fmul_rn(t, ray_d[ray * 3])), y = __fadd_rn(ray_o[ray * 3 + 1], __fmul_rn(t, ray_d[ray * 3 + 1])),
+                    z = __fadd_rn(ray_o[ray * 3 + 2], __fmul_rn(t, ray_d[ray * 3 + 2]));
+        float xs, ys, zs;
+        to_smpl_frame(x, y, z, Rg, Th, xs, ys, zs);
+        const int sx = (int)floorf((xs - g.ox) * fs), sy = (int)floorf((ys - g.oy) * fs), sz = (int)floorf((zs - g.oz) * fs);
+        if (sx < 0 || sx >= snx || sy < 0 || sy >= sny || sz < 0 || sz >= snz) continue;
+        const int off = sub_off[(sz * sny + sy) * snx + sx];
+        const int64_t at = (int64_t)off + rank;
+        if (off >= 0 && at < list_cap) cand_list[at] = make_float4(xs, ys, zs, __int_as_float(idx));
+    }
+}
+
+template <int NCH>
+__global__ void __launch_bounds__(256) cand_search_cells_kernel(const float4* __restrict__ cand_list, const int2* __restrict__ items,
+                                                                const int32_t* __restrict__ cursors, int64_t item_cap, int S,
+                                                                const int2* __restrict__ near_hdr, const uint16_t* __restrict__ near_list,
+                                                                const float4* __restrict__ cell_pts,
+                                                                unsigned long long* __restrict__ ray_mask, int32_t* __restrict__ dense_vid) {
+    __shared__ float4 s_pts[4][64];
+    const int lane = threadIdx.x & 63, wave = __builtin_amdgcn_readfirstlane((int)(threadIdx.x >> 6));
+    const int n_items = (int)min((int64_t)cursors[1], item_cap);
+    const unsigned long long kInit = ((unsigned long long)__float_as_uint(kThresh2) << 32) | 0x7FFFFFFFull;
+    const int stride = (int)gridDim.x * 4;
+    int it = (int)blockIdx.x * 4 + wave;
+    int2 item = items[it < n_items ? it : 0];
+    if (it >= n_items) return;
+    int2 h = near_hdr[item.y & 0xFFFFF];
+    float4 rec = cand_list[item.x + min(lane, item.y >> 20)];
+    for (; it < n_items; it += stride) {
+        const int n = (item.y >> 20) + 1, st = h.x, cn = h.y;
+        const bool live = lane < n;
+        const float xs = rec.x, ys = rec.y, zs = rec.z;
+        const int idx = __float_as_int(rec.w);
+        int e = lane;
+        float4 p = cell_pts[e < cn ? near_list[st + e] : 0];
+        const int itn = it + stride;
+        item = items[itn < n_items ? itn : 0];
+        h = near_hdr[item.y & 0xFFFFF];
+        rec = cand_list[item.x + min(lane, item.y >> 20)];
+        unsigned long long key = kInit;
+        for (int base = 0; base < cn; base += 64) {
+            __builtin_amdgcn_wave_barrier();
+            s_pts[wave][lane] = p;
+            __builtin_amdgcn_wave_barrier();
+            e = base + 64 + lane;
+            if (base + 64 < cn) p = cell_pts[e < cn ? near_list[st + e] : 0];
+            const int m = min(64, cn - base);
+#pragma unroll 4
+            for (int j = 0; j < m; ++j) {
+                const float4 v = s_pts[wave][j];
+                const float dd = dist2_exact(xs, ys, zs, v.x, v.y, v.z);
+                if (dd < kThresh2) {
+                    const unsigned long long cand = ((unsigned long long)__float_as_uint(dd) << 32) | (unsigned)__float_as_int(v.w);
+                    key = cand < key ? cand : key;
+                }
+            }
+        }
+        if (live && (unsigned)(key >> 32) < __float_as_uint(kThresh2)) {
+            const int ray = idx / S, k = idx - ray * S;
+            dense_vid[idx] = (int)(key & 0x7FFFFFFFull);
+            atomicOr(&ray_mask[(size_t)ray * NCH + (k >> 6)], 1ull << (k & 63));
+        }
+    }
+}
+
 template <int NCH>
 __global__ void __launch_bounds__(1024) scan_chunk_mask_kernel(const uint64_t* __restrict__ ray_mask, int R, int32_t* __restrict__ cnt,
                                                                int32_t* __restrict__ base, int32_t* __restrict__ chunk_sum) {
@@ -776,10 +943,11 @@
     }
 }
 
-__global__ void init_counters_kernel(int32_t* counters, int32_t* cand_count, int32_t* sticky) {
+__global__ void init_counters_kernel(int32_t* counters, int32_t* cand_count, int32_t* sticky, int32_t* cell_cursors) {
     if (sticky) { sticky[0] = max(sticky[0], counters[0]); sticky[1] |= counters[3]; sticky[2] += 1; }
     counters[0] = 0; counters[1] = 0x7FFFFFFF; counters[2] = (int32_t)0x80000000; counters[3] = 0;
     *cand_count = 0;
+    if (cell_cursors) { cell_cursors[0] = 0; cell_cursors[1] = 0; }
 }
 
 template <int NCH>
@@ -976,7 +1144,8 @@
 int sherf_sample_mask_nn_impl(const float* ray_o, const float* ray_d, const float* near, const float* far, int R, int S, const float* Rg, const float* Th,
                               const float* grid_hdr, const int32_t* cell_start, const float* cell_pts, const uint32_t* near_mask, int64_t capacity,
                               int32_t* counters, int32_t* ray_base, int32_t* ray_cnt, int32_t* cs_idx, int32_t* cs_vid, float* cs_xs, int32_t* dense_vid,
-                              uint64_t* ray_mask, int32_t* scan_ws, const int32_t* near_hdr, const uint16_t* near_list, sherf_stream_t stream, int32_t* sticky);
+                              uint64_t* ray_mask, int32_t* scan_ws, const int32_t* near_hdr, const uint16_t* near_list, sherf_stream_t stream, int32_t* sticky,
+                              int32_t* cell_ws, int64_t cell_ws_len);
 int sherf_warp_geom_impl(const int32_t* counters, const int32_t* cs_idx, const int32_t* cs_vid, const float* cs_xs, const float* ray_d, int S, const float* Rg,
                          const float* T2C, const float* C2S, const float* t_verts, const float* tgrid_hdr, const int32_t* tcell_start, const float* tcell_pts,
                          int64_t capacity, float* geom, int32_t* cs_tvid, sherf_stream_t stream);
@@ -1035,7 +1204,18 @@
                                        int32_t* cs_vid, float* cs_xs, int32_t* dense_vid, uint64_t* ray_mask,
                                        int32_t* scan_ws, const int32_t* near_hdr, const uint16_t* near_list, sherf_stream_t stream) {
     return sherf_sample_mask_nn_impl(ray_o, ray_d, near, far, R, S, Rg, Th, grid_hdr, cell_start, cell_pts, near_mask, capacity, counters, ray_base, ray_cnt,
-                                     cs_idx, cs_vid, cs_xs, dense_vid, ray_mask, scan_ws, near_hdr, near_list, stream, nullptr);
+                                     cs_idx, cs_vid, cs_xs, dense_vid, ray_mask, scan_ws, near_hdr, near_list, stream, nullptr, nullptr, 0);
+}
+
+extern "C" int sherf_sample_mask_nn_ws(const float* ray_o, const float* ray_d, const float* near, const float* far,
+                                       int R, int S, const float* Rg, const float* Th, const float* grid_hdr,
+                                       const int32_t* cell_start, const float* cell_pts, const uint32_t* near_mask, int64_t capacity,
+                                       int32_t* counters, int32_t* ray_base, int32_t* ray_cnt, int32_t* cs_idx,
+                                       int32_t* cs_vid, float* cs_xs, int32_t* dense_vid, uint64_t* ray_mask,
+                                       int32_t* scan_ws, const int32_t* near_hdr, const uint16_t* near_list, int32_t* cell_ws, int64_t cell_ws_len,
+                                       sherf_stream_t stream) {
+    return sherf_sample_mask_nn_impl(ray_o, ray_d, near, far, R, S, Rg, Th, grid_hdr, cell_start, cell_pts, near_mask, capacity, counters, ray_base, ray_cnt,
+                                     cs_idx, cs_vid, cs_xs, dense_vid, ray_mask, scan_ws, near_hdr, near_list, stream, nullptr, cell_ws, cell_ws_len);
 }
 
 template <int N>
@@ -1063,7 +1243,7 @@
 }
 
 int sherf_points_begin_impl(int32_t* counters, int32_t* scan_ws, int rows, int32_t* sticky, sherf_stream_t stream) {
-    hipLaunchKernelGGL(init_counters_kernel, dim3(1), dim3(1), 0, as_stream(stream), counters, sherf_scan_ws(scan_ws, rows).cand_count, sticky);
+    hipLaunchKernelGGL(init_counters_kernel, dim3(1), dim3(1), 0, as_stream(stream), counters, sherf_scan_ws(scan_ws, rows).cand_count, sticky, static_cast<int32_t*>(nullptr));
     SHERF_LAUNCH_CHECK();
 }
 int sherf_points_search_impl(int rows, const float* grid_hdr, const int32_t* cell_start, const float* cell_pts, const float* cand_list, int64_t list_cap,
@@ -1081,8 +1261,10 @@
                               const int32_t* cell_start, const float* cell_pts, const uint32_t* near_mask, int64_t capacity,
                               int32_t* counters, int32_t* ray_base, int32_t* ray_cnt, int32_t* cs_idx,
                               int32_t* cs_vid, float* cs_xs, int32_t* dense_vid, uint64_t* ray_mask,
-                              int32_t* scan_ws, const int32_t* near_hdr, const uint16_t* near_list, sherf_stream_t stream, int32_t* sticky) {
+                              int32_t* scan_ws, const int32_t* near_hdr, const uint16_t* near_list, sherf_stream_t stream, int32_t* sticky,
+                              int32_t* cell_ws, int64_t cell_ws_len) {
     SHERF_CHECK_ARG(ray_o && ray_d && near && far && Rg && Th && grid_hdr && cell_start && cell_pts && near_mask);
+    SHERF_CHECK_ARG(cell_ws == nullptr || (cell_ws_len >= SHERF_CELL_WS_INTS(R, S) && (reinterpret_cast<uintptr_t>(cell_ws) & 7) == 0));
     SHERF_CHECK_ARG(counters && ray_base && ray_cnt && cs_idx && cs_vid && cs_xs && dense_vid && ray_mask && scan_ws);
     SHERF_CHECK_ARG(R > 0 && S >= 2 && S <= 256 && (int64_t)R * S < 2147483647LL && capacity > 0 && (near_hdr == nullptr) == (near_list == nullptr));
     hipStream_t st = as_stream(stream);
@@ -1093,18 +1275,34 @@
     int32_t* chunk_sum = sw.chunk_sum;
     const float4* cp = reinterpret_cast<const float4*>(cell_pts);
     int32_t* cand_count = sw.cand_count;
-    hipLaunchKernelGGL(init_counters_kernel, dim3(1), dim3(1), 0, st, counters, cand_count, sticky);
+    const bool two_pass = !(g_sherf_debug & 512) && capacity >= (int64_t)R * S;
+    const bool cells = two_pass && cell_ws && near_hdr && near_list && !(g_sherf_debug & (16384 | kDebugSearchByCandidate)) && !(sherf_experiment() & 16384);
+    const SherfCellWs cw = sherf_cell_ws(cell_ws, R, S);
+    hipLaunchKernelGGL(init_counters_kernel, dim3(1), dim3(1), 0, st, counters, cand_count, sticky, cells ? cw.cursors : static_cast<int32_t*>(nullptr));
     hipLaunchKernelGGL(depth_minmax_kernel, dim3(min(256, cdiv(R, 256))), dim3(256), 0, st, near, far, R, S, counters);
-    const bool two_pass = !(g_sherf_debug & 512) && capacity >= (int64_t)R * S;
     if (two_pass) {
         float4* cand_list = reinterpret_cast<float4*>(cs_xs);
         const int64_t list_cap = capacity;
+        int32_t* const no_i32 = nullptr;
+        const int cells_wgs = ((g_sherf_debug >> 20) & 15) ? ((g_sherf_debug >> 20) & 15) : kCellSearchWgs;
 #define SHERF_TWO_PASS(N)                                                                                                          \
-        hipLaunchKernelGGL(cand_mark_kernel<N>, dim3(cdiv(R, 4 * (16 / N))), dim3(256), 0, st, ray_o, ray_d, near, far, R, S, Rg, Th,    \
-                           grid_hdr, near_mask, cand_list, list_cap, cand_count, ray_mask, g_sherf_debug);                         \
-        search_and_scan<N>(st, R, S, grid_hdr, cell_start, cp, cand_list, list_cap, cand_count, near_hdr, near_list, dense_vid, ray_mask, ray_cnt, base_local, \
-                           chunk_sum)
-        if (nch == 1) { SHERF_TWO_PASS(1); } else if (nch == 2) { SHERF_TWO_PASS(2); } else if (nch == 3) { SHERF_TWO_PASS(3); } else { SHERF_TWO_PASS(4); }
+        if (cells) {                                                                                                               \
+            hipLaunchKernelGGL((cand_mark_kernel<N, true>), dim3(cdiv(R, 4 * (16 / N))), dim3(256), 0, st, ray_o, ray_d, near, far, R, S, Rg, Th, \
+                               grid_hdr, near_mask, cand_list, list_cap, cand_count, ray_mask, g_sherf_debug, cw.sub_cnt, cs_idx, cs_vid); \
+            hipLaunchKernelGGL(cand_cells_alloc_kernel, dim3(SHERF_NEAR_SUBCELLS / 256), dim3(256), 0, st, grid_hdr, cw.sub_cnt, cw.sub_off, cw.cursors, \
+                               cw.items, cw.item_cap, list_cap);                                                                   \
+            hipLaunchKernelGGL(cand_place_kernel, dim3(min(8 * n_cus(), cdiv((int64_t)R * S, 256))), dim3(256), 0, st, ray_o, ray_d, near, far, S, Rg, Th, \
+                               grid_hdr, cs_idx, cs_vid, cand_count, cw.sub_off, cand_list, list_cap);                             \
+            hipLaunchKernelGGL(cand_search_cells_kernel<N>, dim3(cells_wgs * n_cus()), dim3(256), 0, st, cand_list, cw.items, cw.cursors, cw.item_cap, S, \
+                               reinterpret_cast<const int2*>(near_hdr), near_list, cp, reinterpret_cast<unsigned long long*>(ray_mask), dense_vid); \
+            hipLaunchKernelGGL(scan_chunk_mask_kernel<N>, dim3(cdiv(R, 1024)), dim3(1024), 0, st, ray_mask, R, ray_cnt, base_local, chunk_sum); \
+        } else {                                                                                                                   \
+            hipLaunchKernelGGL((cand_mark_kernel<N, false>), dim3(cdiv(R, 4 * (16 / N))), dim3(256), 0, st, ray_o, ray_d, near, far, R, S, Rg, Th, \
+                               grid_hdr, near_mask, cand_list, list_cap, cand_count, ray_mask, g_sherf_debug, no_i32, no_i32, no_i32); \
+            search_and_scan<N>(st, R, S, grid_hdr, cell_start, cp, cand_list, list_cap, cand_count, near_hdr, near_list, dense_vid, ray_mask, ray_cnt, base_local, \
+                               chunk_sum);                                                                                         \
+        }
+        if (nch == 1) { SHERF_TWO_PASS(1) } else if (nch == 2) { SHERF_TWO_PASS(2) } else if (nch == 3) { SHERF_TWO_PASS(3) } else { SHERF_TWO_PASS(4) }
 #undef SHERF_TWO_PASS
     } else {
     constexpr int nn_pad = 10 * 1024;
diff --git a/sherf_amd/renderer.py b/sherf_amd/renderer.py
--- a/sherf_amd/renderer.py
+++ b/sherf_amd/renderer.py
@@ -163,6 +163,7 @@
             near_mask=torch.zeros(32768, **i32),
             near_hdr=torch.zeros(2 * NEAR_SUBCELLS + 2, **i32),
             near_list=torch.zeros(125 * V + 3 * NEAR_SUBCELLS, dtype=torch.int16, device=dev),
+            cell_ws=torch.zeros(4 * NEAR_SUBCELLS + 6 + 2 * (R * S // 64), **i32),
         )
         self.key, self.t = key, t
         self.desc = None
@@ -204,7 +205,7 @@
 
     STATIC_FIELDS = ('A', 'posefeat', 'PO', 'SO', 'T2C', 'C2S', 'grid_hdr', 'cell_start', 'cell_pts', 'cell_scratch', 'near_mask',
                      'counters', 'ray_base', 'ray_cnt', 'cs_idx', 'cs_vid', 'cs_xs', 'dense_vid', 'ray_mask', 'scan_ws', 'geom',
-                     'cs_tvid', 'tokens', 'extras', 'sample_out')
+                     'cs_tvid', 'tokens', 'extras', 'sample_out', 'cell_ws')
 
     def descriptor(self, smpl):
         d = self.desc
@@ -215,6 +216,7 @@
         for k in self.STATIC_FIELDS:
             setattr(fr, k, A(self.t[k]))
         fr.sticky = A(self.t['counters']) + 16
+        fr.cell_ws_len = self.t['cell_ws'].numel()
         fr.J_template, fr.J_shapedirs, fr.parents = A(smpl['J_template']), A(smpl['J_shapedirs']), A(smpl['parents_i32'])
         fr.posedirs, fr.shapedirs, fr.weights = A(smpl['posedirs_flat']), A(smpl['shapedirs']), A(smpl['weights'])
         self.desc = (self.t, smpl, fr, dict(near_hdr=A(self.t['near_hdr']), near_list=A(self.t['near_list']), near_cap=self.t['near_list'].numel()))
```
